# sortmerna/sortmerna

Measured on AMD Instinct MI355X. Metric: reads/sec (150 bp vs smr_v4.3_default_db-sized DB), higher is better.
Workload: dtype u8/i32

## Files before the change

include/smr_hip.h:

```cpp
#ifndef SMR_HIP_H
#define SMR_HIP_H
#include <stddef.h>
#include <stdint.h>

#ifdef __cplusplus
extern "C" {
#endif

#define SMR_OK 0
#define SMR_ERR_ARG (-1)
#define SMR_ERR_IO (-2)
#define SMR_ERR_DEVICE (-3)
#define SMR_ERR_CAPACITY (-4)
#define SMR_ERR_STATE (-5)

typedef struct smr_ctx smr_ctx;
typedef struct smr_index smr_index;
typedef struct smr_reads smr_reads;

typedef struct {
  uint32_t skiplengths[3];
  int32_t  num_seeds;
  int32_t  min_lis;
  int32_t  edges;
// ... 108 lines not shown
  int32_t paired_in, paired_out, out2, sout;
  int32_t want_aligned, want_other;
} smr_fxsplit_opts;
int smr_fastx_split(smr_ctx*, int mates , const smr_fxsplit_opts*,
                    const uint8_t* hit , uint8_t* bytes, uint64_t cap, uint64_t off[9], uint64_t* need);
int smr_fastx_split_times(const smr_ctx*, double ms[4]);
typedef struct {
  int  want_sam, want_blast;
  char blast_cols[64];
  double lambda, K;
  uint64_t full_ref_corr, full_read_corr;
} smr_rows_opts;
int smr_rows_part(smr_ctx*, int slot, const smr_params*, const smr_index* ix, const smr_rows_opts*,
                  uint8_t* bytes, uint64_t cap, uint64_t off[3], uint64_t* need);
int smr_rows_times(const smr_ctx*, double ms[4]);
int smr_rows_fmt_batch(smr_ctx*, uint32_t n, const uint32_t* num, const uint32_t* den, char* out);
int smr_pairwise_part(smr_ctx*, int slot, const smr_params*, const smr_index* ix, double lambda, double K, uint64_t full_ref_corr, uint64_t full_read_corr,
                      uint8_t* bytes, uint64_t cap, uint64_t* need);
int smr_pairwise_times(const smr_ctx*, double ms[4]);
typedef struct { uint32_t ref_num, n_reads; uint64_t off; } smr_otu_group;
int smr_otu_part(smr_ctx*, int slot, const smr_params*, const smr_index* ix, double min_id, double min_cov,
                 uint8_t* bytes, uint64_t cap, smr_otu_group* groups, uint64_t groups_cap, uint64_t need[2] , int* any_yid_ycov);
int smr_otu_times(const smr_ctx*, double ms[5]);
int smr_otu_sort_batch(smr_ctx*, uint32_t n, const uint32_t* keys, uint32_t key_bits, uint32_t* perm);
int smr_fastx_denovo(smr_ctx*, int mates, const smr_fxsplit_opts*, const uint8_t* dn ,
                     uint8_t* bytes, uint64_t cap, uint64_t off[5], uint64_t* need);
int smr_state_reset(smr_ctx*);

int smr_align_part(smr_ctx*, int slot, const smr_params*);
int smr_traceback(smr_ctx*, int slot, const smr_params*);

int smr_counters(smr_ctx*, uint64_t* out, uint32_t n_db);
int smr_counters_device(smr_ctx*, void** dptr, uint32_t* n_u64);
int smr_counters_accumulate(smr_ctx*, void* d_acc, uint32_t n_u64);

int smr_idcov_part(smr_ctx*, int slot, const smr_params*, double min_id, double min_cov);
int smr_idcov_counters(smr_ctx*, uint64_t out[4]);
int smr_idcov_counters_device(smr_ctx*, void** dptr, uint32_t* n_u64);
#define SMR_COUNTERS_WITH_IDCOV 70
int smr_idcov_batch(smr_ctx*, uint32_t n, const uint8_t* reads, const uint64_t* read_off, const uint8_t* refs, const uint64_t* ref_off,
                    const uint32_t* cigars, const uint64_t* cigar_off, const int32_t* read_begin, const int32_t* read_end, const uint32_t* readlen,
                    double min_id, double min_cov, uint32_t* out);

int    smr_results_fetch(smr_ctx*);
size_t smr_result_record(const smr_ctx*, uint32_t read_idx, uint8_t* buf, size_t cap);
size_t smr_result_record_batch(const smr_ctx*, int batch, uint32_t read_idx, uint8_t* buf, size_t cap);
int    smr_result_is_hit(const smr_ctx*, uint32_t read_idx);

int smr_state_import(smr_ctx*, const uint8_t* bytes, const uint64_t* off, uint32_t n);
int smr_state_export(smr_ctx*, uint8_t* bytes, uint64_t cap, uint64_t* off, uint32_t n, uint64_t* need);
int smr_counters_import(smr_ctx*, const uint64_t* in, uint32_t n_db);

int smr_seed_scan(smr_ctx*, int slot, const smr_params*, int strand, int pass, uint64_t* n_hits_out);
int smr_seed_hits_fetch(smr_ctx*, uint32_t* triples, uint64_t cap_triples, uint64_t* n_out);

typedef struct {
  double   seed_ms;  uint64_t seed_launches;
  double   chain_ms; uint64_t chain_launches;
  double   trace_ms; uint64_t trace_launches;
  uint64_t n_windows, n_lookup, n_node, n_entry, n_hit, n_read_bytes;
  uint64_t n_sw_fwd, n_sw_rev, n_sw_cells;
  uint64_t n_sw_spec, n_sw_spec_used;
  uint64_t n_seed_redo;
  uint64_t hit_list_cap;
  uint64_t n_seed_shared;
  uint64_t n_seed_shared_builds;
} smr_prof;
int smr_index_build_gpu(smr_ctx*, const char* ref_fasta, uint32_t lnwin, double max_mb, uint32_t max_pos,
                        smr_index** parts_out, uint32_t cap_parts, uint32_t* n_parts_out, char* err, size_t errcap);

int smr_sw_selfcheck(smr_ctx*, uint32_t n_cases, uint32_t seed, uint32_t max_len, uint64_t* n_bad);
int smr_sw_mode(smr_ctx*, int set_to);
int smr_walk_rounds(const smr_ctx*, uint32_t out[3]);
int smr_ssw_batch(smr_ctx*, uint32_t n_pairs, const uint8_t* reads, const uint64_t* read_off, const uint8_t* refs, const uint64_t* ref_off,
                  int match, int mismatch, int score_N, int gap_open, int gap_ext, uint32_t filters, int mode, int32_t* out);
int smr_sw_long_rows(int m);
typedef struct {
  uint32_t read, win_off;
  uint16_t aq, m, nref;
  uint8_t reversed, list_b;
} smr_sw16_task;
int smr_sw16_batch(smr_ctx*, uint32_t n_tasks, const smr_sw16_task* tasks, const uint8_t* ref, uint64_t ref_len, int force_any_n,
                   int match, int mismatch, int score_N, int gap_open, int gap_ext, uint32_t filters, int rows, uint32_t blocks, int32_t* out);
int smr_sw16_launches(const smr_ctx*, uint64_t out[8]);
int smr_cigar_batch(smr_ctx*, uint32_t n_pairs, const uint8_t* reads, const uint64_t* read_off, const uint8_t* refs, const uint64_t* ref_off,
                    const uint16_t* scores, int match, int mismatch, int score_N, int gap_open, int gap_ext,
                    uint32_t* cigar_out, uint64_t cigar_cap, uint64_t* cigar_off_out);
int smr_prof_reset(smr_ctx*);
int smr_prof_get(smr_ctx*, smr_prof* out);
typedef struct { char name[32]; double ms; uint64_t launches; uint64_t bytes; } smr_kprof;
int smr_prof_kernels(smr_ctx*, smr_kprof* out, uint32_t cap, uint32_t* n_out);

typedef struct smr_report smr_report;
typedef struct {
  int fastx;
  int other;
  int blast_tabular;
  char blast_cols[64];
  int sam;
  int blast_pairwise;
  int sam_sq;
  int paired_in;
  int paired_out;
  int out2;
  int sout;
  int zip_out;
  int otu_map;
  int denovo;
  double min_id, min_cov;
} smr_report_opts;
int smr_report_open(const char* out_dir, const smr_report_opts*, int is_fastq, smr_report** out, char* err, size_t errcap);
int smr_report_set_db(smr_report*, uint32_t index_num, double lambda, double K, uint64_t full_ref_corr, uint64_t full_read_corr);
int smr_report_set_part(smr_report*, uint32_t index_num, uint32_t part, const smr_index*);
int smr_report_add(smr_report*, const char* header, const char* seq, const char* qual, const uint8_t* record, size_t record_len);
int smr_report_add_pair(smr_report*, const char* header1, const char* seq1, const char* qual1, const uint8_t* record1, size_t record1_len,
                        const char* header2, const char* seq2, const char* qual2, const uint8_t* record2, size_t record2_len);
int smr_report_add_fastx(smr_report*, const uint8_t* bytes, const uint64_t off[9]);
int smr_report_add_rows(smr_report*, uint32_t index_num, uint32_t part, const uint8_t* bytes, const uint64_t off[3]);
int smr_report_skip_rows(smr_report*, int on);
int smr_report_add_pairwise(smr_report*, uint32_t index_num, uint32_t part, const uint8_t* bytes, uint64_t n);
int smr_report_skip_pairwise(smr_report*, int on);
int smr_report_skip_fastx(smr_report*, int on);
int smr_report_add_otu(smr_report*, uint32_t index_num, uint32_t part, const uint8_t* bytes, uint64_t n_bytes, const smr_otu_group* groups,
                       uint64_t n_groups, int any_yid_ycov);
int smr_report_skip_otu(smr_report*, int on);
int smr_report_add_denovo(smr_report*, const uint8_t* bytes, const uint64_t off[5]);
int smr_report_skip_denovo(smr_report*, int on);
int smr_report_otu_count(smr_report*, uint64_t* total_otu);
int smr_report_otu_merge(smr_report* dst, smr_report* src);
int smr_report_set_cmdline(smr_report*, const char* cmdline);
int smr_report_close(smr_report*);
const char* smr_report_last_error(const smr_report*);

typedef struct {
  const char* ref_file;
  uint32_t skiplengths[3];
  double lambda, K;
  uint32_t minimal_score;
  uint64_t reads_matched;
} smr_summary_db;
typedef struct {
  const char* cmdline; const char* pid; const char* timestamp;
  uint32_t seed_len; int32_t num_seeds, edges, match, mismatch, gap_open, gap_ext, score_N; int32_t sam_sq; int32_t threads;
  const char* const* reads_files; uint32_t n_reads_files;
  uint64_t total_reads, num_aligned, all_reads_len; uint32_t min_read_len, max_read_len;
  const smr_summary_db* dbs; uint32_t n_dbs;
  int is_denovo; uint64_t total_denovo;
  int is_otu_map; uint64_t total_id_cov, total_otu;
} smr_summary;
int smr_summary_write(const char* path, const smr_summary*);

size_t smr_readstats_record(uint64_t all_reads_count, uint64_t all_reads_len, uint32_t min_read_len, uint32_t max_read_len, uint64_t num_aligned,
                            uint64_t num_short, const uint64_t* reads_matched_per_db, uint32_t n_db, uint8_t* buf, size_t cap);
size_t smr_readstats_key(const char* const* reads_files, uint32_t n_files, char* buf, size_t cap);

#ifdef __cplusplus
}
#endif
#endif
```

sortmerna_amd/capi.py:

```python
import ctypes as C
import os

from . import build as _build


class Params(C.Structure):
    _fields_ = [
        ("skiplengths", C.c_uint32 * 3), ("num_seeds", C.c_int32), ("min_lis", C.c_int32), ("edges", C.c_int32),
        ("is_as_percent", C.c_int32), ("match", C.c_int32), ("mismatch", C.c_int32), ("score_N", C.c_int32),
        ("gap_open", C.c_int32), ("gap_ext", C.c_int32), ("num_alignments", C.c_uint32), ("is_best", C.c_int32),
        ("is_full_search", C.c_int32), ("is_forward", C.c_int32), ("is_reverse", C.c_int32), ("minoccur", C.c_uint32),
        ("minimal_score", C.c_uint32), ("index_num", C.c_uint32), ("part", C.c_uint32),
        ("is_last_index_part", C.c_int32),
    ]


class IndexInfo(C.Structure):
    _fields_ = [
        ("lnwin", C.c_uint32), ("n_kmers", C.c_uint32), ("trie_words", C.c_uint64), ("n_ids", C.c_uint32),
        ("n_pos", C.c_uint64), ("n_refs", C.c_uint32), ("ref_bytes", C.c_uint64), ("n_nodes", C.c_uint64),
        ("n_buckets", C.c_uint64), ("n_entries", C.c_uint64), ("bg", C.c_double * 4), ("full_len", C.c_uint64),
        ("numseq", C.c_uint64), ("n_parts", C.c_uint32),
    ]


class ReportOpts(C.Structure):
    _fields_ = [("fastx", C.c_int), ("other", C.c_int), ("blast_tabular", C.c_int), ("blast_cols", C.c_char * 64), ("sam", C.c_int),
                ("blast_pairwise", C.c_int), ("sam_sq", C.c_int), ("paired_in", C.c_int), ("paired_out", C.c_int), ("out2", C.c_int), ("sout", C.c_int), ("zip_out", C.c_int),
                ("otu_map", C.c_int), ("denovo", C.c_int), ("min_id", C.c_double), ("min_cov", C.c_double)]


class FxSplitOpts(C.Structure):
    _fields_ = [("layout", C.c_int32), ("paired_in", C.c_int32), ("paired_out", C.c_int32), ("out2", C.c_int32), ("sout", C.c_int32),
                ("want_aligned", C.c_int32), ("want_other", C.c_int32)]


class RowsOpts(C.Structure):
    _fields_ = [("want_sam", C.c_int), ("want_blast", C.c_int), ("blast_cols", C.c_char * 64), ("lam", C.c_double), ("K", C.c_double),
                ("full_ref_corr", C.c_uint64), ("full_read_corr", C.c_uint64)]


class SummaryDb(C.Structure):
    _fields_ = [("ref_file", C.c_char_p), ("skiplengths", C.c_uint32 * 3), ("lam", C.c_double), ("K", C.c_double),
                ("minimal_score", C.c_uint32), ("reads_matched", C.c_uint64)]


class Summary(C.Structure):
    _fields_ = [("cmdline", C.c_char_p), ("pid", C.c_char_p), ("timestamp", C.c_char_p), ("seed_len", C.c_uint32),
                ("num_seeds", C.c_int32), ("edges", C.c_int32), ("match", C.c_int32), ("mismatch", C.c_int32), ("gap_open", C.c_int32),
                ("gap_ext", C.c_int32), ("score_N", C.c_int32), ("sam_sq", C.c_int32), ("threads", C.c_int32),
                ("reads_files", C.POINTER(C.c_char_p)), ("n_reads_files", C.c_uint32),
                ("total_reads", C.c_uint64), ("num_aligned", C.c_uint64), ("all_reads_len", C.c_uint64),
                ("min_read_len", C.c_uint32), ("max_read_len", C.c_uint32), ("dbs", C.POINTER(SummaryDb)), ("n_dbs", C.c_uint32),
                ("is_denovo", C.c_int), ("total_denovo", C.c_uint64), ("is_otu_map", C.c_int), ("total_id_cov", C.c_uint64), ("total_otu", C.c_uint64)]


class Prof(C.Structure):
    _fields_ = [
        ("seed_ms", C.c_double), ("seed_launches", C.c_uint64), ("chain_ms", C.c_double), ("chain_launches", C.c_uint64),
        ("trace_ms", C.c_double), ("trace_launches", C.c_uint64), ("n_windows", C.c_uint64), ("n_lookup", C.c_uint64),
        ("n_node", C.c_uint64), ("n_entry", C.c_uint64), ("n_hit", C.c_uint64), ("n_read_bytes", C.c_uint64),
        ("n_sw_fwd", C.c_uint64), ("n_sw_rev", C.c_uint64), ("n_sw_cells", C.c_uint64), ("n_sw_spec", C.c_uint64), ("n_sw_spec_used", C.c_uint64), ("n_seed_redo", C.c_uint64), ("hit_list_cap", C.c_uint64),
        ("n_seed_shared", C.c_uint64), ("n_seed_shared_builds", C.c_uint64),
    ]


class Kprof(C.Structure):
    _fields_ = [("name", C.c_char * 32), ("ms", C.c_double), ("launches", C.c_uint64), ("bytes", C.c_uint64)]


EXPORTS = [
    "smr_otu_part", "smr_otu_times", "smr_otu_sort_batch", "smr_fastx_denovo", "smr_report_add_otu", "smr_report_skip_otu", "smr_report_add_denovo", "smr_report_skip_denovo",
    "smr_params_default", "smr_params_refused", "smr_index_load_files", "smr_index_build", "smr_index_build_gpu", "smr_index_write_files", "smr_index_save", "smr_index_load_flat", "smr_index_selfcheck", "smr_index_free",
    "smr_index_get_info", "smr_minimal_score", "smr_minimal_score_split", "smr_refstats_corrected_split", "smr_reads_pack", "smr_reads_load_fastx", "smr_reads_load_fastx_mt", "smr_reads_load_fastx_text", "smr_reads_is_fastq", "smr_reads_record_text", "smr_reads_free", "smr_reads_slice",
    "smr_reads_digest", "smr_reads_count", "smr_reads_total_len", "smr_reads_min_len", "smr_reads_max_len", "smr_create", "smr_device_count", "smr_destroy",
    "smr_last_error", "smr_tuning_text", "smr_index_upload", "smr_index_check_device", "smr_index_pigeonhole", "smr_seed_tuples_fetch", "smr_seed_pool_info", "smr_cand_info_enable", "smr_cand_info", "smr_cand_routes", "smr_index_unload", "smr_batch_select", "smr_set_seed_mode", "smr_reads_upload", "smr_reads_upload_batch", "smr_reads_upload_fastx", "smr_reads_upload_fastx_batch", "smr_reads_upload_fastx_file", "smr_fastx_info", "smr_fastx_times", "smr_fastx_split", "smr_fastx_split_times", "smr_rows_part", "smr_rows_times", "smr_rows_fmt_batch", "smr_pairwise_part", "smr_pairwise_times", "smr_state_reset", "smr_align_part",
    "smr_traceback", "smr_counters", "smr_counters_device", "smr_state_import", "smr_state_export", "smr_counters_import", "smr_results_fetch", "smr_result_record", "smr_result_record_batch", "smr_counters_accumulate",
    "smr_result_is_hit", "smr_seed_scan", "smr_seed_hits_fetch", "smr_sw_selfcheck", "smr_sw_mode", "smr_walk_rounds", "smr_ssw_batch", "smr_sw16_batch", "smr_sw16_launches", "smr_sw_long_rows", "smr_cigar_batch", "smr_idcov_part", "smr_idcov_counters", "smr_idcov_counters_device", "smr_idcov_batch", "smr_prof_reset", "smr_prof_get", "smr_prof_kernels", "smr_refstats_corrected", "smr_report_open",
    "smr_report_set_db", "smr_report_set_part", "smr_report_add", "smr_report_add_pair", "smr_report_add_fastx", "smr_report_skip_fastx", "smr_report_add_rows", "smr_report_skip_rows", "smr_report_add_pairwise", "smr_report_skip_pairwise", "smr_report_set_cmdline", "smr_report_otu_count", "smr_report_otu_merge", "smr_report_close", "smr_report_last_error",
    "smr_summary_write", "smr_readstats_record", "smr_readstats_key",
]

_lib = None


def load(rebuild_if_stale=True):
    global _lib
    if _lib is not None:
        return _lib
    path = _build.LIB
    if rebuild_if_stale and _build.is_stale():
        path = _build.build_library()
    if not os.path.isfile(path):
        raise RuntimeError("libsmr_hip.so is missing; run sortmerna_amd/build.py (needs hipcc)")
    _lib = bind(C.CDLL(path))
    return _lib


def bind(L):
    vp, cp, u32, u64, i32 = C.c_void_p, C.c_char_p, C.c_uint32, C.c_uint64, C.c_int
    L.smr_params_default.argtypes = [C.POINTER(Params)]
    L.smr_index_load_files.restype = i32
    L.smr_index_load_files.argtypes = [cp, u32, cp, C.POINTER(vp), cp, C.c_size_t]
    L.smr_index_build.restype = i32
    L.smr_index_build.argtypes = [cp, u32, C.c_double, u32, u32, C.POINTER(vp), u32, C.POINTER(u32), cp, C.c_size_t]
    L.smr_index_build_gpu.restype = i32
    L.smr_index_build_gpu.argtypes = [vp, cp, u32, C.c_double, u32, C.POINTER(vp), u32, C.POINTER(u32), cp, C.c_size_t]
    L.smr_index_write_files.restype = i32
    L.smr_index_write_files.argtypes = [C.POINTER(vp), u32, cp, cp, cp, C.c_size_t]
    L.smr_index_save.restype = i32
    L.smr_index_save.argtypes = [vp, cp, u64, cp, C.c_size_t]
    L.smr_index_load_flat.restype = i32
    L.smr_index_load_flat.argtypes = [cp, u64, C.POINTER(vp), cp, C.c_size_t]
    L.smr_index_selfcheck.restype = i32
    L.smr_index_selfcheck.argtypes = [vp, cp, C.c_size_t]
    L.smr_index_free.argtypes = [vp]
    L.smr_index_get_info.restype = i32
    L.smr_index_get_info.argtypes = [vp, C.POINTER(IndexInfo)]
    L.smr_minimal_score.restype = u32
    L.smr_minimal_score.argtypes = [C.c_double, C.c_double, C.POINTER(C.c_double), u64, u64, u64, u64, C.c_double]
    L.smr_minimal_score_split.restype = u32
    L.smr_minimal_score_split.argtypes = [C.c_double, C.c_double, C.POINTER(C.c_double), u64, u64, u64, u64, C.c_double, u32]
    L.smr_reads_pack.restype = i32
    L.smr_reads_pack.argtypes = [cp, vp, u32, C.POINTER(vp)]
    L.smr_reads_load_fastx.restype = i32
    L.smr_reads_load_fastx.argtypes = [cp, u64, u64, C.POINTER(vp), cp, C.c_size_t]
    L.smr_reads_load_fastx_mt.restype = i32
    L.smr_reads_load_fastx_mt.argtypes = [cp, u32, C.POINTER(vp), cp, C.c_size_t]
    L.smr_reads_load_fastx_text.restype = i32
    L.smr_reads_load_fastx_text.argtypes = [cp, u32, C.POINTER(vp), cp, C.c_size_t]
    L.smr_reads_is_fastq.restype = i32
    L.smr_reads_is_fastq.argtypes = [vp]
    L.smr_reads_record_text.restype = i32
    L.smr_reads_record_text.argtypes = [vp, u32, cp, C.c_size_t, cp, C.c_size_t, cp, C.c_size_t, C.POINTER(C.c_size_t)]
    L.smr_reads_free.argtypes = [vp]
    for f in ("smr_reads_count", "smr_reads_min_len", "smr_reads_max_len"):
        getattr(L, f).restype = u32
        getattr(L, f).argtypes = [vp]
    L.smr_reads_digest.restype = u64
    L.smr_reads_digest.argtypes = [vp]
    L.smr_reads_total_len.restype = u64
    L.smr_reads_total_len.argtypes = [vp]
    L.smr_create.restype = i32
    L.smr_create.argtypes = [i32, C.POINTER(vp), cp, C.c_size_t]
    L.smr_destroy.argtypes = [vp]
    L.smr_last_error.restype = cp
    L.smr_last_error.argtypes = [vp]
    L.smr_tuning_text.restype = i32
    L.smr_tuning_text.argtypes = [vp, cp, C.c_size_t]
    L.smr_index_upload.restype = i32
    L.smr_index_upload.argtypes = [vp, vp, i32]
    L.smr_index_check_device.restype = i32
    L.smr_index_check_device.argtypes = [vp, i32, vp]
    L.smr_index_pigeonhole.restype = i32
    L.smr_index_pigeonhole.argtypes = [vp, C.POINTER(C.POINTER(C.c_uint32)), C.POINTER(u64), C.POINTER(C.POINTER(C.c_uint32)), C.POINTER(u64), cp, C.c_size_t]
    L.smr_seed_tuples_fetch.restype = i32
    L.smr_seed_tuples_fetch.argtypes = [vp, vp, u64, vp, u32, C.POINTER(u32)]
    L.smr_seed_pool_info.restype = i32
    L.smr_seed_pool_info.argtypes = [vp, C.POINTER(u64)]
    L.smr_cand_info_enable.restype = i32
    L.smr_cand_info_enable.argtypes = [vp, i32]
    L.smr_cand_info.restype = i32
    L.smr_cand_info.argtypes = [vp, C.POINTER(u64)]
    L.smr_cand_routes.restype = i32
    L.smr_cand_routes.argtypes = [vp, vp, u32]
    L.smr_index_unload.restype = i32
    L.smr_index_unload.argtypes = [vp, i32]
    L.smr_batch_select.restype = i32
    L.smr_batch_select.argtypes = [vp, i32]
    L.smr_set_seed_mode.restype = i32
    L.smr_set_seed_mode.argtypes = [vp, i32]
    L.smr_reads_upload.restype = i32
    L.smr_reads_upload.argtypes = [vp, vp, u32]
    L.smr_state_reset.restype = i32
    L.smr_state_reset.argtypes = [vp]
    L.smr_align_part.restype = i32
    L.smr_align_part.argtypes = [vp, i32, C.POINTER(Params)]
    L.smr_traceback.restype = i32
    L.smr_traceback.argtypes = [vp, i32, C.POINTER(Params)]
    L.smr_counters.restype = i32
    L.smr_counters.argtypes = [vp, C.POINTER(u64), u32]
    L.smr_state_import.restype = i32
    L.smr_state_import.argtypes = [vp, vp, vp, u32]
    L.smr_state_export.restype = i32
    L.smr_state_export.argtypes = [vp, vp, u64, vp, u32, C.POINTER(u64)]
    L.smr_counters_import.restype = i32
    L.smr_counters_import.argtypes = [vp, C.POINTER(u64), u32]
    L.smr_counters_device.restype = i32
    L.smr_counters_device.argtypes = [vp, C.POINTER(vp), C.POINTER(u32)]
    L.smr_results_fetch.restype = i32
    L.smr_results_fetch.argtypes = [vp]
    L.smr_result_record.restype = C.c_size_t
    L.smr_result_record.argtypes = [vp, u32, vp, C.c_size_t]
    L.smr_result_record_batch.restype = C.c_size_t
    L.smr_result_record_batch.argtypes = [vp, i32, u32, vp, C.c_size_t]
    L.smr_counters_accumulate.restype = i32
    L.smr_counters_accumulate.argtypes = [vp, vp, u32]
    L.smr_result_is_hit.restype = i32
    L.smr_result_is_hit.argtypes = [vp, u32]
    L.smr_seed_scan.restype = i32
    L.smr_seed_scan.argtypes = [vp, i32, C.POINTER(Params), i32, i32, C.POINTER(u64)]
    L.smr_seed_hits_fetch.restype = i32
    L.smr_seed_hits_fetch.argtypes = [vp, vp, u64, C.POINTER(u64)]
    L.smr_sw_selfcheck.restype = i32
    L.smr_sw_selfcheck.argtypes = [vp, u32, u32, u32, C.POINTER(u64)]
    L.smr_ssw_batch.restype = i32
    L.smr_ssw_batch.argtypes = [vp, u32, vp, vp, vp, vp, i32, i32, i32, i32, i32, u32, i32, vp]
    L.smr_sw16_batch.restype = i32
    L.smr_sw16_batch.argtypes = [vp, u32, vp, vp, u64, i32, i32, i32, i32, i32, i32, u32, i32, u32, vp]
    L.smr_sw16_launches.restype = i32
    L.smr_sw16_launches.argtypes = [vp, C.POINTER(u64)]
    L.smr_sw_long_rows.restype = i32
    L.smr_sw_long_rows.argtypes = [i32]
    L.smr_readstats_record.restype = C.c_size_t
    L.smr_readstats_record.argtypes = [u64, u64, u32, u32, u64, u64, vp, u32, vp, C.c_size_t]
    L.smr_readstats_key.restype = C.c_size_t
    L.smr_readstats_key.argtypes = [vp, u32, vp, C.c_size_t]
    L.smr_reads_upload_batch.restype = i32
    L.smr_reads_upload_batch.argtypes = [vp, i32, vp, u32]
    L.smr_reads_upload_fastx.restype = i32
    L.smr_reads_upload_fastx.argtypes = [vp, vp, u64, u32, u32, C.POINTER(vp)]
    L.smr_reads_upload_fastx_batch.restype = i32
    L.smr_reads_upload_fastx_batch.argtypes = [vp, i32, vp, u64, u32, u32, C.POINTER(vp)]
    L.smr_reads_upload_fastx_file.restype = i32
    L.smr_reads_upload_fastx_file.argtypes = [vp, cp, u32, u32, C.POINTER(vp), cp, C.c_size_t]
    L.smr_fastx_info.restype = i32
    L.smr_fastx_info.argtypes = [vp, C.POINTER(u64)]
    L.smr_fastx_times.restype = i32
    L.smr_fastx_times.argtypes = [vp, C.POINTER(C.c_double)]
    L.smr_fastx_split.restype = i32
    L.smr_fastx_split.argtypes = [vp, i32, C.POINTER(FxSplitOpts), vp, vp, u64, C.POINTER(u64), C.POINTER(u64)]
    L.smr_fastx_split_times.restype = i32
    L.smr_fastx_split_times.argtypes = [vp, C.POINTER(C.c_double)]
    L.smr_rows_part.restype = i32
    L.smr_rows_part.argtypes = [vp, i32, C.POINTER(Params), vp, C.POINTER(RowsOpts), vp, u64, C.POINTER(u64), C.POINTER(u64)]
    L.smr_rows_times.restype = i32
    L.smr_rows_times.argtypes = [vp, C.POINTER(C.c_double)]
    L.smr_rows_fmt_batch.restype = i32
    L.smr_rows_fmt_batch.argtypes = [vp, u32, vp, vp, vp]
    L.smr_report_add_rows.restype = i32
    L.smr_report_add_rows.argtypes = [vp, u32, u32, vp, C.POINTER(u64)]
    L.smr_report_skip_rows.restype = i32
    L.smr_report_skip_rows.argtypes = [vp, i32]
    L.smr_pairwise_part.restype = i32
    L.smr_pairwise_part.argtypes = [vp, i32, C.POINTER(Params), vp, C.c_double, C.c_double, u64, u64, vp, u64, C.POINTER(u64)]
    L.smr_pairwise_times.restype = i32
    L.smr_pairwise_times.argtypes = [vp, C.POINTER(C.c_double)]
    L.smr_report_add_pairwise.restype = i32
    L.smr_report_add_pairwise.argtypes = [vp, u32, u32, vp, u64]
    L.smr_report_skip_pairwise.restype = i32
    L.smr_report_skip_pairwise.argtypes = [vp, i32]
    L.smr_otu_part.restype = i32
    L.smr_otu_part.argtypes = [vp, i32, C.POINTER(Params), vp, C.c_double, C.c_double, vp, u64, vp, u64, C.POINTER(u64), C.POINTER(i32)]
    L.smr_otu_times.restype = i32
    L.smr_otu_times.argtypes = [vp, C.POINTER(C.c_double)]
    L.smr_otu_sort_batch.restype = i32
    L.smr_otu_sort_batch.argtypes = [vp, u32, vp, u32, vp]
    L.smr_fastx_denovo.restype = i32
    L.smr_fastx_denovo.argtypes = [vp, i32, C.POINTER(FxSplitOpts), vp, vp, u64, C.POINTER(u64), C.POINTER(u64)]
    L.smr_report_add_otu.restype = i32
    L.smr_report_add_otu.argtypes = [vp, u32, u32, vp, u64, vp, u64, i32]
    L.smr_report_skip_otu.restype = i32
    L.smr_report_skip_otu.argtypes = [vp, i32]
    L.smr_report_add_denovo.restype = i32
    L.smr_report_add_denovo.argtypes = [vp, vp, C.POINTER(u64)]
    L.smr_report_skip_denovo.restype = i32
    L.smr_report_skip_denovo.argtypes = [vp, i32]
    L.smr_report_add_fastx.restype = i32
    L.smr_report_add_fastx.argtypes = [vp, vp, C.POINTER(u64)]
    L.smr_report_skip_fastx.restype = i32
    L.smr_report_skip_fastx.argtypes = [vp, i32]
    L.smr_reads_slice.restype = i32
    L.smr_reads_slice.argtypes = [vp, u64, u64, C.POINTER(vp)]
    L.smr_idcov_part.restype = i32
    L.smr_idcov_part.argtypes = [vp, i32, C.POINTER(Params), C.c_double, C.c_double]
    L.smr_idcov_counters.restype = i32
    L.smr_idcov_counters.argtypes = [vp, C.POINTER(u64)]
    L.smr_idcov_counters_device.restype = i32
    L.smr_idcov_counters_device.argtypes = [vp, C.POINTER(vp), C.POINTER(u32)]
    L.smr_idcov_batch.restype = i32
    L.smr_idcov_batch.argtypes = [vp, u32, vp, vp, vp, vp, vp, vp, vp, vp, vp, C.c_double, C.c_double, vp]
    L.smr_cigar_batch.restype = i32
    L.smr_cigar_batch.argtypes = [vp, u32, vp, vp, vp, vp, vp, i32, i32, i32, i32, i32, vp, u64, vp]
    L.smr_sw_mode.restype = i32
    L.smr_sw_mode.argtypes = [vp, i32]
    L.smr_walk_rounds.restype = i32
    L.smr_walk_rounds.argtypes = [vp, C.POINTER(C.c_uint32)]
    L.smr_prof_reset.restype = i32
    L.smr_prof_reset.argtypes = [vp]
    L.smr_prof_get.restype = i32
    L.smr_prof_get.argtypes = [vp, C.POINTER(Prof)]
    L.smr_prof_kernels.restype = i32
# ... 30 lines not shown
```

sortmerna_amd/csrc/smr_engine.hip:

```cpp
#include <hip/hip_runtime.h>

#include <algorithm>
#include <mutex>
#include <cstdio>
#include <cstdlib>
#include <cstring>
#include <string>
#include <vector>

#include "smr_kernels.hpp"
#include "smr_idcov.hpp"
#include "smr_import.hpp"
#include "smr_export.hpp"
#include "smr_fastx.hpp"
#include "smr_fxsplit.hpp"
#include "smr_rows.hpp"
#include "smr_pairwise.hpp"
#include "smr_otu.hpp"
#include "smr_ibuild.hpp"
#include "smr_pgbuild.hpp"
#include "smr_hostmem.hpp"
#include "smr_devbuf.hpp"
#include "smr_score_text.hpp"
#include "smr_tuning.hpp"
// ... 81 lines not shown
  double ms[4] = {0, 0, 0, 0};
  FxSplitScratch() = default;
  FxSplitScratch(const FxSplitScratch&) = delete;
  FxSplitScratch& operator=(const FxSplitScratch&) = delete;
  ~FxSplitScratch() { for (auto e : ev) if (e) (void)hipEventDestroy(e); }
};

struct RowsScratch {
  DevBuf<uint4> stat, meta; DevBuf<unsigned long long> excl_s, excl_b, part_s, part_b; DevBuf<uint32_t> err; DevBuf<uint8_t> tab, out;
  uint32_t tab_n = 0; double tab_lambda = 0, tab_K = 0; uint64_t tab_ref = 0, tab_read = 0;
  hipEvent_t ev[7] = {};
  double ms[4] = {0, 0, 0, 0};
  RowsScratch() = default;
  RowsScratch(const RowsScratch&) = delete;
  RowsScratch& operator=(const RowsScratch&) = delete;
  ~RowsScratch() { for (auto e : ev) if (e) (void)hipEventDestroy(e); }
};

struct PairScratch {
  hipEvent_t ev[7] = {};
  double ms[4] = {0, 0, 0, 0};
  PairScratch() = default;
  PairScratch(const PairScratch&) = delete;
  PairScratch& operator=(const PairScratch&) = delete;
  ~PairScratch() { for (auto e : ev) if (e) (void)hipEventDestroy(e); }
};

struct OtuScratch {
  DevBuf<uint8_t> pass, out; DevBuf<uint2> meta; DevBuf<uint4> pairs; DevBuf<uint32_t> key[2], val[2], gstart, err;
  DevBuf<unsigned long long> excl, part, hist, wexcl, wpart, gexcl, gpart; DevBuf<OtuGroup> groups;
  hipEvent_t ev[10] = {};
  double ms[5] = {0, 0, 0, 0, 0};
  OtuScratch() = default;
  OtuScratch(const OtuScratch&) = delete;
  OtuScratch& operator=(const OtuScratch&) = delete;
  ~OtuScratch() { for (auto e : ev) if (e) (void)hipEventDestroy(e); }
};

struct smr_ctx {
  const Tuning tune;
  explicit smr_ctx(const Tuning& t) : tune(t) {}
  int device = 0;
  DevStream stream, upload_stream;
  std::string err;
  std::mutex err_m, sel_m;
  int n_cu = 256;
  DevIndex idx[64];
  Batch bt[SMR_MAX_BATCHES];
  Batch* b = &bt[0];
  DevBuf<uint32_t> d_pool; uint64_t pool_words = 0;
  uint64_t n_pool_grown = 0;
  uint32_t pool_inline = 0;
  uint32_t hcap = 4;
  int seed_exact = tune.seed_exact;
  uint32_t cand_bloom = tune.cand_bloom;
  int seed_shared = tune.seed_shared;
  DevBuf<uint16_t> d_sw_scr; uint32_t sw_scr_stride = 0;
  int last_seed_slot = -1;
  SharedSort shared;
  uint64_t n_seed_shared = 0, n_seed_shared_builds = 0;
  uint32_t ccap = tune.ccap;
  SeedScratch seed; SeedBufs sb = {};
  uint64_t sb_slots = 0; uint32_t sb_nk = 0;
  uint32_t chain_blocks = 0;
  DevBuf<unsigned long long> d_tuples; uint32_t chain_scap = 512;
  uint32_t keys_need = 0;
  bool chain_ext = false;
  DevBuf<uint32_t> d_stab; DevBuf<unsigned long long> d_tuples2;
  size_t chain_lds_attr = 0, begins_lds_attr = 0, split_lds_attr = 0, bins_lds_attr = 0;
  DevBuf<uint32_t> d_fidx; DevBuf<RState> d_fstate; DevBuf<AlignRec> d_faln;
  DevBuf<uint32_t> d_fidcov;
  DevBuf<uint8_t> d_xbytes; DevBuf<unsigned long long> d_xoff, d_xpart;
  int sw_mode = tune.sw_packed;
  DevBuf<unsigned long long> d_keys; uint32_t keys_cap = 0;
  DevBuf<unsigned long long> d_pairs; DevBuf<uint32_t> d_lis; uint32_t pairs_cap = 0;
  DevBuf<uint2> d_hits; uint32_t hits_cap = 0;
  DevBuf<uint8_t> d_rdq;
  DevBuf<uint2> d_mrec; DevBuf<uint32_t> d_mpool;
  DevBuf<uint2> d_wlist[2]; DevBuf<WState> d_wstate[2]; DevBuf<WTask> d_wtask[2]; DevBuf<uint2> d_wres[2];
  DevBuf<uint32_t> d_wtidx, d_wslow; DevBuf<unsigned long long> d_wctr; size_t walk_cap = 0; uint32_t walk_kcap = 0;
  size_t walk_lds_attr = 0, pg_lds_attr = 0, search_lds_attr = 0;
  uint64_t sw16_launches[8] = {};
  uint32_t walk_need[3] = {0, 0, 0};
  DevBuf<unsigned long long> d_wstat; uint32_t wstat_n = 0; int wstat_pass[8] = {}; uint32_t wstat_rm[8] = {};
  DevBuf<int> d_bound;
  DevBuf<uint32_t> d_tasks;
  DevBuf<uint8_t> d_trflags;
  DevBuf<int> d_trrows;
  EvPool ev;
  double kp_ms[KP_COUNT] = {}; uint64_t kp_l[KP_COUNT] = {};
  DevBuf<unsigned long long> d_ctr_snap;
  bool cinfo_on = false; DevBuf<uint8_t> d_croute; uint32_t croute_n = 0;
  uint32_t cinfo_attempts = 0, cinfo_retry[5] = {0, 0, 0, 0, 0};
  FxScratch fx[2];
  uint64_t fx_info[4] = {0, 0, 0, 0}; double fx_ms[5] = {0, 0, 0, 0, 0};
  FxSplitScratch fxs;
  RowsScratch rows;
  PairScratch pair;
  OtuScratch otu;
};
struct KpSave { double ms[KP_COUNT]; uint64_t l[KP_COUNT]; };

#define SEED_REDO_CAP 16384u

int dev_fail(smr_ctx* c, const char* call, hipError_t e) {
  std::lock_guard<std::mutex> l_(c->err_m);
  c->err = std::string(call) + ": " + hipGetErrorString(e);
  return SMR_ERR_DEVICE;
}

namespace {

#define HIPCHK(ctx, call)                                          \
  do {                                                             \
    hipError_t e_ = (call);                                        \
    if (e_ != hipSuccess) return dev_fail((ctx), #call, e_);       \
  } while (0)

void set_err(smr_ctx* c, const std::string& msg) { std::lock_guard<std::mutex> l_(c->err_m); c->err = msg; }


template <class T> struct arg_of { typedef T type; };
template <class... P> void launch(smr_ctx* c, void (*k)(P...), dim3 grid, dim3 block, size_t lds, typename arg_of<P>::type... a) {
  hipLaunchKernelGGL(k, grid, block, lds, c->stream, a...);
}
template <class... P> void launch_on(hipStream_t st, void (*k)(P...), dim3 grid, dim3 block, size_t lds, typename arg_of<P>::type... a) {
  hipLaunchKernelGGL(k, grid, block, lds, st, a...);
}
template <class... F> int raise_lds_limit(smr_ctx* c, size_t& high_water, size_t bytes, size_t free_bytes, F... kernels) {
  if (bytes <= free_bytes || bytes <= high_water) return SMR_OK;
  for (const void* k : {(const void*)kernels...}) HIPCHK(c, hipFuncSetAttribute(k, hipFuncAttributeMaxDynamicSharedMemorySize, (int)bytes));
  high_water = bytes;
  return SMR_OK;
}

const char* scheme_unsupported(int mismatch, int score_N, int gap_open, int gap_ext);
DParams make_dparams(const smr_ctx* c, const DevIndex& di, const smr_params* p) {
  DParams P;
  memset(&P, 0, sizeof P);
  P.lnwin = di.lnwin; P.partialwin = di.lnwin / 2;
  if (p->skiplengths[0] == 0 || p->skiplengths[1] == 0 || p->skiplengths[2] == 0) {
    P.skip[0] = di.lnwin; P.skip[1] = di.lnwin / 2; P.skip[2] = 3;
  } else { P.skip[0] = p->skiplengths[0]; P.skip[1] = p->skiplengths[1]; P.skip[2] = p->skiplengths[2]; }
  P.num_seeds = p->num_seeds; P.min_lis = p->min_lis; P.edges = p->edges; P.is_as_percent = p->is_as_percent;
  P.match = p->match; P.mismatch = p->mismatch; P.score_N = p->score_N; P.gap_open = p->gap_open; P.gap_ext = p->gap_ext;
  P.minimal_score = p->minimal_score; P.num_alignments = p->num_alignments;
  P.is_best = p->is_best; P.is_full_search = p->is_full_search; P.is_forward = p->is_forward; P.is_reverse = p->is_reverse;
  P.minoccur = p->minoccur; P.index_num = p->index_num; P.part = p->part; P.is_last_index_part = p->is_last_index_part;
  P.slots = c->b->slots;
  P.sw_mode = scheme_unsupported(p->mismatch, p->score_N, p->gap_open, p->gap_ext) ? -1 : c->sw_mode;
  P.sw_scratch = c->d_sw_scr; P.sw_scratch_stride = c->sw_scr_stride;
  return P;
}

const char* scheme_unsupported(int mismatch, int score_N, int gap_open, int gap_ext) {
  const int mm = std::max(-mismatch, -std::min(score_N, 0));
  if (2 * gap_open < mm || 2 * gap_ext < mm) return "scoring scheme outside the supported range (2*gap_open and 2*gap_ext must be >= |mismatch|)";
  if (score_N > 0) return "scoring scheme outside the supported range (score_N must be <= 0: the kernels pad sequences with N)";
  if (gap_open <= gap_ext) return "scoring scheme outside the supported range (gap_open must be greater than gap_ext: the reference's 16-bit kernel ends its lazy-F loop early otherwise, ssw.c:496-507)";
  return nullptr;
}

int check_params(smr_ctx* c, const smr_params* p, bool sw = true) {
  if (!p) { set_err(c, "null params"); return SMR_ERR_ARG; }
  if (p->index_num >= 64) { set_err(c, "index_num must be < 64"); return SMR_ERR_ARG; }
  if ((uint64_t)p->minoccur >= 0x3FFFFFFFull) { set_err(c, "minoccur must be < 2^30 - 1"); return SMR_ERR_ARG; }
// ... 410 lines not shown
  c->wstat_n = 0;
  const uint32_t tb = 256, nb = (B.n + tb - 1) / tb;
  const int single = (p->is_forward != 0) ^ (p->is_reverse != 0);
  launch(c, k_ctr_begin, dim3(1), dim3(256), 0, B.d_ctr, c->d_ctr_snap);
  launch(c, k_begin_part, dim3(nb), dim3(tb), 0, dreads(c), P, B.d_saved, B.d_saved_aln, B.d_work, B.d_work_aln, B.d_rw, B.d_ctr);
  for (int count = 0; count < (single ? 1 : 2); count++) {
    launch(c, k_begin_strand, dim3(nb), dim3(tb), 0, B.n, P, count, B.d_work, B.d_rw);
    HIPCHK(c, hipMemsetAsync(&B.d_ctr[C_PCUR], 0, C_NSHARD * C_PCUR_STRIDE * 8, c->stream));
    for (int pass = 0; pass < 3; pass++) {
      if (pass > 0 && P.skip[pass] == P.skip[pass - 1]) continue;
      if ((rc = launch_seed(c, di, P, pass, !p->is_last_index_part, ((single && p->is_reverse) || count == 1) ? 1 : 0))) return rc;
      if ((rc = launch_chain(c, di, P, plan, pass, single || count == 1))) return rc;
    }
  }
  HIPCHK(c, hipGetLastError());
  return SMR_OK;
}

int judge_attempt(smr_ctx* c, const DParams& P, const std::vector<unsigned long long>& h, bool& retry) {
  int rc;
  retry = false;
  if (h[C_ERR_HITCAP]) { c->cinfo_retry[0]++; if (!grow_hcap(c, P.partialwin)) return SMR_ERR_CAPACITY; retry = true; }
  if (h[C_ERR_POOL]) { c->cinfo_retry[1]++; if ((rc = grow_pool(c))) return rc; retry = true; }
  if (h[C_ERR_PAIRS]) {
    c->cinfo_retry[2]++;
    c->pairs_cap *= 4; c->hits_cap *= 4; c->d_pairs.release(); c->d_lis.release(); c->d_hits.release(); c->d_tuples.release(); c->d_tuples2.release();
    if (c->pairs_cap > (1u << 22)) { set_err(c, "per-read candidate scratch exceeds capacity"); return SMR_ERR_CAPACITY; }
    retry = true;
  }
  if (h[C_ERR_REDO]) { c->cinfo_retry[3]++; c->seed_exact = 1; retry = true; }
  {
    Batch& B = *c->b;
    if (h[C_SEED_REDO] < B.redo_seen || h[C_WINDOWS] < B.win_seen) B.redo_seen = B.win_seen = 0;
    const unsigned long long redo = h[C_SEED_REDO] - B.redo_seen, waves = (h[C_WINDOWS] - B.win_seen) / 32;
    B.redo_seen = h[C_SEED_REDO]; B.win_seen = h[C_WINDOWS];
    if (!retry && redo * 64 > waves && c->ccap < PG_CAND_CAP_MAX) {
      c->ccap *= 2;
      say(c->tune, "%llu of ~%llu seed-search waves overflowed their candidate pool: %u records per wave from now on\n", redo, waves, c->ccap);
    }
  }
  if (h[C_ERR_SCAP]) {
    if (c->chain_ext) { set_err(c, "more than 49152 references share seeds with one read (candidate set capacity)"); return SMR_ERR_CAPACITY; }
    c->chain_ext = true; retry = true; c->cinfo_retry[4]++;
    say(c->tune, "a read shares seeds with more references than its wave's LDS table holds: per-block global candidate tables enabled (%.1f GB)\n",
        (double)c->chain_blocks * (4.0 * CH_EXT_CAP * 4 + (double)c->pairs_cap * 8 + (double)CH_EXT_CAP * 8) / 1e9);
    if (c->keys_cap < CH_EXT_CAP) { c->d_keys.release(); c->keys_cap = 0; c->keys_need = CH_EXT_CAP; }
  }
  if (h[C_ERR_SLOTS]) { set_err(c, "a read produced more alignments than max_alignments_per_read (smr_reads_upload)"); return SMR_ERR_CAPACITY; }
  return SMR_OK;
}
}

extern "C" int smr_align_part(smr_ctx* c, int slot, const smr_params* p) {
  if (!c || slot < 0 || slot >= 64) return SMR_ERR_ARG;
  if (!c->idx[slot].used || !c->b->d_saved) { set_err(c, "index slot empty or no reads uploaded"); return SMR_ERR_STATE; }
  if (c->b->idcov_ran) { set_err(c, "smr_align_part after smr_idcov_part: the id / coverage pass counts final alignments (denovo_stats runs after align, processor.cpp:368); smr_state_reset or upload first"); return SMR_ERR_STATE; }
  HIPCHK(c, hipSetDevice(c->device));
  int rc = check_params(c, p); if (rc) return rc;
  const DevIndex& di = c->idx[slot];
  if (di.lnwin < 8 || di.lnwin > 20) { set_err(c, "unsupported seed length"); return SMR_ERR_ARG; }
  DParams P = make_dparams(c, di, p);
  if ((rc = refuse_percent_edges(c, di, p))) return rc;
  const AlignPlan plan = align_plan(c, P);
  if (plan.lds > 150 * 1024) { set_err(c, "reads too long for this build of the SW kernel (LDS)"); return SMR_ERR_CAPACITY; }
  c->b->last_num_alignments = p->num_alignments;
  c->b->fetched = false;
  ev_drop(c);
  if (c->b->n == 0) return SMR_OK;
  if ((rc = ensure_pool(c))) return rc;
  if (plan.striped && (rc = ensure_striped_scratch(c, P, p))) return rc;
  std::vector<unsigned long long> h;
  HIPCHK(c, hipMemcpyAsync(c->d_ctr_snap, c->b->d_ctr, C_TOTAL * 8, hipMemcpyDeviceToDevice, c->stream));
  c->cinfo_attempts = 0;
  for (int q = 0; q < 5; q++) c->cinfo_retry[q] = 0;
  for (int attempt = 0; attempt < 16; attempt++) {
    const KpSave kp0 = kp_save(c);
    if ((rc = run_attempt(c, di, P, p, plan))) return rc;
    if ((rc = read_ctr(c, h))) return rc;
    ev_collect(c);
    bool retry;
    if ((rc = judge_attempt(c, P, h, retry))) return rc;
    if (retry) { kp_restore(c, kp0); continue; }
    if ((rc = adapt_walk_rounds(c))) return rc;
    if ((rc = launch_begins(c, di, P, plan))) return rc;
    launch(c, k_commit_part, dim3((c->b->n + 255u) / 256u), dim3(256), 0, c->b->n, P, c->b->d_saved, c->b->d_saved_aln, c->b->d_work, c->b->d_work_aln, c->b->d_rw);
    HIPCHK(c, hipGetLastError());
    HIPCHK(c, hipStreamSynchronize(c->stream));
    ev_collect(c);
    return SMR_OK;
  }
  set_err(c, "capacity retries exhausted");
  return SMR_ERR_CAPACITY;
}

#include "smr_engine_trace.hpp"
#include "smr_engine_idcov.hpp"
#include "smr_engine_import.hpp"
#include "smr_engine_export.hpp"
#include "smr_engine_fastx.hpp"
#include "smr_engine_fxsplit.hpp"
#include "smr_engine_rows.hpp"
#include "smr_engine_pairwise.hpp"
#include "smr_engine_otu.hpp"
extern "C" int smr_counters(smr_ctx* c, uint64_t* out, uint32_t n_db) {
  if (!c || !out) return SMR_ERR_ARG;
  HIPCHK(c, hipSetDevice(c->device));
  std::vector<unsigned long long> h;
  int rc = read_ctr(c, h); if (rc) return rc;
  out[0] = h[C_NUM_ALIGNED]; out[1] = h[C_NUM_SHORT];
  for (uint32_t i = 0; i < n_db && i < 64; i++) out[2 + i] = h[C_PER_DB + i];
  return SMR_OK;
}
extern "C" int smr_counters_device(smr_ctx* c, void** dptr, uint32_t* n_u64) {
  if (!c || !dptr || !n_u64) return SMR_ERR_ARG;
  *dptr = c->b->d_ctr; *n_u64 = C_PER_DB + 64;
  return SMR_OK;
}

__global__ void k_ctr_accumulate(const unsigned long long* __restrict__ ctr, unsigned long long* __restrict__ acc, uint32_t n) {
  const uint32_t k = blockIdx.x * blockDim.x + threadIdx.x;
  if (k < n) acc[k] += ctr[k < C_PER_DB + 64 ? k : C_IDCOV + (k - (C_PER_DB + 64))];
}
extern "C" int smr_counters_accumulate(smr_ctx* c, void* d_acc, uint32_t n_u64) {
  if (!c || !d_acc || n_u64 > C_PER_DB + 64 + 4 || !c->b->d_ctr) return SMR_ERR_ARG;
  HIPCHK(c, hipSetDevice(c->device));
  launch(c, k_ctr_accumulate, dim3((n_u64 + 127) / 128), dim3(128), 0, (const unsigned long long*)c->b->d_ctr, (unsigned long long*)d_acc, n_u64);
  HIPCHK(c, hipGetLastError());
  HIPCHK(c, hipStreamSynchronize(c->stream));
  return SMR_OK;
}

__global__ void k_results_compact(uint32_t n, uint32_t slots, const RState* __restrict__ saved, const AlignRec* __restrict__ saved_aln,
                                  uint32_t* __restrict__ out_idx, RState* __restrict__ out_state, AlignRec* __restrict__ out_aln, unsigned long long* __restrict__ ctr) {
  const uint32_t r = blockIdx.x * blockDim.x + threadIdx.x;
  RState s; s.n_align = 0;
  if (r < n) s = saved[r];
  const uint32_t p = block_append(&ctr[C_FETCH_N], s.n_align != 0);
  if (s.n_align == 0) return;
  out_idx[p] = r; out_state[p] = s;
  for (uint32_t k = 0; k < s.n_align && k < slots; k++) out_aln[(size_t)p * slots + k] = saved_aln[(size_t)r * slots + k];
}

extern "C" int smr_results_fetch(smr_ctx* c) {
  if (!c || !c->b->d_saved) return SMR_ERR_STATE;
  HIPCHK(c, hipSetDevice(c->device));
  Batch& B = *c->b;
  int rc;
  const size_t need_r = std::max<size_t>(B.n, 1), need_a = std::max<size_t>((size_t)B.n * B.slots, 1);
  if ((rc = c->d_fidx.reserve(c, need_r)) || (rc = c->d_fstate.reserve(c, need_r)) || (rc = c->d_faln.reserve(c, need_a))) return rc;
  HIPCHK(c, hipMemsetAsync(&B.d_ctr[C_FETCH_N], 0, 8, c->stream));
  if (B.n) launch(c, k_results_compact, dim3((B.n + 1023) / 1024), dim3(1024), 0, B.n, B.slots, (const RState*)B.d_saved, (const AlignRec*)B.d_saved_aln,
                              c->d_fidx, c->d_fstate, c->d_faln, B.d_ctr);
  std::vector<unsigned long long> h;
  rc = read_ctr(c, h); if (rc) return rc;
  const uint64_t cw = std::min<uint64_t>(h[C_CIGAR_CURSOR], B.cigar_words);
  const size_t nhit = (size_t)std::min<unsigned long long>(h[C_FETCH_N], B.n);
  B.h_cigar.resize(cw);
  B.h_idx.resize(nhit); B.h_state.resize(nhit); B.h_aln.resize(nhit * B.slots);
  if (nhit) {
    HIPCHK(c, hipMemcpyAsync(B.h_idx.data(), c->d_fidx, nhit * 4, hipMemcpyDeviceToHost, c->stream));
    HIPCHK(c, hipMemcpyAsync(B.h_state.data(), c->d_fstate, nhit * sizeof(RState), hipMemcpyDeviceToHost, c->stream));
    HIPCHK(c, hipMemcpyAsync(B.h_aln.data(), c->d_faln, nhit * B.slots * sizeof(AlignRec), hipMemcpyDeviceToHost, c->stream));
  }
  if (cw) HIPCHK(c, hipMemcpyAsync(B.h_cigar.data(), B.d_cigar, cw * 4, hipMemcpyDeviceToHost, c->stream));
  B.h_idcov.clear();
  if (B.d_idcov && nhit) {
// ... 110 lines not shown
  if (tuples) { if (cap_tuples < nt) return SMR_ERR_CAPACITY; if (nt) HIPCHK(c, hipMemcpy(tuples, c->sb.srt, (size_t)nt * sizeof(SeedTup), hipMemcpyDeviceToHost)); }
  if (cbase) { if (cap_cbase < c->sb.nc + 1u) return SMR_ERR_CAPACITY; HIPCHK(c, hipMemcpy(cbase, c->sb.cbase, (size_t)(c->sb.nc + 1u) * 4, hipMemcpyDeviceToHost)); }
  return SMR_OK;
}

extern "C" int smr_seed_pool_info(smr_ctx* c, uint64_t info[4]) {
  if (!c || !info) return SMR_ERR_ARG;
  HIPCHK(c, hipSetDevice(c->device));
  std::vector<unsigned long long> cur(C_NSHARD * C_PCUR_STRIDE, 0ull);
  if (c->b->d_ctr) {
    HIPCHK(c, hipMemcpyAsync(cur.data(), &c->b->d_ctr[C_PCUR], cur.size() * 8, hipMemcpyDeviceToHost, c->stream));
    HIPCHK(c, hipStreamSynchronize(c->stream));
  }
  const uint64_t region = std::min<uint64_t>(c->pool_words, 0x7FFFFFF0ull) / C_NSHARD;
  uint64_t hi = 0;
  for (int s = 0; s < C_NSHARD; s++) if (cur[s * C_PCUR_STRIDE]) hi = std::max<uint64_t>(hi, s * region + cur[s * C_PCUR_STRIDE]);
  info[0] = c->pool_words; info[1] = c->n_pool_grown; info[2] = hi; info[3] = c->pool_inline;
  return SMR_OK;
}

extern "C" int smr_cand_info_enable(smr_ctx* c, int on) {
  if (!c) return SMR_ERR_ARG;
  c->cinfo_on = on != 0;
  if (!c->cinfo_on) c->croute_n = 0;
  return SMR_OK;
}
extern "C" int smr_cand_info(smr_ctx* c, uint64_t info[13]) {
  if (!c || !info) return SMR_ERR_ARG;
  info[0] = c->cinfo_attempts;
  for (int q = 0; q < 5; q++) info[1 + q] = c->cinfo_retry[q];
  info[6] = c->chain_ext ? 1 : 0; info[7] = c->chain_scap; info[8] = c->keys_cap; info[9] = c->pairs_cap; info[10] = c->hits_cap;
  info[11] = c->cinfo_on ? 1 : 0; info[12] = c->croute_n;
  return SMR_OK;
}
extern "C" int smr_cand_routes(smr_ctx* c, uint8_t* out, uint32_t n) {
  if (!c || !out) return SMR_ERR_ARG;
  if (!c->cinfo_on || !c->d_croute || n != c->croute_n) { set_err(c, "smr_cand_routes: no route bytes for that many reads (smr_cand_info_enable before smr_align_part)"); return SMR_ERR_STATE; }
  HIPCHK(c, hipSetDevice(c->device));
  if (n) { HIPCHK(c, hipMemcpyAsync(out, c->d_croute, (size_t)n, hipMemcpyDeviceToHost, c->stream)); HIPCHK(c, hipStreamSynchronize(c->stream)); }
  return SMR_OK;
}

extern "C" int smr_seed_hits_fetch(smr_ctx* c, uint32_t* triples, uint64_t cap_triples, uint64_t* n_out) {
  if (!c || !n_out) return SMR_ERR_ARG;
  HIPCHK(c, hipSetDevice(c->device));
  std::vector<unsigned long long> h;
  int rc = read_ctr(c, h); if (rc) return rc;
  uint64_t words = h[C_POOL_CURSOR] ? std::min<uint64_t>(c->pool_words, 0x7FFFFFF0ull) : 0;
  std::vector<uint32_t> pool(words);
  std::vector<RWork> rw(c->b->n);
  if (words) HIPCHK(c, hipMemcpy(pool.data(), c->d_pool, words * 4, hipMemcpyDeviceToHost));
  if (c->b->n) HIPCHK(c, hipMemcpy(rw.data(), c->b->d_rw, (size_t)c->b->n * sizeof(RWork), hipMemcpyDeviceToHost));
  std::vector<uint32_t> po;
  if (c->last_seed_slot >= 0 && c->idx[c->last_seed_slot].used) {
    const DevIndex& di = c->idx[c->last_seed_slot];
    po.resize((size_t)di.n_ids + 1);
    HIPCHK(c, hipMemcpy(po.data(), di.pos_off, po.size() * 4, hipMemcpyDeviceToHost));
  }
  auto orig = [&](uint32_t idp) -> uint32_t {
    if (po.size() < 2) return idp;
    size_t lo = 0, hi = po.size() - 1;
    while (hi - lo > 1) { const size_t mid = (lo + hi) / 2; if ((uint64_t)po[mid] + mid <= idp) lo = mid; else hi = mid; }
    return (uint32_t)lo;
  };
  uint64_t o = 0;
  for (uint32_t r = 0; r < c->b->n; r++) {
    for (int pp = 0; pp < 3; pp++) {
      const uint32_t cnt = rw[r].blk_cnt[pp], bo = rw[r].blk_off[pp];
      for (uint32_t q = 0; q < cnt && (uint64_t)bo + 2 * q + 1 < words; q++) {
        if (triples && o < cap_triples) { triples[3 * o] = r; triples[3 * o + 1] = orig(pool[bo + 2 * q]); triples[3 * o + 2] = pool[bo + 2 * q + 1]; }
        o++;
      }
    }
  }
  *n_out = o;
  return SMR_OK;
}

extern "C" int smr_prof_reset(smr_ctx* c) {
  if (!c) return SMR_ERR_ARG;
  HIPCHK(c, hipSetDevice(c->device));
  for (int k = 0; k < KP_COUNT; k++) { c->kp_ms[k] = 0; c->kp_l[k] = 0; }
  c->n_seed_shared = c->n_seed_shared_builds = 0;
  for (int k = 0; k < SMR_MAX_BATCHES; k++)
    if (c->bt[k].d_ctr) {
      HIPCHK(c, hipMemsetAsync(&c->bt[k].d_ctr[C_WINDOWS], 0, 9 * 8, c->stream));
      HIPCHK(c, hipMemsetAsync(&c->bt[k].d_ctr[C_SW_SPEC], 0, 3 * 8, c->stream));
      HIPCHK(c, hipMemsetAsync(&c->bt[k].d_ctr[C_TUP_F], 0, C_SHARD_NX * 8, c->stream));
      HIPCHK(c, hipMemsetAsync(&c->bt[k].d_ctr[C_SHARDS], 0, C_SHARD_W * C_NSHARD * 8, c->stream));
    }
  HIPCHK(c, hipStreamSynchronize(c->stream));
  return SMR_OK;
}
extern "C" int smr_prof_get(smr_ctx* c, smr_prof* o) {
  if (!c || !o) return SMR_ERR_ARG;
  HIPCHK(c, hipSetDevice(c->device));
  std::vector<unsigned long long> h(C_TOTAL, 0), t(C_TOTAL);
  for (int k = 0; k < SMR_MAX_BATCHES; k++) {
    if (!c->bt[k].d_ctr) continue;
    HIPCHK(c, hipMemcpyAsync(t.data(), c->bt[k].d_ctr, C_TOTAL * 8, hipMemcpyDeviceToHost, c->stream));
    HIPCHK(c, hipStreamSynchronize(c->stream));
    if (c->tune.debug_phases) {
      unsigned long long ph[7] = {0, 0, 0, 0, 0, 0, 0};
      for (int s2 = 0; s2 < C_NSHARD; s2++) for (int q = 0; q < 7; q++) ph[q] += t[C_SHARDS + C_SHARD_W * s2 + C_SHARD_PH + q];
      fprintf(stderr, "[smr] phase cycles (batch %d): %llu %llu %llu %llu %llu %llu %llu  (-DSMR_CHAIN_PHASES: claim, gather+prefix, walk1, walk2+cands, pairs+sort, "
              "window/lis/book, sw; -DSMR_SEED_PHASES (k_seed_pg): setup, directory ranges, entries, -, candidate selection, output, -)\n", k, ph[0], ph[1], ph[2], ph[3], ph[4], ph[5], ph[6]);
    }
    fold_shards(t);
    for (int q = 0; q < C_COUNT; q++) h[q] += t[q];
  }
  o->seed_ms = c->kp_ms[KP_KEYS] + c->kp_ms[KP_SPLIT] + c->kp_ms[KP_BINS] + c->kp_ms[KP_PG0] + c->kp_ms[KP_PG1] + c->kp_ms[KP_FINISH]; o->seed_launches = c->kp_l[KP_KEYS];
  o->chain_ms = c->kp_ms[KP_CAND] + c->kp_ms[KP_CHAIN] + c->kp_ms[KP_BEGINS] + c->kp_ms[KP_WALK] + c->kp_ms[KP_SW16] + c->kp_ms[KP_WNEXT]; o->chain_launches = c->kp_l[KP_CAND] + c->kp_l[KP_BEGINS];
  o->trace_ms = c->kp_ms[KP_TRACE]; o->trace_launches = c->kp_l[KP_TRACE];
  o->n_windows = h[C_WINDOWS]; o->n_lookup = h[C_LOOKUP]; o->n_node = h[C_NODE]; o->n_entry = h[C_ENTRY]; o->n_hit = h[C_HIT]; o->n_read_bytes = h[C_READ_BYTES];
  o->n_sw_fwd = h[C_SW_FWD]; o->n_sw_rev = h[C_SW_REV]; o->n_sw_cells = h[C_SW_CELLS];
  o->n_sw_spec = h[C_SW_SPEC]; o->n_sw_spec_used = h[C_SW_SPEC_USED]; o->n_seed_redo = h[C_SEED_REDO]; o->hit_list_cap = c->hcap;
  o->n_seed_shared = c->n_seed_shared; o->n_seed_shared_builds = c->n_seed_shared_builds;
  return SMR_OK;
}

extern "C" int smr_prof_kernels(smr_ctx* c, smr_kprof* out, uint32_t cap, uint32_t* n_out) {
  if (!c || !out || !n_out) return SMR_ERR_ARG;
  HIPCHK(c, hipSetDevice(c->device));
  std::vector<unsigned long long> h(C_TOTAL, 0), t(C_TOTAL);
  for (int k = 0; k < SMR_MAX_BATCHES; k++) {
    if (!c->bt[k].d_ctr) continue;
    HIPCHK(c, hipMemcpyAsync(t.data(), c->bt[k].d_ctr, C_TOTAL * 8, hipMemcpyDeviceToHost, c->stream));
    HIPCHK(c, hipStreamSynchronize(c->stream));
    fold_shards(t);
    for (int q = 0; q < C_COUNT; q++) h[q] += t[q];
  }
  const unsigned long long T = h[C_TUP_ALL];
  unsigned long long bytes[KP_COUNT] = {};
  bytes[KP_KEYS] = h[C_B_KEYS] + sizeof(SeedTup) * T;
  bytes[KP_SPLIT] = bytes[KP_BINS] = 2 * sizeof(SeedTup) * T;
  bytes[KP_PG0] = h[C_B_PG0]; bytes[KP_PG1] = h[C_B_PG1]; bytes[KP_FINISH] = h[C_B_FIN];
  uint32_t n = 0;
  for (int k = 0; k < KP_COUNT && n < cap; k++, n++) {
    memset(&out[n], 0, sizeof out[n]);
    snprintf(out[n].name, sizeof out[n].name, "%s", KP_NAME[k]);
    out[n].ms = c->kp_ms[k]; out[n].launches = c->kp_l[k]; out[n].bytes = bytes[k];
  }
  *n_out = n;
  return SMR_OK;
}
```

sortmerna_amd/csrc/smr_engine_chain.hpp:

```cpp

uint32_t chain_edges(const DParams& P, uint32_t len) { return P.is_as_percent ? (uint32_t)((P.edges / 100.0) * len) + 1 : (uint32_t)std::max(P.edges, 0); }
void chain_lds(const smr_ctx* c, const DParams& P, uint32_t& ml, uint32_t& rf, uint32_t& rq, size_t& bytes) {
  const uint32_t mq_len = std::min<uint32_t>(c->b->max_len, SW_X4_MAX_ROWS);
  ml = (c->b->max_len + 15) & ~15u;
  rf = (c->b->max_len + 2 * chain_edges(P, c->b->max_len) + 16 + 15) & ~15u;
  rq = std::min(rf, (mq_len + 2 * chain_edges(P, mq_len) + 16 + 15) & ~15u);
  bytes = 5 * (size_t)std::min<uint32_t>(ml, SW_X4_MAX_ROWS) + (size_t)9 * rq + (size_t)CH_KEYS_LDS * 8 + (size_t)std::max<uint32_t>(4u * CH_PAIRS_LDS, 2u * c->chain_scap) * 4 +
          (size_t)CH_HITS_LDS * 8 + (size_t)(CH_HITS_LDS + 8) * 4 + (size_t)c->chain_scap * 4;
}
void chain_lds(const smr_ctx* c, const DParams& P, uint32_t& ml, uint32_t& rf, size_t& bytes) { uint32_t rq; chain_lds(c, P, ml, rf, rq, bytes); }
int ensure_bound(smr_ctx* c, uint32_t blocks, uint32_t rf) {
  if (c->b->max_len <= SW_X4_MAX_ROWS) return SMR_OK;
  int rc = c->d_bound.reserve(c, (size_t)blocks * 2 * rf);
  return rc ? rc : c->d_rdq.reserve(c, (size_t)blocks * ((c->b->max_len + 15) & ~15u));
}

struct AlignPlan { uint32_t ml, rf, rq; size_t lds; bool lng, striped, split, x4, begins_sw16; int rows; };
int sw16_rows(uint32_t max_len) {
  const uint32_t wmq = std::min<uint32_t>(max_len, WK_MAX_ROWS);
  return wmq <= 104 ? 13 : wmq <= 152 ? 19 : wmq <= 208 ? 26 : 32;
}
AlignPlan align_plan(const smr_ctx* c, const DParams& P) {
  AlignPlan a;
  chain_lds(c, P, a.ml, a.rf, a.rq, a.lds);
  const uint32_t max_len = c->b->max_len;
  const bool packed = P.sw_mode >= 1;
  a.lng = max_len > SW_X4_MAX_ROWS;
  a.striped = P.sw_mode < 0;
  a.split = packed && c->tune.walk_split && c->tune.handover && sw_pk_fits((int)std::min<uint32_t>(max_len, WK_MAX_ROWS), (int)a.rq, P.match, P.mismatch, P.score_N, P.gap_open);
  a.x4 = packed && !a.lng && sw_pk_fits((int)max_len, (int)a.rf, P.match, P.mismatch, P.score_N, P.gap_open);
  a.begins_sw16 = a.x4 && c->tune.walk_split && !c->tune.begins_x4;
  a.rows = sw16_rows(max_len);
  return a;
}

typedef decltype(&k_chain<false, false, false>) chain_fn;
chain_fn chain_kernel(bool ext, bool lng, bool striped) {
  static const chain_fn K[8] = {k_chain<false, false, false>, k_chain<true, false, false>, k_chain<false, true, false>, k_chain<true, true, false>,
                                k_chain<false, false, true>,  k_chain<true, false, true>,  k_chain<false, true, true>,  k_chain<true, true, true>};
  return K[(ext ? 1 : 0) | (lng ? 2 : 0) | (striped ? 4 : 0)];
}
typedef decltype(&k_begins<false, false>) begins_fn;
begins_fn begins_kernel(bool lng, bool striped) {
  static const begins_fn K[4] = {k_begins<false, false>, k_begins<true, false>, k_begins<false, true>, k_begins<true, true>};
  return K[(lng ? 1 : 0) | (striped ? 2 : 0)];
}
typedef decltype(&k_sw16<13>) sw16_fn;
void launch_sw16(smr_ctx* c, int rows, int counted, uint32_t blocks, const DReads& rd, const DIndex& ix, const DParams& P, const WTask* tasks, const uint32_t* tix, const uint32_t* tix2,
                 const unsigned long long* wc, uint2* res) {
  static const sw16_fn K[4] = {k_sw16<13>, k_sw16<19>, k_sw16<26>, k_sw16<32>};
  const int v = rows == 13 ? 0 : rows == 19 ? 1 : rows == 26 ? 2 : 3;
  launch(c, K[v], dim3(blocks ? blocks : (uint32_t)c->n_cu * 4u * (uint32_t)SW16_WAVES(rows)), dim3(64), 0, rd, ix, P, tasks, tix, tix2, wc, res);
  if (counted >= 0) c->sw16_launches[counted + v]++;
}

__global__ void k_wstat(const unsigned long long* __restrict__ wctr, unsigned long long* __restrict__ out, uint32_t rounds) {
  if (threadIdx.x < 32) out[threadIdx.x] = threadIdx.x < rounds ? wctr[(size_t)threadIdx.x * WC_STRIDE + WC_NLIST] : 0ull;
}
int adapt_walk_rounds(smr_ctx* c) {
  if (c->tune.walk_rounds_fixed || !c->wstat_n || !c->d_wstat) return SMR_OK;
  unsigned long long h[8 * 32];
  HIPCHK(c, hipMemcpyAsync(h, c->d_wstat, (size_t)c->wstat_n * 32 * 8, hipMemcpyDeviceToHost, c->stream));
  HIPCHK(c, hipStreamSynchronize(c->stream));
  const unsigned long long few = (unsigned long long)c->n_cu * 8ull;
  uint32_t need[3] = {0, 0, 0};
  for (uint32_t e = 0; e < c->wstat_n; e++) {
    uint32_t want = 2;
    for (uint32_t r = 0; r < c->wstat_rm[e]; r++) if (h[e * 32 + r] > few) want = r + 2 + (r + 1 == c->wstat_rm[e] ? 2u : 0u);
    need[c->wstat_pass[e]] = std::max(need[c->wstat_pass[e]], want);
  }
  for (int p = 0; p < 3; p++) if (need[p]) {
    const uint32_t prev = c->walk_need[p] ? c->walk_need[p] : c->tune.walk_rounds;
    c->walk_need[p] = std::min(c->tune.walk_rounds, need[p] >= prev ? need[p] : prev - std::max(1u, (prev - need[p]) / 2u));
  }
  c->wstat_n = 0;
  return SMR_OK;
}

int launch_chain(smr_ctx* c, const DevIndex& di, const DParams& P, const AlignPlan& plan, int pass, int is_last_strand) {
  Batch& B = *c->b;
  const uint32_t ml = plan.ml, rf = plan.rf, rq = plan.rq;
  const size_t lds = plan.lds;
  const bool split = plan.split;
  int rc;
  HIPCHK(c, hipMemsetAsync(&B.d_ctr[C_WORK_NEXT], 0, 8, c->stream));
  if ((rc = raise_lds_limit(c, c->chain_lds_attr, lds, 64 * 1024, chain_kernel(0, 0, 0), chain_kernel(1, 0, 0), chain_kernel(0, 1, 0), chain_kernel(1, 1, 0),
                            chain_kernel(0, 0, 1), chain_kernel(1, 0, 1), chain_kernel(0, 1, 1), chain_kernel(1, 1, 1)))) return rc;
  const uint32_t blocks = std::min<uint32_t>(c->chain_blocks, std::max(B.n, 1u));
  if ((rc = ensure_bound(c, c->chain_blocks, rf))) return rc;
  int* const gb = plan.lng ? c->d_bound.get() : nullptr;
  uint8_t* const grd = plan.lng ? c->d_rdq.get() : nullptr;
  if (c->tune.handover) {
    if ((rc = c->d_mrec.reserve(c, B.n)) || (rc = c->d_mpool.reserve(c, (size_t)((B.n + CAND_BLOCK - 1u) / CAND_BLOCK) * CAND_BLOCK * CAND_REC_WORDS))) return rc;
  }
  const uint2* const mrec = c->tune.handover ? c->d_mrec.get() : nullptr;
  const uint32_t wml = (std::min<uint32_t>(B.max_len, WK_MAX_ROWS) + 15) & ~15u;
  const uint32_t RMX = c->tune.walk_rounds, WK = c->tune.walk_k;
  const uint32_t RM = (!c->tune.walk_rounds_fixed && c->walk_need[pass]) ? std::min(RMX, c->walk_need[pass]) : RMX;
  if (split) {
    const size_t n = B.n;
    if (c->walk_cap < n || c->walk_kcap < WK) {
      for (int q = 0; q < 2; q++)
        if ((rc = c->d_wlist[q].alloc(c, n)) || (rc = c->d_wstate[q].alloc(c, n)) || (rc = c->d_wtask[q].alloc(c, n * WK)) || (rc = c->d_wres[q].alloc(c, n * WK))) return rc;
      if ((rc = c->d_wtidx.alloc(c, 2 * n * WK)) || (rc = c->d_wslow.alloc(c, n))) return rc;
      c->walk_cap = n; c->walk_kcap = WK;
    }
    if ((rc = c->d_wctr.reserve(c, (size_t)(RMX + 2) * WC_STRIDE)) || (rc = c->d_wstat.reserve(c, (size_t)8 * 32))) return rc;
    HIPCHK(c, hipMemsetAsync(c->d_wctr, 0, (size_t)(RMX + 2) * WC_STRIDE * 8, c->stream));
    if ((rc = raise_lds_limit(c, c->walk_lds_attr, (size_t)wml + rq, 64 * 1024, k_walk<true>))) return rc;
  }
  const size_t n_tix = (size_t)c->walk_cap * c->walk_kcap;
  unsigned long long* const n_slow = split ? c->d_wctr + (size_t)(RMX + 1) * WC_STRIDE : nullptr;
  const dim3 per_read((B.n + 255u) / 256u);
  ev_mark(c, KP_CAND);
  launch(c, k_cand, dim3((B.n + CAND_BLOCK - 1u) / CAND_BLOCK), dim3(256), CAND_LDS_BYTES(c->cand_bloom, c->tune.handover), dreads(c), dindex(di), P, pass, is_last_strand, B.d_work, B.d_rw, c->d_pool, B.d_marks, c->cand_bloom,
         c->tune.handover ? c->d_mrec.get() : nullptr, c->d_mpool, c->d_mpool.cap());
  if (split) {
    ev_mark(c, KP_WNEXT);
    launch(c, k_wlist, dim3((B.n + 1023u) / 1024u), dim3(1024), 0, dreads(c), B.d_marks, mrec, (uint32_t)WK_MAX_ROWS, c->d_wlist[0], c->d_wslow, c->d_wctr, n_slow, c->tune.walk_debug ? n_slow + 8 : nullptr, (P.num_seeds >= 2 && c->tune.walk_gather) ? 1 : 0);
    if (c->cinfo_on) launch(c, k_cand_route, per_read, dim3(256), 0, B.n, B.d_marks, mrec, c->d_wlist[0], c->d_wctr, 0, c->d_croute);
    const uint32_t walk_blocks = (uint32_t)c->n_cu * 4u * SMR_WALK_WAVES_PER_SIMD;
    for (uint32_t rnd = 0; rnd < RM; rnd++) {
      const int cur = (int)(rnd & 1u), prv = cur ^ 1;
      unsigned long long* const wc = c->d_wctr + (size_t)rnd * WC_STRIDE;
      const bool fin = rnd + 1 == RM;
      ev_mark(c, KP_WALK);
      launch(c, fin ? k_walk<true> : k_walk<false>, dim3(fin ? walk_blocks * 3u / SMR_WALK_WAVES_PER_SIMD : walk_blocks), dim3(64), fin ? (size_t)wml + rq : 0,
             dreads(c), dindex(di), P, pass, is_last_strand, B.d_work, B.d_work_aln, B.d_rw, B.d_ctr, mrec, c->d_mpool, c->d_pool, c->d_wlist[cur],
             c->d_wstate[prv], c->d_wtask[prv], c->d_wres[prv], c->d_wstate[cur], c->d_wtask[cur], c->d_wtidx, c->d_wtidx + n_tix, wc, WK, n_tix, (int)rnd, wml, rq, c->tune.walk_assume);
      if (fin) continue;
      ev_mark(c, KP_SW16);
      launch_sw16(c, plan.rows, 0, 0, dreads(c), dindex(di), P, c->d_wtask[cur], c->d_wtidx, c->d_wtidx + n_tix, wc, c->d_wres[cur]);
      ev_mark(c, KP_WNEXT);
      launch(c, k_wnext, dim3((uint32_t)c->n_cu * 2u), dim3(1024), 0, P, is_last_strand, B.d_work, B.d_rw, B.d_ctr, c->d_wlist[cur], c->d_wstate[cur],
             c->d_wres[cur], c->d_wlist[prv], wc, wc + WC_STRIDE, WK, n_tix, (int)rnd);
    }
    if (!c->tune.walk_rounds_fixed && c->wstat_n < 8) {
      launch(c, k_wstat, dim3(1), dim3(32), 0, c->d_wctr, c->d_wstat + (size_t)c->wstat_n * 32, RM);
      c->wstat_pass[c->wstat_n] = pass; c->wstat_rm[c->wstat_n] = RM; c->wstat_n++;
    }
    if (c->tune.walk_debug) {
      std::vector<unsigned long long> h((size_t)(RMX + 2) * WC_STRIDE);
      HIPCHK(c, hipMemcpyAsync(h.data(), c->d_wctr, h.size() * 8, hipMemcpyDeviceToHost, c->stream));
      HIPCHK(c, hipStreamSynchronize(c->stream));
      { const unsigned long long* q = &h[(size_t)(RMX + 1) * WC_STRIDE];
        fprintf(stderr, "libsmr_hip: walk rounds (pass %d): slow %llu (positions <= 64 / 128 / 256 / 512 / more / > 64 hits: %llu %llu %llu %llu %llu %llu);", pass, q[0], q[8], q[9], q[10], q[11], q[12], q[13]); }
      for (uint32_t rnd = 0; rnd < RM; rnd++) fprintf(stderr, " %llu/%llu+%llu", h[(size_t)rnd * WC_STRIDE + WC_NLIST], h[(size_t)rnd * WC_STRIDE + WC_NTASK], h[(size_t)rnd * WC_STRIDE + WC_NTASK2]);
      fprintf(stderr, "\n");
    }
  }
  ev_mark(c, KP_CHAIN);
  for (int ext = 0; ext <= (c->chain_ext ? 1 : 0); ext++) {
    if (ext) HIPCHK(c, hipMemsetAsync(&B.d_ctr[C_WORK_NEXT], 0, 8, c->stream));
    if (c->cinfo_on) launch(c, k_cand_route, per_read, dim3(256), 0, B.n, B.d_marks, nullptr, nullptr, nullptr, 1 + ext, c->d_croute);
    launch(c, chain_kernel(ext, plan.lng, plan.striped), dim3(blocks), dim3(64), lds, dreads(c), dindex(di), P, pass, is_last_strand, B.d_work, B.d_work_aln, B.d_rw, c->d_pool, B.d_ctr,
           c->d_tuples, c->d_keys, c->d_pairs, c->d_lis, c->d_hits, c->keys_cap, c->pairs_cap, c->hits_cap, ml, rf, c->chain_scap, c->chain_ext ? c->d_stab.get() : nullptr,
           c->chain_ext ? c->d_tuples2.get() : nullptr, rq, gb, grd, B.d_marks, mrec, c->d_mpool, split ? c->d_wslow.get() : nullptr, n_slow);
  }
  ev_stop(c);
  HIPCHK(c, hipGetLastError());
  return SMR_OK;
}

int launch_begins(smr_ctx* c, const DevIndex& di, const DParams& P, const AlignPlan& plan) {
  Batch& B = *c->b;
  int rc;
  const uint64_t ntot = (uint64_t)B.n * B.slots;
  if ((rc = c->d_tasks.reserve(c, 2 * ntot))) return rc;
  const int x4 = plan.x4 ? 1 : 0;
  const size_t lds_b = x4 ? (size_t)4 * (plan.ml + plan.rf) : (plan.lng ? 0 : (size_t)plan.ml + plan.rf);
  const uint32_t bg_blocks = (uint32_t)c->n_cu * 8u;
  if ((rc = ensure_bound(c, std::max(bg_blocks, c->chain_blocks), plan.rf))) return rc;
  if ((rc = raise_lds_limit(c, c->begins_lds_attr, lds_b, 64 * 1024, begins_kernel(0, 0), begins_kernel(1, 0), begins_kernel(0, 1), begins_kernel(1, 1)))) return rc;
  HIPCHK(c, hipMemsetAsync(&B.d_ctr[C_BEGIN_N], 0, 16, c->stream));
  ev_mark(c, KP_BEGINS);
  launch(c, k_begins_collect, dim3((uint32_t)((ntot + 1023) / 1024)), dim3(1024), 0, B.n, B.slots, B.d_work, B.d_rw, B.d_work_aln, c->d_tasks, B.d_ctr);
  const size_t task_cap = (size_t)c->walk_cap * c->walk_kcap;
  if (plan.begins_sw16 && c->d_wtask[0] && c->d_wctr && ntot <= task_cap) {
    for (int stage = 0; stage < 2; stage++) {
      HIPCHK(c, hipMemsetAsync(c->d_wctr, 0, (size_t)WC_STRIDE * 8, c->stream));
      launch(c, k_begins_prep, dim3((uint32_t)c->n_cu * 2u), dim3(1024), 0, dindex(di), B.slots, c->d_tasks, &B.d_ctr[C_BEGIN_N], B.d_work_aln, stage, c->d_wtask[0], c->d_wtidx, c->d_wctr);
      launch_sw16(c, plan.rows, 4, 0, dreads(c), dindex(di), P, c->d_wtask[0], c->d_wtidx, c->d_wtidx + task_cap, c->d_wctr, c->d_wres[0]);
      launch(c, k_begins_apply, dim3((uint32_t)c->n_cu * 4u), dim3(256), 0, c->d_tasks, &B.d_ctr[C_BEGIN_N], B.d_work_aln, stage, c->d_wtask[0], c->d_wres[0], B.d_ctr);
    }
  } else
    launch(c, begins_kernel(plan.lng, plan.striped), dim3(bg_blocks), dim3(64), lds_b, dreads(c), dindex(di), P, c->d_tasks, B.d_work_aln, B.d_ctr, plan.ml, plan.rf, x4,
           plan.lng ? c->d_bound.get() : nullptr, plan.lng ? c->d_rdq.get() : nullptr);
  ev_stop(c);
  return SMR_OK;
}

void fold_shards(std::vector<unsigned long long>& h) {
  for (int s = 0; s < C_NSHARD; s++)
    for (int k = 0; k < C_SHARD_W; k++) {
      if (k < C_SHARD_X) h[C_WINDOWS + k] += h[C_SHARDS + C_SHARD_W * s + k];
      else if (k < C_SHARD_X + C_SHARD_NX) h[C_TUP_F + k - C_SHARD_X] += h[C_SHARDS + C_SHARD_W * s + k];
      h[C_SHARDS + C_SHARD_W * s + k] = 0;
    }
  unsigned long long mx = 0;
  for (int s = 0; s < C_NSHARD; s++) mx = std::max(mx, h[C_PCUR + s * C_PCUR_STRIDE]);
  h[C_POOL_CURSOR] = mx;
}

int read_ctr(smr_ctx* c, std::vector<unsigned long long>& h) {
  h.resize(C_TOTAL);
  HIPCHK(c, hipMemcpyAsync(h.data(), c->b->d_ctr, C_TOTAL * 8, hipMemcpyDeviceToHost, c->stream));
  HIPCHK(c, hipStreamSynchronize(c->stream));
  fold_shards(h);
  return SMR_OK;
}
```

sortmerna_amd/csrc/smr_engine_swseam.hpp:

```cpp

__device__ __forceinline__ uint32_t sc_hash(uint32_t a, uint32_t b, uint32_t c) {
  uint32_t h = a * 0x9E3779B1u ^ (b + 0x7F4A7C15u) * 0x85EBCA6Bu ^ (c + 0x165667B1u) * 0xC2B2AE35u;
  h ^= h >> 15; h *= 0x2C1B3C6Du; h ^= h >> 12; h *= 0x297A2D39u; h ^= h >> 15;
  return h;
}
__global__ void __launch_bounds__(64) k_sw_selfcheck(uint32_t n_cases, uint32_t seed, uint32_t max_m, uint32_t lds_m, uint32_t lds_n,
                                                     int match, int mismatch, int scoreN, int go, int ge, int mode_b, unsigned long long* out) {
  SMR_DYN_LDS(unsigned char, lds_raw);
  uint8_t* rdq = lds_raw;
  uint8_t* rfq = rdq + lds_m;
  int* bound = (int*)(rfq + lds_n);
  __shared__ int s_n;
  const int lane = smr::lane_id();
  for (uint32_t cs = blockIdx.x; cs < n_cases; cs += gridDim.x) {
    const uint32_t hm = sc_hash(seed, cs, 1);
    const int m = 1 + (int)(hm % max_m);
    for (int q = lane; q < m; q += 64) { const uint32_t h = sc_hash(seed, cs, 100u + (uint32_t)q); rdq[q] = (h & 63u) == 0 ? 4 : (uint8_t)((h >> 8) & 3u); }
    __syncthreads();
    if (lane == 0) {
      int n = 0;
      const bool homolog = (hm >> 20) & 3u;
      const int flank = (int)((hm >> 24) & 15u);
      for (int q = 0; q < flank; q++) rfq[n++] = (uint8_t)(sc_hash(seed, cs, 5000u + (uint32_t)q) & 3u);
      for (int q = 0; q < m && n + 2 < (int)lds_n; q++) {
// ... 159 lines not shown
  HIPCHK(c, hipMemcpyAsync(d_ro, read_off, ((size_t)n_pairs + 1) * 8, hipMemcpyHostToDevice, c->stream));
  HIPCHK(c, hipMemcpyAsync(d_fo, ref_off, ((size_t)n_pairs + 1) * 8, hipMemcpyHostToDevice, c->stream));
  if (mode == 3) {
    for (uint32_t i = 0; i < n_pairs; i++) {
      const uint64_t m = read_off[i + 1] - read_off[i], n = ref_off[i + 1] - ref_off[i];
      if (m > SW_X4_MAX_ROWS || !sw_pk_fits((int)m, (int)n, match, mismatch, score_N, gap_open)) {
        set_err(c, "smr_ssw_batch mode 3: a pair is outside the range of the four-problem kernel"); return SMR_ERR_ARG;
      }
    }
    hipLaunchKernelGGL(k_ssw_batch_x4, dim3(std::min<uint32_t>((n_pairs + 3) / 4, (uint32_t)c->n_cu * 8u)), dim3(64), (size_t)4 * (lm + ln), c->stream, n_pairs, (const uint8_t*)d_reads,
                       (const unsigned long long*)d_ro, (const uint8_t*)d_refs, (const unsigned long long*)d_fo, lm, ln, match, mismatch, score_N, gap_open, gap_ext, filters, d_out);
  } else
  {
    const uint32_t gb = std::min<uint32_t>(n_pairs, (uint32_t)c->n_cu * 8u), stride = 5u * 16u * ((uint32_t)(mx_m + 7) / 8u + 1u);
    uint16_t* d_scr = nullptr;
    if (mode == 4) { IB_GET(d_scr_, uint16_t, (size_t)gb * stride); d_scr = d_scr_; }
    if (mode == 5) hipLaunchKernelGGL(k_ssw_long, dim3(gb), dim3(64), lds, c->stream, n_pairs, (const uint8_t*)d_reads,
                       (const unsigned long long*)d_ro, (const uint8_t*)d_refs, (const unsigned long long*)d_fo, lm, ln, match, mismatch, score_N, gap_open, gap_ext, filters, d_out);
    else if (mode == 4) hipLaunchKernelGGL(k_ssw_batch<true>, dim3(gb), dim3(64), lds, c->stream, n_pairs, (const uint8_t*)d_reads,
                       (const unsigned long long*)d_ro, (const uint8_t*)d_refs, (const unsigned long long*)d_fo, lm, ln, match, mismatch, score_N, gap_open, gap_ext, filters, -1, d_out, d_scr, stride);
    else hipLaunchKernelGGL(k_ssw_batch<false>, dim3(gb), dim3(64), lds, c->stream, n_pairs, (const uint8_t*)d_reads,
                       (const unsigned long long*)d_ro, (const uint8_t*)d_refs, (const unsigned long long*)d_fo, lm, ln, match, mismatch, score_N, gap_open, gap_ext, filters, mode, d_out, d_scr, stride);
  }
  HIPCHK(c, hipMemcpyAsync(out, d_out, (size_t)n_pairs * 5 * 4, hipMemcpyDeviceToHost, c->stream));
  HIPCHK(c, hipStreamSynchronize(c->stream));
  return SMR_OK;
}

extern "C" int smr_sw_long_rows(int m) { return smr::sw_long_rows(m); }

extern "C" int smr_sw16_batch(smr_ctx* c, uint32_t n_tasks, const smr_sw16_task* tasks, const uint8_t* ref, uint64_t ref_len, int force_any_n,
                              int match, int mismatch, int score_N, int gap_open, int gap_ext, uint32_t filters, int rows, uint32_t blocks, int32_t* out) {
  if (!c || (n_tasks && (!tasks || !out)) || (ref_len && !ref)) return SMR_ERR_ARG;
  if (rows != 13 && rows != 19 && rows != 26 && rows != 32) { set_err(c, "smr_sw16_batch: rows must be 13, 19, 26 or 32"); return SMR_ERR_ARG; }
  if (blocks > 65536u) { set_err(c, "smr_sw16_batch: at most 65536 blocks"); return SMR_ERR_ARG; }
  if (match <= 0 || match > 127 || mismatch > 0 || mismatch < -127 || score_N < -127 || gap_open < 0 || gap_open > 255 || gap_ext < 0 || gap_ext > 255) { set_err(c, "smr_sw16_batch: bad scoring options"); return SMR_ERR_ARG; }
  if (const char* why = scheme_unsupported(mismatch, score_N, gap_open, gap_ext)) { set_err(c, why); return SMR_ERR_ARG; }
  if (!c->b->used || !c->b->d_words) { set_err(c, "smr_sw16_batch: no reads uploaded into the selected batch"); return SMR_ERR_STATE; }
  (void)hipSetDevice(c->device);
  const uint32_t n_reads = c->b->n;
  std::vector<uint32_t> len(n_reads);
  if (n_reads) HIPCHK(c, hipMemcpyAsync(len.data(), c->b->d_len, (size_t)n_reads * 4, hipMemcpyDeviceToHost, c->stream));
  HIPCHK(c, hipStreamSynchronize(c->stream));
  std::vector<WTask> tk(std::max<uint32_t>(n_tasks, 1));
  std::vector<uint32_t> ia, ib;
  for (uint32_t i = 0; i < n_tasks; i++) {
    const smr_sw16_task& t = tasks[i];
    const char* why = nullptr;
    if (t.read >= n_reads) why = "read index outside the batch";
    else if (t.m == 0 || t.nref == 0) why = "empty span or window";
    else if (t.m > WK_MAX_ROWS || (int)t.m > 8 * rows) why = "span longer than the kernel takes (8 x rows, at most WK_MAX_ROWS)";
    else if ((uint64_t)t.aq + t.m > len[t.read]) why = "rows outside the read";
    else if ((uint64_t)t.win_off + t.nref > ref_len) why = "window outside the reference letters";
    else if (!sw_pk_fits((int)t.m, (int)t.nref, match, mismatch, score_N, gap_open)) why = "numbers outside the packed representation (sw_pk_fits)";
    else if (t.reversed > 1 || t.list_b > 1) why = "reversed / list_b must be 0 or 1";
    if (why) { set_err(c, std::string("smr_sw16_batch: task ") + std::to_string(i) + ": " + why); return SMR_ERR_ARG; }
    WTask o;
    memset(&o, 0, sizeof o);
    o.r = t.read; o.max_ref = 0; o.rf_start = t.win_off; o.ars = 0; o.head = 0; o.aq = t.aq; o.m = t.m; o.nref = t.nref; o.flags = t.reversed ? 1 : 0;
    tk[i] = o;
    (t.list_b ? ib : ia).push_back(i);
  }
  if (n_tasks == 0) return SMR_OK;
  DevPool pool;
  IB_GET(d_ref, uint8_t, ref_len + 8); IB_GET(d_tk, WTask, n_tasks); IB_GET(d_ia, uint32_t, n_tasks); IB_GET(d_ib, uint32_t, n_tasks);
  IB_GET(d_wc, unsigned long long, WC_STRIDE); IB_GET(d_res, uint2, n_tasks);
  HIPCHK(c, hipMemsetAsync(d_ref, 0, ref_len + 8, c->stream));
  if (ref_len) HIPCHK(c, hipMemcpyAsync(d_ref, ref, ref_len, hipMemcpyHostToDevice, c->stream));
  DIndex ix;
  memset(&ix, 0, sizeof ix);
  ix.ref_seq = d_ref;
  ix.ref_any_n = (force_any_n || (ref_len && memchr(ref, 4, ref_len))) ? 1u : 0u;
  DParams P;
  memset(&P, 0, sizeof P);
  P.match = match; P.mismatch = mismatch; P.score_N = score_N; P.gap_open = gap_open; P.gap_ext = gap_ext; P.sw_mode = c->sw_mode;
  unsigned long long wc[WC_STRIDE] = {};
  std::vector<uint2> res(n_tasks);
  wc[WC_NTASK] = ia.size(); wc[WC_NTASK2] = ib.size();
  HIPCHK(c, hipMemcpyAsync(d_tk, tk.data(), (size_t)n_tasks * sizeof(WTask), hipMemcpyHostToDevice, c->stream));
  if (!ia.empty()) HIPCHK(c, hipMemcpyAsync(d_ia, ia.data(), ia.size() * 4, hipMemcpyHostToDevice, c->stream));
  if (!ib.empty()) HIPCHK(c, hipMemcpyAsync(d_ib, ib.data(), ib.size() * 4, hipMemcpyHostToDevice, c->stream));
  HIPCHK(c, hipMemcpyAsync(d_wc, wc, sizeof wc, hipMemcpyHostToDevice, c->stream));
  HIPCHK(c, hipMemsetAsync(d_res, 0xEE, (size_t)n_tasks * sizeof(uint2), c->stream));
  launch_sw16(c, rows, -1, blocks, dreads(c), ix, P, d_tk, d_ia, d_ib, d_wc, d_res);
  HIPCHK(c, hipGetLastError());
  HIPCHK(c, hipMemcpyAsync(res.data(), d_res, (size_t)n_tasks * sizeof(uint2), hipMemcpyDeviceToHost, c->stream));
  HIPCHK(c, hipStreamSynchronize(c->stream));
  std::vector<uint32_t> beg;
  std::vector<WTask> tb(tk);
  for (uint32_t i = 0; i < n_tasks; i++) {
    int32_t* o = out + (size_t)i * 5;
    const int score = res[i].x > 65535u ? 65535 : (int)res[i].x;
    o[0] = score; o[1] = o[2] = o[3] = o[4] = -1;
    if (tasks[i].list_b) {
      if (res[i].y != 0xFFFFFFFFu) { set_err(c, "smr_sw16_batch: a score-only task came back with an end cell"); return SMR_ERR_DEVICE; }
      continue;
    }
    if (res[i].y == 0xFFFFFFFFu || res[i].y == 0xEEEEEEEEu) { set_err(c, "smr_sw16_batch: a task of the end-cell list came back without one"); return SMR_ERR_DEVICE; }
    const int end_ref = (int)(res[i].y >> 16) - 1, end_read = (int)(res[i].y & 0xFFFFu);
    o[2] = end_ref; o[4] = score > 0 ? end_read : 0;
    if (end_ref < -1 || end_ref >= (int)tk[i].nref || end_read >= (int)tk[i].m || (score > 0 && end_ref < 0)) {
      set_err(c, "smr_sw16_batch: task " + std::to_string(i) + " came back with an end cell outside its span and window"); return SMR_ERR_DEVICE;
    }
    if ((uint32_t)score >= filters && score > 0) {
      WTask& b = tb[i];
      b.m = (uint16_t)(end_read + 1); b.nref = (uint16_t)(end_ref + 1);
      b.aq = (uint16_t)(tk[i].aq + end_read); b.rf_start = tk[i].rf_start + (uint64_t)end_ref; b.flags = (uint16_t)(tk[i].flags | 2u);
      beg.push_back(i);
    }
  }
  if (beg.empty()) return SMR_OK;
  memset(wc, 0, sizeof wc);
  wc[WC_NTASK] = beg.size();
  HIPCHK(c, hipMemcpyAsync(d_tk, tb.data(), (size_t)n_tasks * sizeof(WTask), hipMemcpyHostToDevice, c->stream));
  HIPCHK(c, hipMemcpyAsync(d_ia, beg.data(), beg.size() * 4, hipMemcpyHostToDevice, c->stream));
  HIPCHK(c, hipMemcpyAsync(d_wc, wc, sizeof wc, hipMemcpyHostToDevice, c->stream));
  HIPCHK(c, hipMemsetAsync(d_res, 0xEE, (size_t)n_tasks * sizeof(uint2), c->stream));
  launch_sw16(c, rows, -1, blocks, dreads(c), ix, P, d_tk, d_ia, d_ib, d_wc, d_res);
  HIPCHK(c, hipGetLastError());
  HIPCHK(c, hipMemcpyAsync(res.data(), d_res, (size_t)n_tasks * sizeof(uint2), hipMemcpyDeviceToHost, c->stream));
  HIPCHK(c, hipStreamSynchronize(c->stream));
  for (uint32_t i : beg) {
    int32_t* o = out + (size_t)i * 5;
    if (res[i].y == 0xFFFFFFFFu || res[i].y == 0xEEEEEEEEu) { set_err(c, "smr_sw16_batch: a begin-cell task came back without a cell"); return SMR_ERR_DEVICE; }
    const int b_ref = (int)(res[i].y >> 16) - 1, b_read = (int)(res[i].y & 0xFFFFu);
    o[1] = o[2] - b_ref; o[3] = o[4] - b_read;
  }
  return SMR_OK;
}

extern "C" int smr_sw16_launches(const smr_ctx* c, uint64_t out[8]) {
  if (!c || !out) return SMR_ERR_ARG;
  for (int k = 0; k < 8; k++) out[k] = c->sw16_launches[k];
  return SMR_OK;
}

extern "C" int smr_sw_mode(smr_ctx* c, int set_to) {
  if (!c) return SMR_ERR_ARG;
  if (set_to >= 0 && set_to <= 2) c->sw_mode = set_to;
  return c->sw_mode;
}

extern "C" int smr_walk_rounds(const smr_ctx* c, uint32_t out[3]) {
  if (!c || !out) return SMR_ERR_ARG;
  for (int p = 0; p < 3; p++) out[p] = (!c->tune.walk_rounds_fixed && c->walk_need[p]) ? std::min(c->tune.walk_rounds, c->walk_need[p]) : c->tune.walk_rounds;
  return SMR_OK;
}
```

sortmerna_amd/csrc/smr_tuning.hpp:

```cpp
#pragma once
#include <algorithm>
#include <cstdarg>
#include <cstdint>
#include <cstdio>
#include <cstdlib>
#include <string>

namespace smr {

struct TuningLimits { uint32_t walk_k_max, cand_cap0, cand_cap_max, bloom_words_max, pool_words_min, hot_bin, hot_sub, selfcheck_cases; };

struct Tuning {
  int sw_packed = 2;
  bool seed_exact = false;
  int seed_shared = 1;
  uint32_t hot_min = 1024;
  uint32_t hot_bin = 0;
  uint32_t hot_sub = 0;
  bool seg_inline = true;
  int handover = 1;
  int walk_split = 1;
  uint32_t walk_rounds = 8;
  bool walk_rounds_fixed = false;
  uint32_t walk_k = 4;
  int walk_gather = 1;
  uint32_t walk_assume = 3;
  bool begins_x4 = false;
  bool pg_host = false;
  bool trace_global_rows = false;
  uint32_t cand_bloom = 128;
  uint32_t ccap = 0;
  uint64_t pool_words = 0;
  uint64_t cigar_words = 0;
  uint32_t sw_selfcheck = 0;
  bool verbose = false;
  bool seed_debug = false;
  bool walk_debug = false;
  bool debug_phases = false;
};

#define SMR_TUNING_TABLE(X)                                                                                                              \
  X(SMR_SW_PACKED, sw_packed) X(SMR_SEED_EXACT, seed_exact) X(SMR_SEED_SHARED, seed_shared) X(SMR_SEED_DEDUP, hot_min)                   \
  X(SMR_SEED_HOT_BIN, hot_bin) X(SMR_SEED_HOT_SUB, hot_sub) X(SMR_SEG_INLINE, seg_inline) X(SMR_HANDOVER, handover)                     \
  X(SMR_WALK_SPLIT, walk_split) X(SMR_WALK_ROUNDS, walk_rounds) X(SMR_WALK_K, walk_k) X(SMR_WALK_GATHER, walk_gather)                   \
  X(SMR_WALK_ASSUME, walk_assume) X(SMR_BEGINS_X4, begins_x4) X(SMR_PG_HOST, pg_host) X(SMR_TRACE_GLOBAL_ROWS, trace_global_rows)       \
  X(SMR_CAND_BLOOM, cand_bloom) X(SMR_PG_CAND_CAP, ccap) X(SMR_SEED_POOL_WORDS, pool_words) X(SMR_CIGAR_POOL_WORDS, cigar_words)        \
  X(SMR_SW_SELFCHECK, sw_selfcheck) X(SMR_VERBOSE, verbose) X(SMR_SEED_DEBUG, seed_debug) X(SMR_WALK_DEBUG, walk_debug)                 \
  X(SMR_DEBUG_PHASES, debug_phases)

inline Tuning read_tuning(const TuningLimits& L) {
  Tuning t;
  t.hot_bin = L.hot_bin; t.hot_sub = L.hot_sub; t.ccap = L.cand_cap0; t.sw_selfcheck = L.selfcheck_cases;
  const char* e;
  if ((e = getenv("SMR_SW_PACKED"))) t.sw_packed = atoi(e);
  if ((e = getenv("SMR_SEED_EXACT"))) t.seed_exact = atoi(e) != 0;
  if ((e = getenv("SMR_SEED_SHARED"))) t.seed_shared = atoi(e);
  if ((e = getenv("SMR_SEED_DEDUP"))) t.hot_min = (uint32_t)std::max(0, atoi(e));
  if ((e = getenv("SMR_SEED_HOT_BIN"))) t.hot_bin = (uint32_t)std::max(1, atoi(e));
  if ((e = getenv("SMR_SEED_HOT_SUB"))) t.hot_sub = (uint32_t)std::max(1, atoi(e));
  if ((e = getenv("SMR_SEG_INLINE"))) t.seg_inline = atoi(e) != 0;
  if ((e = getenv("SMR_HANDOVER"))) t.handover = atoi(e);
  if ((e = getenv("SMR_WALK_SPLIT"))) t.walk_split = atoi(e);
  if ((e = getenv("SMR_WALK_ROUNDS"))) { t.walk_rounds = (uint32_t)std::max(1, std::min(32, atoi(e))); t.walk_rounds_fixed = true; }
  if ((e = getenv("SMR_WALK_K"))) t.walk_k = (uint32_t)std::max(1, std::min((int)L.walk_k_max, atoi(e)));
  if ((e = getenv("SMR_WALK_GATHER"))) t.walk_gather = atoi(e);
  if ((e = getenv("SMR_WALK_ASSUME"))) t.walk_assume = (uint32_t)atoi(e);
  t.begins_x4 = getenv("SMR_BEGINS_X4") != nullptr;
  if ((e = getenv("SMR_PG_HOST"))) t.pg_host = atoi(e) != 0;
  t.trace_global_rows = getenv("SMR_TRACE_GLOBAL_ROWS") != nullptr;
  if ((e = getenv("SMR_CAND_BLOOM"))) { uint32_t b = 64; while (b < L.bloom_words_max && b < (uint32_t)atoi(e)) b <<= 1; t.cand_bloom = b; }
  if ((e = getenv("SMR_PG_CAND_CAP"))) t.ccap = std::min<uint32_t>(L.cand_cap_max, std::max<uint32_t>(4u, (uint32_t)atoi(e)));
  if ((e = getenv("SMR_SEED_POOL_WORDS"))) t.pool_words = std::min<uint64_t>(std::max<uint64_t>(strtoull(e, nullptr, 0), L.pool_words_min), 0x7FFFFFF0ull);
  if ((e = getenv("SMR_CIGAR_POOL_WORDS"))) t.cigar_words = std::max<uint64_t>(strtoull(e, nullptr, 10), 16);
  if ((e = getenv("SMR_SW_SELFCHECK"))) t.sw_selfcheck = (uint32_t)atoi(e);
  t.verbose = getenv("SMR_VERBOSE") != nullptr;
  t.seed_debug = getenv("SMR_SEED_DEBUG") != nullptr;
  t.walk_debug = getenv("SMR_WALK_DEBUG") != nullptr;
  t.debug_phases = getenv("SMR_DEBUG_PHASES") != nullptr;
  return t;
}

inline std::string tuning_text(const Tuning& t) {
  std::string s;
#define SMR_TUNING_LINE(name, member) s += #name "=" + std::to_string(+t.member) + "\n";
  SMR_TUNING_TABLE(SMR_TUNING_LINE)
#undef SMR_TUNING_LINE
  return s;
}

__attribute__((format(printf, 2, 3))) inline void say(const Tuning& t, const char* fmt, ...) {
  if (!t.verbose) return;
  va_list a;
  va_start(a, fmt);
  fputs("libsmr_hip: ", stderr);
  vfprintf(stderr, fmt, a);
  va_end(a);
}

inline uint32_t tuning_host_threads(uint32_t cap) { const char* e = getenv("SMR_HOST_THREADS"); return e ? std::min<uint32_t>(cap, (uint32_t)std::max(1, atoi(e))) : cap; }
inline uint32_t tuning_load_threads(uint32_t dflt) { const char* e = getenv("SMR_LOAD_THREADS"); return e ? std::min<uint32_t>(256, std::max(1, atoi(e))) : dflt; }
inline bool tuning_ib_timing() { return getenv("SMR_IB_TIMING") != nullptr; }

}
```

sortmerna_amd/csrc/smr_walk.hpp:

```cpp
#pragma once

namespace smr {

#define WK_MAX 15u
__host__ __device__ __forceinline__ uint32_t walk_tasks_per_read(uint32_t nlist, unsigned long long cap, uint32_t k0, int round) {
  if (round == 0) return k0;
  const unsigned long long q = nlist ? cap / nlist : (unsigned long long)WK_MAX;
  return (uint32_t)(q < k0 ? k0 : (q > WK_MAX ? WK_MAX : q));
}
#define WK_MAX_ROWS 256u
#define WK_MAX_POS 128u
#ifndef WK_CLAIM
#define WK_CLAIM 24u
#endif
enum { WC_NLIST = 0, WC_CLAIM = 16, WC_NTASK = 32, WC_NTASK2 = 48, WC_STRIDE = 64 };

struct WTask {
  uint32_t r, max_ref;
  uint64_t rf_start;
  uint32_t ars, head;
  uint16_t aq, m, nref;
  uint16_t flags;
};
struct WState {
  uint32_t k, it, ms_lo, ms_hi, begin_ref, begin_read;
  int32_t best;
  uint32_t bits;
  uint32_t cells;
};
#define WS_NK(bits) (((bits) >> 8) & 15u)

__global__ void __launch_bounds__(1024) k_wlist(DReads rd, uint8_t* __restrict__ marks, const uint2* __restrict__ mrec, uint32_t max_rows, uint2* __restrict__ list0,
                                                uint32_t* __restrict__ slow, unsigned long long* __restrict__ wc0, unsigned long long* __restrict__ n_slow, unsigned long long* census, int gather) {
  const uint32_t i = blockIdx.x * blockDim.x + threadIdx.x;
  const bool mk = i < rd.n && marks[i] == 1;
  const bool fast = mk && mrec && (mrec[i].x != NONE || (mrec[i].y - 1u < WK_MAX_POS && gather)) && rd.len[i] <= max_rows;
  const uint32_t o = block_append(&wc0[WC_NLIST], fast);
  if (fast) { list0[o] = make_uint2(i, NONE); marks[i] = 0; }
  const uint32_t o2 = block_append(n_slow, mk && !fast);
  if (mk && !fast) slow[o2] = i;
  if (census) {
    const uint32_t np = (mk && !fast && mrec) ? mrec[i].y : 0u;
    const bool s = mk && !fast;
    const int cls = !s ? -1 : np == 0xFFFFFFFFu ? 5 : np <= 64u ? 0 : np <= 128u ? 1 : np <= 256u ? 2 : np <= 512u ? 3 : 4;
    for (int q = 0; q < 6; q++) { const unsigned long long m = __ballot(cls == q); if (m && (threadIdx.x & 63u) == 0) atomicAdd(&census[q], (unsigned long long)__popcll(m)); }
  }
}

__global__ void __launch_bounds__(256) k_cand_route(uint32_t n, const uint8_t* __restrict__ marks, const uint2* __restrict__ mrec, const uint2* __restrict__ list0,
                                                    const unsigned long long* __restrict__ wc0, int stage, uint8_t* __restrict__ route) {
  const uint32_t i = blockIdx.x * blockDim.x + threadIdx.x;
  if (stage == 0) {
    if (i < n && i < (uint32_t)wc0[WC_NLIST]) { const uint32_t r = list0[i].x; if (r < n) route[r] |= (uint8_t)(mrec[r].x != NONE ? SMR_ROUTE_RECORD : SMR_ROUTE_GATHER); }
  } else if (i < n && marks[i] == (stage == 1 ? 1u : 2u)) route[i] |= (uint8_t)(stage == 1 ? SMR_ROUTE_CHAIN : SMR_ROUTE_EXT);
}

__device__ __forceinline__ int dpp_quad_ror1(int v) { return __builtin_amdgcn_update_dpp(v, v, 0x93 , 0xF, 0xF, false); }
template <int U> __device__ __forceinline__ int dpp_quad_bcast(int v) { return __builtin_amdgcn_update_dpp(v, v, U * 0x55 , 0xF, 0xF, false); }
__device__ __forceinline__ unsigned long long quad_max_u64(unsigned long long v) {
  for (int d = 2; d > 0; d >>= 1) { const unsigned long long o = __shfl_xor(v, d, 64); v = o > v ? o : v; }
  return v;
}

struct __attribute__((aligned(4))) Sw16W3 { uint32_t a, b, c; };
struct __attribute__((aligned(4))) Sw16W2 { uint32_t a, b; };
template <int R, bool HASN, bool KEYS>
__device__ __forceinline__ SwRes sw_quad16(const uint32_t* __restrict__ rec, uint32_t len, uint32_t reversed, int m, int aq, const uint8_t* __restrict__ ref, int n,
                                           int match, int mismatch, int scoreN, int go, int ge, int dir) {
  const int gl = lane_id() & 3;
  const pk16 GE = pk_splat(ge), GO = pk_splat(go), ZERO = pk_splat(0);
  const uint32_t TN = (((uint32_t)(scoreN + go)) & 0xFFFFu) * 0x00010001u;
  uint32_t tlo[R], thi[R];
  pk16 Y[R], E[R];
  uint32_t key[KEYS ? R : 1];
  pk16 hmax = ZERO;
  const uint32_t t_mm = ((uint32_t)(mismatch + go) & 0xFFu) * 0x01010101u, t_x = ((uint32_t)(mismatch + go) ^ (uint32_t)(match + go)) & 0xFFu,
                 t_n = ((uint32_t)(scoreN + go) & 0xFFu) * 0x01010101u;
  const uint32_t cw = (len + 15u) >> 4, cwm = max(cw, 1u) - 1u, awm = max((len + 31u) >> 5, 1u) - 1u;
  const int sgn = reversed ? -dir : dir;
  uint32_t cwd[2][3], awd[2][2];
  int pa[2], cw0[2], aw0[2];
#pragma unroll
  for (int hf = 0; hf < 2; hf++) {
    const int row0 = (gl + 4 * hf) * R, nv = max(1, min(R, m - row0));
    const int k0 = aq + dir * row0;
    pa[hf] = reversed ? (int)len - 1 - k0 : k0;
    const int pmin = max(0, min(pa[hf], pa[hf] + sgn * (nv - 1)));
    cw0[hf] = (int)min((uint32_t)pmin >> 4, cwm); aw0[hf] = (int)min((uint32_t)pmin >> 5, awm);
    const Sw16W3 c3 = *reinterpret_cast<const Sw16W3*>(rec + cw0[hf]);
    const Sw16W2 a2 = *reinterpret_cast<const Sw16W2*>(rec + cw + aw0[hf]);
    cwd[hf][0] = c3.a; cwd[hf][1] = c3.b; cwd[hf][2] = c3.c; awd[hf][0] = a2.a; awd[hf][1] = a2.b;
  }
#pragma unroll
  for (int j = 0; j < R; j++) {
    uint32_t t2[2];
#pragma unroll
    for (int hf = 0; hf < 2; hf++) {
      const int row = (gl + 4 * hf) * R + j;
      uint32_t t = 0;
      if (row < m) {
        const int ph = pa[hf] + sgn * j;
        const int wi = (ph >> 4) - cw0[hf], ai = (ph >> 5) - aw0[hf];
        const uint32_t wd = wi == 0 ? cwd[hf][0] : wi == 1 ? cwd[hf][1] : cwd[hf][2];
        const uint32_t ad = ai == 0 ? awd[hf][0] : awd[hf][1];
        uint32_t c = (wd >> ((ph & 15) * 2)) & 3u;
        if (reversed) c = 3u - c;
        if ((ad >> (ph & 31)) & 1u) c = 4u;
        t = c == 4u ? t_n : t_mm ^ (t_x << (8u * c));
      }
      t2[hf] = t;
    }
    tlo[j] = t2[0]; thi[j] = t2[1];
    Y[j] = pk_splat(-go); E[j] = ZERO; if (KEYS) key[j] = 0;
  }
  int steps = m > 0 ? n + (m + R - 1) / R - 1 : 0;
  for (int d = 32; d > 0; d >>= 1) steps = max(steps, __shfl_xor(steps, d, 64));
#ifdef SMR_SW16_NOSTEPS
  steps = min(steps, 4);
#endif
  uint32_t lastY = pk_bits(pk_splat(-go)), lastF = 0, selcur = PK_SEL_NONE * 0x00010001u;
  pk16 diag0 = pk_splat(-go);
  const uint32_t in_y = (uint32_t)(-go) & 0xFFFFu;
  uint32_t xlo = ((uint32_t)(0x3FFF + gl) << 1) | 1u;
  const bool first = gl == 0;
  uint32_t wnext = gl < n ? pk_sel_of(ref[dir * gl]) : PK_SEL_NONE;
#define SW16_STEP(U)                                                                                                        \
  {                                                                                                                         \
    const uint32_t win = (uint32_t)dpp_quad_bcast<U>((int)wcur);                                                            \
    const uint32_t rY = (uint32_t)dpp_quad_ror1((int)lastY), rF = (uint32_t)dpp_quad_ror1((int)lastF), rS = (uint32_t)dpp_quad_ror1((int)selcur); \
    const pk16 upY = pk_from(first ? ((rY << 16) | in_y) : rY);                                                             \
    const pk16 upF = pk_from(first ? (rF << 16) : rF);                                                                      \
    selcur = first ? ((rS << 16) | win | 0x00040000u) : rS;                                                                 \
    uint32_t nmask = 0;                                                                                                     \
    if (HASN) nmask = ((selcur >> 8) & 0x00010001u) * 0xFFFFu;                                                              \
    const uint32_t xhi = xlo + 7u;                                                                                          \
    pk16 diag = diag0, uy = upY, uf = upF;                                                                                  \
    _Pragma("unroll") for (int j = 0; j < R; j++) {                                                                         \
      uint32_t T = perm_b32(thi[j], tlo[j], selcur);                                                                        \
      if (HASN) T = (T & ~nmask) | (TN & nmask);                                                                            \
      const pk16 a = pk_add(diag, pk_from(T));                                                                              \
      const pk16 e = pk_max(pk_subs_u(E[j], GE), Y[j]);       \
      const pk16 f = pk_max(pk_sub(uf, GE), uy);                                                                            \
      const pk16 h = pk_max(pk_max(a, e), f);                            \
      diag = Y[j];                                                                                                          \
      const pk16 y = pk_sub(h, GO);                                                                                         \
      Y[j] = y; E[j] = e;                                                                                                   \
      if (KEYS) { const uint32_t hu = pk_bits(h); key[j] = max(key[j], max((hu << 16) | xlo, (hu & 0xFFFF0000u) | xhi)); }  \
      else hmax = pk_max(hmax, h);                                                                                          \
      uy = y; uf = f;                                                                                                       \
    }                                                                                                                       \
    diag0 = upY;                                                                                                            \
    lastY = pk_bits(uy); lastF = pk_bits(uf);                                                                               \
    xlo -= 2u;                                                                                                              \
  }
  for (int t = 0; t < steps; t += 4) {
    const uint32_t wcur = wnext;
    const int cq = t + 4 + gl;
    wnext = cq < n ? pk_sel_of(ref[dir * cq]) : PK_SEL_NONE;
    SW16_STEP(0) SW16_STEP(1) SW16_STEP(2) SW16_STEP(3)
  }
#undef SW16_STEP
  if (!KEYS) {
    const uint32_t hb = pk_bits(hmax);
    int sc = max((int)(hb & 0xFFFFu), (int)(hb >> 16));
    for (int d = 2; d > 0; d >>= 1) sc = max(sc, __shfl_xor(sc, d, 64));
    SwRes rs; rs.score = sc; rs.end_ref = -2; rs.end_read = 0xFFFF;
    return rs;
  }
  int bestH = 0, bestcol = 0x1FFFFF, bestrow = 0x1FFFFF;
#pragma unroll
  for (int j = 0; j < R; j++) {
    const int h = (int)(key[j] >> 16);
    const int hf = (key[j] & 1u) ? 0 : 1;
    const int col = 0x3FFF - (int)((key[j] >> 1) & 0x7FFFu);
    const int row = (gl + 4 * hf) * R + j;
    if (h > bestH || (h == bestH && h > 0 && (col < bestcol || (col == bestcol && row < bestrow)))) { bestH = h; bestcol = col; bestrow = row; }
  }
  unsigned long long k64 = bestH > 0 ? (((unsigned long long)bestH << 42) | ((unsigned long long)(0x1FFFFF - bestcol) << 21) |
                                        (unsigned long long)(0x1FFFFF - bestrow)) : 0ull;
  k64 = quad_max_u64(k64);
  SwRes rr;
  if (k64 == 0) { rr.score = 0; rr.end_ref = -1; rr.end_read = m - 1; return rr; }
  rr.score = (int)(k64 >> 42);
  rr.end_ref = 0x1FFFFF - (int)((k64 >> 21) & 0x1FFFFF);
  rr.end_read = 0x1FFFFF - (int)(k64 & 0x1FFFFF);
  return rr;
}

__device__ __forceinline__ uint2 wres_pack(const SwRes& s) { return make_uint2((uint32_t)s.score, s.end_ref < -1 ? 0xFFFFFFFFu : ((uint32_t)(s.end_ref + 1) << 16) | ((uint32_t)s.end_read & 0xFFFFu)); }
__device__ __forceinline__ SwRes wres_unpack(const uint2 v) {
  SwRes s; s.score = (int)v.x;
  if (v.y == 0xFFFFFFFFu) { s.end_ref = -2; s.end_read = 0; }
  else { s.end_ref = (int)(v.y >> 16) - 1; s.end_read = (int)(v.y & 0xFFFFu); }
  return s;
}

#ifndef SW16_WAVES
#define SW16_WAVES(R) ((R) <= 13 ? 4 : (R) <= 19 ? 3 : 2)
#endif
template <int R>
__global__ void __launch_bounds__(64, SW16_WAVES(R)) k_sw16(DReads rd, DIndex ix, DParams P, const WTask* __restrict__ tk, const uint32_t* __restrict__ tidx1,
                                                           const uint32_t* __restrict__ tidx2, const unsigned long long* __restrict__ wc, uint2* __restrict__ res) {
  const int lane = lane_id(), g = lane >> 2, gl = lane & 3;
  const uint32_t ntA = (uint32_t)wc[WC_NTASK], ntB = (uint32_t)wc[WC_NTASK2];
  const uint32_t npassA = (ntA + 15u) / 16u, npass = npassA + (ntB + 15u) / 16u;
  auto slot_of = [&](uint32_t p) -> uint32_t {
    const bool keys = p < npassA;
    const uint32_t ti = (keys ? p : p - npassA) * 16u + (uint32_t)g;
    return (p < npass && ti < (keys ? ntA : ntB)) ? (keys ? tidx1 : tidx2)[ti] : NONE;
  };
  uint32_t slot_next = slot_of(blockIdx.x);
  for (uint32_t p = blockIdx.x; p < npass; p += gridDim.x) {
    const bool keys = p < npassA;
    const uint32_t ti = (keys ? p : p - npassA) * 16u + (uint32_t)g;
    const uint32_t* const tidx = keys ? tidx1 : tidx2;
    const uint32_t slot = slot_next;
    const bool have = slot != NONE;
    int m = 0, n = 0, aq = 0, dir = 1;
    uint32_t len = 0, reversed = 0;
    const uint32_t* rec = rd.words;
    const uint8_t* ref = ix.ref_seq;
    if (have) {
      const WTask t = tk[slot];
      m = t.m; n = t.nref; aq = t.aq; reversed = t.flags & 1u; dir = (t.flags & 2u) ? -1 : 1;
      len = rd.len[t.r]; rec = rd.words + rd.rec_off[t.r];
      ref = ix.ref_seq + t.rf_start;
    }
    slot_next = slot_of(p + gridDim.x);
    int nn = n;
    for (int d = 32; d > 0; d >>= 1) nn = max(nn, __shfl_xor(nn, d, 64));
    bool hn = false;
    if (ix.ref_any_n) {
      const int nm = max(n, 1) - 1;
      for (int q0 = gl; q0 < nn; q0 += 32) {
        uint8_t b[8];
#pragma unroll
        for (int i = 0; i < 8; i++) b[i] = ref[dir * min(q0 + 4 * i, nm)];
#pragma unroll
        for (int i = 0; i < 8; i++) hn |= (q0 + 4 * i < n) && b[i] == 4;
      }
    }
    SwRes s;
    const bool hasn = __any(hn);
#define SW16_ARGS rec, len, reversed, m, aq, ref, n, P.match, P.mismatch, P.score_N, P.gap_open, P.gap_ext, dir
    if (keys) { if (hasn) s = sw_quad16<R, true, true>(SW16_ARGS); else s = sw_quad16<R, false, true>(SW16_ARGS); }
    else { if (hasn) s = sw_quad16<R, true, false>(SW16_ARGS); else s = sw_quad16<R, false, false>(SW16_ARGS); }
#undef SW16_ARGS
    if (have && gl == 0) res[tidx[ti]] = wres_pack(s);
  }
}

#ifndef SMR_WALK_WAVES_PER_SIMD
#define SMR_WALK_WAVES_PER_SIMD 5
#endif
template <bool FINAL>
__global__ void __launch_bounds__(64, FINAL ? 3 : SMR_WALK_WAVES_PER_SIMD)
k_walk(DReads rd, DIndex ix, DParams P, int pass, int is_last_strand, RState* __restrict__ work, AlignRec* __restrict__ work_aln, RWork* __restrict__ rw,
       unsigned long long* __restrict__ ctr, const uint2* __restrict__ mrec, const uint32_t* __restrict__ mpool, const uint32_t* __restrict__ pool,
       const uint2* __restrict__ list, const WState* __restrict__ ws_prev, const WTask* __restrict__ tk_prev, const uint2* __restrict__ res_prev,
       WState* __restrict__ ws_cur, WTask* __restrict__ tk_cur, uint32_t* __restrict__ tidx, uint32_t* __restrict__ tidx2, unsigned long long* __restrict__ wc,
       uint32_t K0, unsigned long long task_cap, int round, uint32_t lds_ml, uint32_t lds_rf, uint32_t assume_min) {
  SMR_DYN_LDS(unsigned char, lds_raw);
  __shared__ unsigned long long l_pairs[WK_MAX_POS];
  __shared__ uint2 l_cand[64];
  __shared__ unsigned long long l_cref[64];
  __shared__ uint32_t l_clen[64];
  __shared__ uint32_t l_hkey[256], l_hcnt[256];
  __shared__ unsigned long long l_stage[WK_MAX_POS];
  __shared__ WTask s_ctk[WK_MAX];
  __shared__ uint2 s_cres[WK_MAX];
  __shared__ uint32_t s_tix[WK_CLAIM * WK_MAX];
  __shared__ uint32_t s_next, s_tbase;
  const int lane = lane_id();
  const uint32_t nlist = (uint32_t)wc[WC_NLIST];
  const uint32_t K = walk_tasks_per_read(nlist, task_cap, K0, round);
  const uint32_t Kp = round > 0 ? walk_tasks_per_read((uint32_t)(wc - WC_STRIDE)[WC_NLIST], task_cap, K0, round - 1) : K0;
  unsigned long long n_fwd = 0, n_cells = 0, n_spec = 0, n_spec_used = 0, n_newhit = 0;
#ifdef SMR_WALK_PHASES
  unsigned long long wph[7] = {0, 0, 0, 0, 0, 0, 0}, wlast = clock64();
#define WPH(i) { const unsigned long long tn_ = clock64(); wph[i] += tn_ - wlast; wlast = tn_; }
#else
#define WPH(i)
#endif
  const uint32_t claim = max(1u, min(WK_CLAIM, nlist / (gridDim.x * 4u)));
  for (;;) {
    __syncthreads();
    if (lane == 0) s_next = (uint32_t)atomicAdd(&wc[WC_CLAIM], (unsigned long long)claim);
    __syncthreads();
    const uint32_t chunk_base = s_next;
    if (chunk_base >= nlist) break;
    const uint32_t chunk_n = min(claim, nlist - chunk_base);
    uint32_t ntix = 0, ntix2 = 0;
    uint32_t c_r = 0, c_prev = NONE, c_len = 0;
    uint2 c_mr = make_uint2(NONE, 0u);
    if ((uint32_t)lane < chunk_n) { const uint2 le = list[chunk_base + lane]; c_r = le.x; c_prev = le.y; c_mr = mrec[c_r]; c_len = rd.len[c_r]; }
    for (uint32_t ci = 0; ci < chunk_n; ci++) {
      const uint32_t e = chunk_base + ci;
      const uint32_t r = (uint32_t)__builtin_amdgcn_readlane((int)c_r, (int)ci), prev = (uint32_t)__builtin_amdgcn_readlane((int)c_prev, (int)ci);
      const uint32_t len = (uint32_t)__builtin_amdgcn_readlane((int)c_len, (int)ci);
      const uint2 mr = make_uint2((uint32_t)__builtin_amdgcn_readlane((int)c_mr.x, (int)ci), (uint32_t)__builtin_amdgcn_readlane((int)c_mr.y, (int)ci));
      RWork w = rw[r];
      RState st = work[r];
      const uint32_t* rec = FINAL ? rd.words + rd.rec_off[r] : nullptr;
      WState ps; ps.bits = 0;
      if (prev != NONE) ps = ws_prev[prev];
      uint32_t live_bits = 0;
      if (w.strand_active && w.search && w.pass_n == (uint32_t)pass && mr.y - 1u < WK_MAX_POS) {
        WPH(0)
        const uint32_t npos = mr.y;
        uint32_t seq[2] = {0, 0}, pos[2] = {0, 0}, win[2] = {0, 0};
        const bool valid[2] = {(uint32_t)lane < npos, (uint32_t)lane + 64u < npos};
        __syncthreads();
        if (mr.x != NONE) {
          const uint32_t* rp = mpool + mr.x;
          if (valid[0]) { seq[0] = rp[lane]; pos[0] = rp[npos + lane]; win[0] = rp[2u * npos + lane]; }
        } else {
          uint32_t* const g_hp = (uint32_t*)l_stage;
          uint32_t* const g_lo = g_hp + 65, * const g_wn = g_lo + 64;
          const uint32_t nh = w.hit_total;
          uint32_t lo = 0, ln = 0;
          if ((uint32_t)lane < nh) {
            const uint32_t h = (uint32_t)lane, c0 = w.blk_cnt[0], c1 = w.blk_cnt[1];
            const uint32_t at = h < c0 ? w.blk_off[0] + 2 * h : h - c0 < c1 ? w.blk_off[1] + 2 * (h - c0) : w.blk_off[2] + 2 * (h - c0 - c1);
            const uint32_t id = pool[at];
            g_wn[lane] = pool[at + 1];
            lo = id + 1u; ln = ix.pos_arr[id].x;
          }
          uint32_t tot;
          const uint32_t ex = wave_excl_scan_u32(ln, tot);
          if ((uint32_t)lane < nh) { g_hp[lane] = ex; g_lo[lane] = lo; }
          if (lane == 0) g_hp[nh] = tot;
          __syncthreads();
#pragma unroll
          for (int q = 0; q < 2; q++) if (valid[q]) {
            const uint32_t p = (uint32_t)lane + 64u * q;
            uint32_t h = 0;
            for (uint32_t step = 32; step > 0; step >>= 1) { const uint32_t t = h + step; if (t < nh && g_hp[t] <= p) h = t; }
            const uint2 pa = ix.pos_arr[g_lo[h] + (p - g_hp[h])];
            seq[q] = pa.y; pos[q] = pa.x; win[q] = g_wn[h];
          }
          __syncthreads();
        }
#pragma unroll
        for (int q = 0; q < 4; q++) { l_hkey[lane + 64 * q] = 0xFFFFFFFFu; l_hcnt[lane + 64 * q] = 0; }
        __syncthreads();
        uint32_t slot[2] = {0, 0};
#pragma unroll
        for (int q = 0; q < 2; q++) if (valid[q]) {
          uint32_t sl = (seq[q] * 0x9E3779B1u) >> 24;
          for (;;) { const uint32_t o = atomicCAS(&l_hkey[sl], 0xFFFFFFFFu, seq[q]); if (o == 0xFFFFFFFFu || o == seq[q]) break; sl = (sl + 1u) & 255u; }
          atomicAdd(&l_hcnt[sl], 1u);
          slot[q] = sl;
        }
        __threadfence_block();
        __syncthreads();
        const bool mem0 = valid[0] && (int)l_hcnt[slot[0]] >= P.num_seeds, mem1 = valid[1] && (int)l_hcnt[slot[1]] >= P.num_seeds;
        const unsigned long long mm0 = __ballot(mem0), mm1 = __ballot(mem1);
        const uint32_t tot0 = (uint32_t)__popcll(mm0), total = tot0 + (uint32_t)__popcll(mm1);
        const unsigned long long ltm = (1ull << lane) - 1ull;
        if (mem0) l_stage[__popcll(mm0 & ltm)] = ((unsigned long long)slot[0] << 48) | ((unsigned long long)pos[0] << 16) | (unsigned long long)(win[0] & 0xFFFFu);
        if (mem1) l_stage[tot0 + (uint32_t)__popcll(mm1 & ltm)] = ((unsigned long long)slot[1] << 48) | ((unsigned long long)pos[1] << 16) | (unsigned long long)(win[1] & 0xFFFFu);
        __syncthreads();
        if (total > 64) wave_sort_u64(l_stage, total);
        else if (total > 1) {
          unsigned long long key = (uint32_t)lane < total ? l_stage[lane] : ~0ull;
          uint32_t np2 = 2; while (np2 < total) np2 <<= 1;
          for (uint32_t kk = 2; kk <= np2; kk <<= 1)
            for (uint32_t j = kk >> 1; j > 0; j >>= 1) {
              const unsigned long long o = __shfl_xor(key, (int)j, 64);
              const bool want_min = (((uint32_t)lane & j) == 0) == (((uint32_t)lane & kk) == 0);
              if (want_min ? o < key : key < o) key = o;
            }
          if ((uint32_t)lane < total) l_stage[lane] = key;
        }
        __syncthreads();
// ... 61 lines not shown
          wk.pending_pop = 0;
          return 1;
        };
        auto next_task = [&](Walk& wk, SwTask& tk) -> bool {
          const uint2 ce = l_cand[wk.k];
          const unsigned long long* pairs = l_pairs + (ce.y >> 8);
          const uint32_t np = ce.y & 0xFFu;
          while (wk.it != np && wk.go_on) {
            if (!wk.pending_pop) {
              wk.pending_pop = 1;
              const uint64_t end_ref_max = (uint64_t)wk.begin_ref + len - wk.begin_read - P.lnwin + 1;
              int push = 0;
              for (;;) {
                const uint32_t pi = wk.it + (uint32_t)lane;
                const bool okp = pi < np && (uint64_t)(uint32_t)(pairs[min(pi, np - 1)] >> 32) <= end_ref_max;
                const unsigned long long pm = __ballot(okp);
                const uint32_t pc = pm == ~0ull ? 64u : (uint32_t)__ffsll((long long)~pm) - 1u;
                if (pc) { wk.it += pc; wk.ms_hi = wk.it; push = 1; }
                if (pc < 64u) break;
              }
              int skip_to_pop = 0;
              if (!push && wk.is_aligned) skip_to_pop = 1;
              else wk.is_aligned = 0;
              if (!skip_to_pop && (wk.ms_hi - wk.ms_lo) >= (uint32_t)P.num_seeds) {
                uint32_t lis0;
                const uint32_t nw = wk.ms_hi - wk.ms_lo;
                uint32_t* const lisb = (uint32_t*)l_stage;
                const uint32_t nl = nw <= 64 ? wave_lis_first(pairs + wk.ms_lo, nw, lis0) : serial_lis_first(pairs + wk.ms_lo, nw, lisb, lisb + WK_MAX_POS, lis0);
                if (nl >= (uint32_t)P.min_lis) {
                  const unsigned long long pl = pairs[wk.ms_lo + lis0];
                  const uint32_t lcs_ref_start = (uint32_t)(pl >> 32), lcs_que_start = (uint32_t)pl;
                  const uint64_t reflen = l_clen[wk.k];
                  uint64_t hd = 0, tail = 0, align_ref_start = 0, align_que_start = 0, align_length = 0;
                  uint32_t edges;
                  if (P.is_as_percent) edges = (uint32_t)((P.edges / 100.0) * (double)rlen);
                  else edges = (uint32_t)P.edges;
                  if (lcs_ref_start < lcs_que_start) {
                    align_ref_start = 0; align_que_start = lcs_que_start - lcs_ref_start; hd = 0;
                    if (reflen < rlen) {
                      tail = 0;
                      if (align_que_start > (rlen - reflen)) align_length = reflen - (align_que_start - (rlen - reflen));
                      else align_length = reflen;
                    } else {
                      tail = reflen - align_ref_start - rlen;
                      if (tail > (uint64_t)(uint32_t)(edges - 1)) tail = edges;
                      align_length = rlen + hd + tail - align_que_start;
                    }
                  } else {
                    align_ref_start = lcs_ref_start - lcs_que_start; align_que_start = 0;
                    if (align_ref_start > (uint64_t)(uint32_t)(edges - 1)) hd = edges;
                    if (align_ref_start + rlen > reflen) { tail = 0; align_length = reflen - align_ref_start - hd; }
                    else {
                      tail = reflen - align_ref_start - rlen;
                      if (tail > (uint64_t)(uint32_t)(edges - 1)) tail = edges;
                      align_length = rlen + hd + tail;
                    }
                  }
                  tk.max_ref = ce.x; tk.align_ref_start = align_ref_start; tk.head = hd; tk.align_que_start = align_que_start;
                  tk.m = (int)(align_length - hd - tail); tk.nref = (int)align_length;
                  tk.rf_start = l_cref[wk.k] + align_ref_start - hd;
                  return true;
                }
              }
            }
            wk.pending_pop = 0;
            if (wk.ms_hi > wk.ms_lo) wk.ms_lo++;
            if (wk.ms_hi == wk.ms_lo) {
              if (wk.it != np) { const unsigned long long pn = pairs[wk.it]; wk.begin_ref = (uint32_t)(pn >> 32); wk.begin_read = (uint32_t)pn; }
              else break;
            } else { const unsigned long long pn = pairs[wk.ms_lo]; wk.begin_ref = (uint32_t)(pn >> 32); wk.begin_read = (uint32_t)pn; }
          }
          return false;
        };
        auto advance = [&](Walk& wk, SwTask& tk) -> int {
          for (;;) {
            if (!wk.started) {
              if (load_candidate(wk) != 1) return 0;
              wk.started = 1;
            }
            if (next_task(wk, tk)) return 1;
            wk.k++; wk.started = 0;
          }
        };
        auto put_task = [&](uint32_t j, const SwTask& t) {
          if (lane == 0) {
            WTask o; o.r = r; o.max_ref = t.max_ref; o.rf_start = t.rf_start; o.ars = (uint32_t)t.align_ref_start; o.head = (uint32_t)t.head; o.aq = (uint16_t)t.align_que_start;
            o.m = (uint16_t)t.m; o.nref = (uint16_t)t.nref; o.flags = w.reversed ? 1 : 0;
            tk_cur[(size_t)e * K + j] = o;
          }
        };
        auto task_ok = [&](const SwTask& t) -> bool { return t.m > 0 && t.nref > 0 && (uint32_t)t.m <= lds_ml && (uint32_t)t.nref <= lds_rf && (uint32_t)t.nref <= 0xFFFFu; };

        Walk R;
        int search = 1, last_aligned = 0;
        SwTask tk;
        bool have_tk = false;
        if (prev == NONE) {
          R.k = 0; R.it = 0; R.ms_lo = 0; R.ms_hi = 0; R.begin_ref = 0; R.begin_read = 0;
          R.is_aligned = 0; R.best = w.best; R.go_on = 1; R.started = 0; R.pending_pop = 0;
        } else {
          R.k = ps.k; R.it = ps.it; R.ms_lo = ps.ms_lo; R.ms_hi = ps.ms_hi; R.begin_ref = ps.begin_ref; R.begin_read = ps.begin_read; R.best = ps.best;
          R.is_aligned = (int)(ps.bits & 1u); R.go_on = (int)((ps.bits >> 1) & 1u); R.started = (int)((ps.bits >> 2) & 1u); R.pending_pop = (int)((ps.bits >> 3) & 1u);
          search = (int)((ps.bits >> 4) & 1u); last_aligned = (int)((ps.bits >> 6) & 1u);
          const WTask c0 = s_ctk[0];
          tk.max_ref = c0.max_ref; tk.rf_start = c0.rf_start; tk.align_ref_start = c0.ars; tk.head = c0.head; tk.align_que_start = c0.aq; tk.m = c0.m; tk.nref = c0.nref;
          have_tk = true;
        }
        const uint32_t max_SW_score = len * (uint32_t)P.match;
        bool live = false, rdq_staged = false, dirty = false;
        for (;;) {
          WPH(3)
          if (!have_tk) { if (advance(R, tk) != 1) break; }
          WPH(2)
          if (w.has_amb && !w.is04) { w.is04 = 1; w.aval = 4; }
          const int m = tk.m, nref = tk.nref;
          const bool sw_ok = task_ok(tk);
          if (!sw_ok && (m > 0 && nref > 0)) { if (lane == 0) atomicAdd(&ctr[C_ERR_PAIRS], 1ull); }
          SwRes fw; fw.score = 0; fw.end_ref = -1; fw.end_read = m - 1;
          if (sw_ok) {
            int ce = -1;
            if (have_tk) ce = 0;
            else for (uint32_t q = 0; q < n_prev; q++)
              if (s_ctk[q].max_ref == tk.max_ref && s_ctk[q].rf_start == tk.rf_start && (uint32_t)s_ctk[q].aq == (uint32_t)tk.align_que_start && (int)s_ctk[q].m == m && (int)s_ctk[q].nref == nref) { ce = (int)q; break; }
            if (ce >= 0) { fw = wres_unpack(s_cres[ce]); if (ce > 0) n_spec_used++; }
            else if (!FINAL) {
              const int assume = prev == NONE ? ((ncand > 0 && (l_cand[0].y & 0xFFu) >= assume_min) ? 1 : 0) : last_aligned;
              WState o; o.k = R.k; o.it = R.it; o.ms_lo = R.ms_lo; o.ms_hi = R.ms_hi; o.begin_ref = R.begin_ref; o.begin_read = R.begin_read; o.best = R.best;
              const uint32_t bits0 = (uint32_t)(R.is_aligned & 1) | ((uint32_t)(R.go_on & 1) << 1) | ((uint32_t)(R.started & 1) << 2) | ((uint32_t)(R.pending_pop & 1) << 3) | ((uint32_t)(search & 1) << 4) |
                                     ((uint32_t)(last_aligned & 1) << 6);
              uint32_t nk = 1, cells = (uint32_t)m * (uint32_t)nref;
              put_task(0, tk);
              R.is_aligned = assume;
              bool ended = false;
              while (nk < K) {
                SwTask t2;
                if (advance(R, t2) != 1) { ended = true; break; }
                if (!task_ok(t2)) break;
                put_task(nk, t2); nk++; cells += (uint32_t)t2.m * (uint32_t)t2.nref;
                R.is_aligned = assume;
              }
              n_spec += nk - 1;
              o.bits = bits0 | ((ended && !assume) ? 32u : 0u) | (nk << 8); o.cells = cells;
              if (lane == 0) ws_cur[e] = o;
              live_bits = nk << 8;
              if (assume) { for (uint32_t q = lane; q < nk; q += 64) s_tix[ntix + q] = e * K + q; ntix += nk; }
              else { for (uint32_t q = lane; q < nk; q += 64) s_tix[WK_CLAIM * WK_MAX - 1u - (ntix2 + q)] = e * K + q; ntix2 += nk; }
              live = true;
              WPH(4)
              break;
            } else {
              uint8_t* const rdq = lds_raw; uint8_t* const rfq = lds_raw + lds_ml;
              __syncthreads();
              if (!rdq_staged) { for (uint32_t q = lane; q < len; q += 64) rdq[q] = (uint8_t)read_nt(rec, len, q, w.reversed, 4u); rdq_staged = true; }
              for (int q = lane; q < nref; q += 64) rfq[q] = ix.ref_seq[tk.rf_start + q];
              __syncthreads();
              fw = sw_wave(rdq, m, (int)tk.align_que_start, 1, rfq, nref, 0, 1, nullptr, P.match, P.mismatch, P.score_N, P.gap_open, P.gap_ext, P.sw_mode);
              __syncthreads();
            }
            n_fwd++; n_cells += (unsigned long long)m * nref;
          }
          have_tk = false;
          const int score1 = fw.score > 65535 ? 65535 : fw.score;
          R.is_aligned = (sw_ok && (uint32_t)score1 > P.minimal_score);
          last_aligned = R.is_aligned;
          if (R.is_aligned) {
            dirty = true;
            if ((uint32_t)score1 == max_SW_score) ++st.max_SW_count;
            AlignRec al;
            al.ref_begin1 = (int32_t)(tk.align_ref_start - tk.head);
            const bool no_end = fw.end_ref < -1;
            al.ref_end1 = (no_end ? nref - 1 : fw.end_ref) + (int32_t)(tk.align_ref_start - tk.head);
            al.read_begin1 = (int32_t)tk.align_que_start;
            al.read_end1 = (no_end ? m - 1 : fw.end_read) + (int32_t)tk.align_que_start;
            al.readlen = len; al.ref_num = tk.max_ref;
            al.index_num = (uint16_t)P.index_num; al.part = (uint16_t)P.part;
            al.strand = (uint8_t)!w.reversed; al.score1 = (uint16_t)score1;
            al.has_cigar = no_end ? 3 : 2; al.cigar_off = 0; al.cigar_len = 0;
            AlignRec* slots = work_aln + (size_t)r * P.slots;
            if (!st.is_hit) {
              st.is_hit = 1;
              n_newhit++;
            }
            if (P.num_alignments == 0 || !P.is_best || (P.is_best && st.n_align < P.num_alignments)) {
              if (st.n_align < P.slots) { if (lane == 0) slots[st.n_align] = al; st.n_align++; w.is_new_hit = 1; }
              else { if (lane == 0) atomicAdd(&ctr[C_ERR_SLOTS], 1ull); }
            } else if (P.is_best && st.n_align == P.num_alignments) {
              __syncthreads();
              if (slots[st.min_index].score1 < (uint16_t)score1) {
                if (P.num_alignments > 1 && st.max_index == 0 && st.min_index == 0) {
                  uint32_t mn = 0, mx = 0;
                  for (uint32_t q = 1; q < st.n_align; q++) { if (slots[q].score1 < slots[mn].score1) mn = q; if (slots[q].score1 > slots[mx].score1) mx = q; }
                  st.min_index = mn; st.max_index = mx;
                }
                const uint32_t mn = st.min_index, mx = st.max_index;
                const uint16_t mx_score = slots[mx].score1;
                __syncthreads();
                if (lane == 0) slots[mn] = al;
                __threadfence_block();
                __syncthreads();
                w.is_new_hit = 1;
                if ((uint16_t)score1 > (mn == mx ? (uint16_t)score1 : mx_score) && st.n_align > 1) {
                  st.max_index = mn;
                  uint32_t m2 = 0;
                  for (uint32_t q = 1; q < st.n_align; q++) if (slots[q].score1 < slots[m2].score1) m2 = q;
                  st.min_index = m2;
                }
              }
            }
            __syncthreads();
            if (P.num_alignments > 0) {
              if (P.is_best) { if (P.num_alignments == st.max_SW_count) R.go_on = 0; }
              else if (P.num_alignments == st.n_align) R.go_on = 0;
            }
            search = 0;
          }
        }
        if (live) { if (dirty && lane == 0) { work[r] = st; rw[r] = w; } }
        else { w.best = R.best; chain_finish_read(P, is_last_strand, r, st, w, search, lane == 0, work, rw); }
        WPH(5)
      }
      if (!live_bits && lane == 0) ws_cur[e].bits = 0;
    }
    if (!FINAL && ntix) {
      __syncthreads();
      if (lane == 0) s_tbase = (uint32_t)atomicAdd(&wc[WC_NTASK], (unsigned long long)ntix);
      __syncthreads();
      const uint32_t tb = s_tbase;
      for (uint32_t q = lane; q < ntix; q += 64) tidx[tb + q] = s_tix[q];
    }
    if (!FINAL && ntix2) {
      __syncthreads();
      if (lane == 0) s_tbase = (uint32_t)atomicAdd(&wc[WC_NTASK2], (unsigned long long)ntix2);
      __syncthreads();
      const uint32_t tb = s_tbase;
      for (uint32_t q = lane; q < ntix2; q += 64) tidx2[tb + q] = s_tix[WK_CLAIM * WK_MAX - 1u - q];
    }
    WPH(6)
  }
  if (lane == 0) {
    if (n_fwd) ctr_add(ctr, C_SW_FWD, n_fwd);
    if (n_cells) ctr_add(ctr, C_SW_CELLS, n_cells);
    if (n_spec) atomicAdd(&ctr[C_SW_SPEC], n_spec);
    if (n_spec_used) atomicAdd(&ctr[C_SW_SPEC_USED], n_spec_used);
    if (n_newhit) { atomicAdd(&ctr[C_NUM_ALIGNED], n_newhit); atomicAdd(&ctr[C_PER_DB + P.index_num], n_newhit); }
#ifdef SMR_WALK_PHASES
    for (int q = 0; q < 7; q++) if (wph[q]) atomicAdd(&ctr[C_SHARDS + (blockIdx.x & (C_NSHARD - 1)) * C_SHARD_W + C_SHARD_PH + q], wph[q]);
#endif
  }
#undef WPH
}

__global__ void __launch_bounds__(1024) k_wnext(DParams P, int is_last_strand, RState* __restrict__ work, RWork* __restrict__ rw, unsigned long long* __restrict__ ctr,
                                                const uint2* __restrict__ list, const WState* __restrict__ ws, const uint2* __restrict__ res, uint2* __restrict__ list_next,
                                                const unsigned long long* __restrict__ wc, unsigned long long* __restrict__ wc_next, uint32_t K0, unsigned long long task_cap, int round) {
  const uint32_t n = (uint32_t)wc[WC_NLIST];
  const uint32_t K = walk_tasks_per_read(n, task_cap, K0, round);
  unsigned long long n_fwd = 0, n_cells = 0, n_used = 0;
  for (uint32_t base = blockIdx.x * blockDim.x; base < n; base += gridDim.x * blockDim.x) {
    const uint32_t e = base + threadIdx.x;
    bool live = false;
    uint32_t r = 0;
    if (e < n) {
      const WState s = ws[e];
      const uint32_t nk = WS_NK(s.bits);
      if (nk > 0) {
        live = true;
        r = list[e].x;
        if (s.bits & 32u) {
          bool any = false;
          for (uint32_t j = 0; j < nk; j++) { const uint32_t sc = res[(size_t)e * K + j].x; any |= (sc > 65535u ? 65535u : sc) > P.minimal_score; }
          if (!any) {
            RWork w = rw[r];
            RState st = work[r];
            if (w.has_amb && !w.is04) { w.is04 = 1; w.aval = 4; }
            w.best = s.best;
            n_fwd += nk; n_cells += s.cells; n_used += nk - 1;
            chain_finish_read(P, is_last_strand, r, st, w, (int)((s.bits >> 4) & 1u), true, work, rw);
            live = false;
          }
        }
      }
    }
    const uint32_t o = block_append(&wc_next[WC_NLIST], live);
    if (live) list_next[o] = make_uint2(r, e);
  }
  for (int d = 32; d > 0; d >>= 1) { n_fwd += __shfl_xor(n_fwd, d, 64); n_cells += __shfl_xor(n_cells, d, 64); n_used += __shfl_xor(n_used, d, 64); }
  if (lane_id() == 0) {
    if (n_fwd) ctr_add(ctr, C_SW_FWD, n_fwd);
    if (n_cells) ctr_add(ctr, C_SW_CELLS, n_cells);
    if (n_used) atomicAdd(&ctr[C_SW_SPEC_USED], n_used);
  }
}

__global__ void __launch_bounds__(1024) k_begins_prep(DIndex ix, uint32_t slots, const uint32_t* __restrict__ tasks, const unsigned long long* __restrict__ n_tasks_p, const AlignRec* __restrict__ work_aln,
                                                      int stage, WTask* __restrict__ tk, uint32_t* __restrict__ tidx, unsigned long long* __restrict__ wc) {
  const uint32_t n_tasks = (uint32_t)*n_tasks_p;
  for (uint32_t base = blockIdx.x * blockDim.x; base < n_tasks; base += gridDim.x * blockDim.x) {
    const uint32_t t = base + threadIdx.x;
    bool take = false;
    if (t < n_tasks) {
      const AlignRec al = work_aln[tasks[t]];
      take = stage == 0 ? al.has_cigar == 3 : al.has_cigar >= 2;
      if (take) {
        WTask o;
        o.r = tasks[t] / slots; o.max_ref = al.ref_num; o.ars = 0; o.head = 0;
        o.m = (uint16_t)(al.read_end1 - al.read_begin1 + 1); o.nref = (uint16_t)(al.ref_end1 - al.ref_begin1 + 1);
        if (stage == 0) { o.aq = (uint16_t)al.read_begin1; o.rf_start = ix.ref_off[al.ref_num] + (uint64_t)al.ref_begin1; o.flags = al.strand ? 0 : 1; }
        else { o.aq = (uint16_t)al.read_end1; o.rf_start = ix.ref_off[al.ref_num] + (uint64_t)al.ref_end1; o.flags = (al.strand ? 0 : 1) | 2; }
        tk[t] = o;
      }
    }
    const uint32_t p = block_append(&wc[WC_NTASK], take);
    if (take) tidx[p] = t;
  }
}
__global__ void __launch_bounds__(256) k_begins_apply(const uint32_t* __restrict__ tasks, const unsigned long long* __restrict__ n_tasks_p, AlignRec* __restrict__ work_aln, int stage,
                                                      const WTask* __restrict__ tk, const uint2* __restrict__ res, unsigned long long* __restrict__ ctr) {
  const uint32_t n_tasks = (uint32_t)*n_tasks_p;
  unsigned long long n_rev = 0, n_cells = 0;
  for (uint32_t t = blockIdx.x * blockDim.x + threadIdx.x; t < n_tasks; t += gridDim.x * blockDim.x) {
    AlignRec* const al = work_aln + tasks[t];
    const uint32_t hc = al->has_cigar;
    if (stage == 0 ? hc != 3 : hc < 2) continue;
    const SwRes s = wres_unpack(res[t]);
    if (stage == 0) { al->ref_end1 = al->ref_begin1 + s.end_ref; al->read_end1 = al->read_begin1 + s.end_read; al->has_cigar = 2; }
    else { al->ref_begin1 = al->ref_end1 - s.end_ref; al->read_begin1 = al->read_end1 - s.end_read; al->has_cigar = 0; n_rev++; n_cells += (unsigned long long)tk[t].m * tk[t].nref; }
  }
  for (int d = 32; d > 0; d >>= 1) { n_rev += __shfl_xor(n_rev, d, 64); n_cells += __shfl_xor(n_cells, d, 64); }
  if (lane_id() == 0) { if (n_rev) ctr_add(ctr, C_SW_REV, n_rev); if (n_cells) ctr_add(ctr, C_SW_CELLS, n_cells); }
}

}
// ... 1 lines not shown
```

sortmerna_amd/engine.py:

```python
import ctypes as C

import numpy as np

from . import capi


OTU_GROUP = np.dtype([("ref_num", np.uint32), ("n_reads", np.uint32), ("off", np.uint64)])


class SmrError(RuntimeError):
    pass


def default_params(**kw):
    p = capi.Params()
    capi.load().smr_params_default(C.byref(p))
    for k, v in kw.items():
        if k == "skiplengths":
            for i in range(3):
                p.skiplengths[i] = v[i]
        else:
            if not hasattr(p, k):
                raise AttributeError(k)
            setattr(p, k, v)
# ... 188 lines not shown
    err = C.create_string_buffer(512)
    rc = L.smr_index_pigeonhole(index.h, C.byref(pg), C.byref(npg), C.byref(r3), C.byref(nr3), err, 512)
    if rc != 0:
        raise SmrError("smr_index_pigeonhole: %s (rc=%d)" % (err.value.decode(), rc))
    return np.ctypeslib.as_array(pg, shape=(npg.value,)), np.ctypeslib.as_array(r3, shape=(nr3.value,))


ROUTE_RECORD, ROUTE_GATHER, ROUTE_CHAIN, ROUTE_EXT = 1, 2, 4, 8
FASTX_VIEW = 1
FASTX_KEEP = 2


class Engine:

    def __init__(self, device=0):
        self.L = capi.load()
        h = C.c_void_p()
        err = C.create_string_buffer(512)
        rc = self.L.smr_create(device, C.byref(h), err, 512)
        if rc != 0:
            raise SmrError("smr_create: %s (rc=%d)" % (err.value.decode(), rc))
        self.h = h
        self.n_reads = 0
        self._batch_n = {}
        self._cur = 0

    def _chk(self, rc, what):
        if rc != 0:
            raise SmrError("%s: %s (rc=%d)" % (what, self.L.smr_last_error(self.h).decode(), rc))

    def upload_index(self, index, slot=0):
        self._chk(self.L.smr_index_upload(self.h, index.h, slot), "smr_index_upload")

    def check_device_index(self, index, slot=0):
        self._chk(self.L.smr_index_check_device(self.h, slot, index.h), "smr_index_check_device")

    def unload_index(self, slot=0):
        self._chk(self.L.smr_index_unload(self.h, slot), "smr_index_unload")

    def select_batch(self, batch):
        self._chk(self.L.smr_batch_select(self.h, batch), "smr_batch_select")
        self.n_reads = self._batch_n.get(batch, 0)
        self._cur = batch

    def set_seed_mode(self, exact_counters):
        self._chk(self.L.smr_set_seed_mode(self.h, int(bool(exact_counters))), "smr_set_seed_mode")

    def sw_mode(self, set_to=-1):
        return self.L.smr_sw_mode(self.h, set_to)

    def walk_rounds(self):
        out = (C.c_uint32 * 3)()
        self._chk(self.L.smr_walk_rounds(self.h, out), "smr_walk_rounds")
        return list(out)

    def sw_selfcheck(self, n_cases=256, seed=1, max_len=700):
        bad = C.c_uint64()
        self._chk(self.L.smr_sw_selfcheck(self.h, n_cases, seed, max_len, C.byref(bad)), "smr_sw_selfcheck")
        return bad.value

    def ssw_batch(self, reads, refs, match=2, mismatch=-3, score_N=-3, gap_open=5, gap_ext=2, filters=0, mode=1):
        import numpy as np
        n = len(reads)
        ro = np.zeros(n + 1, dtype=np.uint64); fo = np.zeros(n + 1, dtype=np.uint64)
        ro[1:] = np.cumsum([len(x) for x in reads]); fo[1:] = np.cumsum([len(x) for x in refs])
        rb = np.frombuffer(b"".join(reads) + b"\0", dtype=np.uint8).copy(); fb = np.frombuffer(b"".join(refs) + b"\0", dtype=np.uint8).copy()
        out = np.zeros((n, 5), dtype=np.int32)
        self._chk(self.L.smr_ssw_batch(self.h, n, rb.ctypes.data, ro.ctypes.data, fb.ctypes.data, fo.ctypes.data, match, mismatch, score_N,
                                       gap_open, gap_ext, filters, mode, out.ctypes.data), "smr_ssw_batch")
        return out

    SW16_TASK = np.dtype([("read", "<u4"), ("win_off", "<u4"), ("aq", "<u2"), ("m", "<u2"), ("nref", "<u2"), ("reversed", "u1"), ("list_b", "u1")])

    def sw16_batch(self, tasks, ref, rows, match=2, mismatch=-3, score_N=-3, gap_open=5, gap_ext=2, filters=0, blocks=0, force_any_n=False):
        n = len(tasks)
        t = np.zeros(max(n, 1), dtype=self.SW16_TASK)
        for i, (r, aq, m, rev, wo, nref, lb) in enumerate(tasks):
            t[i] = (r, wo, aq, m, nref, rev, lb)
        rf = np.frombuffer(bytes(ref) + b"\0", dtype=np.uint8).copy()
        out = np.zeros((max(n, 1), 5), dtype=np.int32)
        self._chk(self.L.smr_sw16_batch(self.h, n, t.ctypes.data, rf.ctypes.data, len(ref), int(bool(force_any_n)), match, mismatch, score_N, gap_open, gap_ext,
                                        filters, rows, blocks, out.ctypes.data), "smr_sw16_batch")
        return out[:n]

    def sw16_launches(self):
        out = (C.c_uint64 * 8)()
        self._chk(self.L.smr_sw16_launches(self.h, out), "smr_sw16_launches")
        return dict(zip((13, 19, 26, 32), out[:4])), dict(zip((13, 19, 26, 32), out[4:]))

    def sw_long_rows(self, m):
        return self.L.smr_sw_long_rows(int(m))

    def cigar_batch(self, reads, refs, scores, match=2, mismatch=-3, score_N=-3, gap_open=5, gap_ext=2):
        n = len(reads)
        ro = np.zeros(n + 1, dtype=np.uint64); fo = np.zeros(n + 1, dtype=np.uint64)
        ro[1:] = np.cumsum([len(x) for x in reads]); fo[1:] = np.cumsum([len(x) for x in refs])
        rb = np.frombuffer(b"".join(reads) + b"\0", dtype=np.uint8).copy(); fb = np.frombuffer(b"".join(refs) + b"\0", dtype=np.uint8).copy()
        sc = np.asarray(scores, dtype=np.uint16)
        off = np.zeros(n + 1, dtype=np.uint64)
        cap = int(ro[-1] + fo[-1]) + 4 * n + 16
        out = np.zeros(cap, dtype=np.uint32)
        self._chk(self.L.smr_cigar_batch(self.h, n, rb.ctypes.data, ro.ctypes.data, fb.ctypes.data, fo.ctypes.data, sc.ctypes.data, match, mismatch, score_N,
                                         gap_open, gap_ext, out.ctypes.data, cap, off.ctypes.data), "smr_cigar_batch")
        return [out[int(off[i]):int(off[i + 1])].copy() for i in range(n)]

    def upload_reads(self, reads, max_alignments_per_read=1):
        self._chk(self.L.smr_reads_upload(self.h, reads.h, max_alignments_per_read), "smr_reads_upload")
        self.n_reads = reads.count
        self._batch_n[self._cur] = reads.count

    def upload_reads_batch(self, batch, reads, max_alignments_per_read=1):
        self._chk(self.L.smr_reads_upload_batch(self.h, batch, reads.h, max_alignments_per_read), "smr_reads_upload_batch")
        self._batch_n[batch] = reads.count

    def upload_fastx(self, data_or_path, max_alignments_per_read=1, batch=None, view=False, keep=False):
        h = C.c_void_p()
        flags = (FASTX_VIEW if view else 0) | (FASTX_KEEP if keep else 0)
        keep = None
        if isinstance(data_or_path, str):
            if batch is not None:
                raise SmrError("upload_fastx: batch= takes bytes (read the file first)")
            err = C.create_string_buffer(512)
            rc, what = self.L.smr_reads_upload_fastx_file(self.h, data_or_path.encode(), max_alignments_per_read, flags, C.byref(h), err, 512), "smr_reads_upload_fastx_file"
        else:
            keep = C.create_string_buffer(bytes(data_or_path), len(data_or_path) + 1)
            if batch is None:
                rc, what = self.L.smr_reads_upload_fastx(self.h, keep, len(data_or_path), max_alignments_per_read, flags, C.byref(h)), "smr_reads_upload_fastx"
            else:
                rc, what = self.L.smr_reads_upload_fastx_batch(self.h, batch, keep, len(data_or_path), max_alignments_per_read, flags, C.byref(h)), "smr_reads_upload_fastx_batch"
        self._chk(rc, what)
        reads = Reads(h, keep)
        if batch is None:
            self.n_reads = reads.count
        self._batch_n[self._cur if batch is None else batch] = reads.count
        return reads

    def fastx_info(self):
        info = (C.c_uint64 * 4)()
        self._chk(self.L.smr_fastx_info(self.h, info), "smr_fastx_info")
        return tuple(int(x) for x in info)

    def fastx_times(self):
        ms = (C.c_double * 5)()
        self._chk(self.L.smr_fastx_times(self.h, ms), "smr_fastx_times")
        return dict(zip(("h2d", "lines", "records", "pack", "d2h"), (float(x) for x in ms)))

    def fastx_split(self, layout=0, mates=None, paired_in=False, paired_out=False, out2=False, sout=False, aligned=True, other=True, hit=None):
        o = capi.FxSplitOpts(int(layout), int(bool(paired_in)), int(bool(paired_out)), int(bool(out2)), int(bool(sout)), int(bool(aligned)), int(bool(other)))
        hb = None if hit is None else (C.c_uint8 * max(len(hit), 1))(*[1 if x else 0 for x in hit])
        m = -1 if mates is None else int(mates)
        off = (C.c_uint64 * 9)()
        need = C.c_uint64(0)
        self._chk(self.L.smr_fastx_split(self.h, m, C.byref(o), hb, None, 0, off, C.byref(need)), "smr_fastx_split")
        buf = (C.c_uint8 * max(need.value, 1))()
        if need.value:
            self._chk(self.L.smr_fastx_split(self.h, m, C.byref(o), hb, buf, need.value, off, C.byref(need)), "smr_fastx_split")
        raw = bytes(buf)
        return [raw[off[k]:off[k + 1]] for k in range(8)]

    def fastx_split_times(self):
        ms = (C.c_double * 4)()
        self._chk(self.L.smr_fastx_split_times(self.h, ms), "smr_fastx_split_times")
        return dict(zip(("measure", "scans", "copy", "d2h"), (float(x) for x in ms)))

    def rows_part(self, slot, params, index, sam=True, blast=False, cols="", lam=0.0, K=0.0, full_ref=0, full_read=0):
        o = capi.RowsOpts()
# ... 319 lines not shown
```

Before: 54.58 million.

## Score speculative look-ahead SW tasks on a column prefix with adaptive fallback

Speculative look-ahead Smith-Waterman tasks for reads expected to align can now be scored over only a prefix of the reference window. The prefix result is packed as a lower and upper bound. The walk accepts the lower bound when it already decides the outcome against the current best-N minimum score, and otherwise redoes the full task. Prefix tasks go through a separate third index list, and device counters track how many were decided versus redone. A host-side adapter turns prefix tasks off for a number of parts when too many are redone, at the cost of an extra sync per part to read those counters.

Result: faster. 55.69 million, median of 6 (+2.0%).

```diff
diff --git a/include/smr_hip.h b/include/smr_hip.h
--- a/include/smr_hip.h
+++ b/include/smr_hip.h
@@ -214,6 +214,14 @@
 } smr_sw16_task;
 int smr_sw16_batch(smr_ctx*, uint32_t n_tasks, const smr_sw16_task* tasks, const uint8_t* ref, uint64_t ref_len, int force_any_n,
                    int match, int mismatch, int score_N, int gap_open, int gap_ext, uint32_t filters, int rows, uint32_t blocks, int32_t* out);
+typedef struct {
+  uint32_t read, win_off;
+  uint16_t aq, m, nref, cols;
+  uint8_t reversed, pad_[3];
+} smr_sw16_prefix_task;
+int smr_sw16_prefix_batch(smr_ctx*, uint32_t n_tasks, const smr_sw16_prefix_task* tasks, const uint8_t* ref, uint64_t ref_len, int force_any_n,
+                          int match, int mismatch, int score_N, int gap_open, int gap_ext, int rows, uint32_t blocks, int32_t* out);
+int smr_walk_prefix_stats(smr_ctx*, uint64_t out[8]);
 int smr_sw16_launches(const smr_ctx*, uint64_t out[8]);
 int smr_cigar_batch(smr_ctx*, uint32_t n_pairs, const uint8_t* reads, const uint64_t* read_off, const uint8_t* refs, const uint64_t* ref_off,
                     const uint16_t* scores, int match, int mismatch, int score_N, int gap_open, int gap_ext,
diff --git a/sortmerna_amd/capi.py b/sortmerna_amd/capi.py
--- a/sortmerna_amd/capi.py
+++ b/sortmerna_amd/capi.py
@@ -76,7 +76,7 @@
     "smr_reads_digest", "smr_reads_count", "smr_reads_total_len", "smr_reads_min_len", "smr_reads_max_len", "smr_create", "smr_device_count", "smr_destroy",
     "smr_last_error", "smr_tuning_text", "smr_index_upload", "smr_index_check_device", "smr_index_pigeonhole", "smr_seed_tuples_fetch", "smr_seed_pool_info", "smr_cand_info_enable", "smr_cand_info", "smr_cand_routes", "smr_index_unload", "smr_batch_select", "smr_set_seed_mode", "smr_reads_upload", "smr_reads_upload_batch", "smr_reads_upload_fastx", "smr_reads_upload_fastx_batch", "smr_reads_upload_fastx_file", "smr_fastx_info", "smr_fastx_times", "smr_fastx_split", "smr_fastx_split_times", "smr_rows_part", "smr_rows_times", "smr_rows_fmt_batch", "smr_pairwise_part", "smr_pairwise_times", "smr_state_reset", "smr_align_part",
     "smr_traceback", "smr_counters", "smr_counters_device", "smr_state_import", "smr_state_export", "smr_counters_import", "smr_results_fetch", "smr_result_record", "smr_result_record_batch", "smr_counters_accumulate",
-    "smr_result_is_hit", "smr_seed_scan", "smr_seed_hits_fetch", "smr_sw_selfcheck", "smr_sw_mode", "smr_walk_rounds", "smr_ssw_batch", "smr_sw16_batch", "smr_sw16_launches", "smr_sw_long_rows", "smr_cigar_batch", "smr_idcov_part", "smr_idcov_counters", "smr_idcov_counters_device", "smr_idcov_batch", "smr_prof_reset", "smr_prof_get", "smr_prof_kernels", "smr_refstats_corrected", "smr_report_open",
+    "smr_result_is_hit", "smr_seed_scan", "smr_seed_hits_fetch", "smr_sw_selfcheck", "smr_sw_mode", "smr_walk_rounds", "smr_ssw_batch", "smr_sw16_batch", "smr_sw16_prefix_batch", "smr_walk_prefix_stats", "smr_sw16_launches", "smr_sw_long_rows", "smr_cigar_batch", "smr_idcov_part", "smr_idcov_counters", "smr_idcov_counters_device", "smr_idcov_batch", "smr_prof_reset", "smr_prof_get", "smr_prof_kernels", "smr_refstats_corrected", "smr_report_open",
     "smr_report_set_db", "smr_report_set_part", "smr_report_add", "smr_report_add_pair", "smr_report_add_fastx", "smr_report_skip_fastx", "smr_report_add_rows", "smr_report_skip_rows", "smr_report_add_pairwise", "smr_report_skip_pairwise", "smr_report_set_cmdline", "smr_report_otu_count", "smr_report_otu_merge", "smr_report_close", "smr_report_last_error",
     "smr_summary_write", "smr_readstats_record", "smr_readstats_key",
 ]
@@ -208,6 +208,10 @@
     L.smr_ssw_batch.argtypes = [vp, u32, vp, vp, vp, vp, i32, i32, i32, i32, i32, u32, i32, vp]
     L.smr_sw16_batch.restype = i32
     L.smr_sw16_batch.argtypes = [vp, u32, vp, vp, u64, i32, i32, i32, i32, i32, i32, u32, i32, u32, vp]
+    L.smr_sw16_prefix_batch.restype = i32
+    L.smr_sw16_prefix_batch.argtypes = [vp, u32, vp, vp, u64, i32, i32, i32, i32, i32, i32, i32, u32, vp]
+    L.smr_walk_prefix_stats.restype = i32
+    L.smr_walk_prefix_stats.argtypes = [vp, C.POINTER(u64)]
     L.smr_sw16_launches.restype = i32
     L.smr_sw16_launches.argtypes = [vp, C.POINTER(u64)]
     L.smr_sw_long_rows.restype = i32
diff --git a/sortmerna_amd/csrc/smr_engine.hip b/sortmerna_amd/csrc/smr_engine.hip
--- a/sortmerna_amd/csrc/smr_engine.hip
+++ b/sortmerna_amd/csrc/smr_engine.hip
@@ -187,6 +187,8 @@
   size_t walk_lds_attr = 0, pg_lds_attr = 0, search_lds_attr = 0;
   uint64_t sw16_launches[8] = {};
   uint32_t walk_need[3] = {0, 0, 0};
+  DevBuf<unsigned long long> d_wpstat;
+  bool pfx_live = true; uint32_t pfx_parts_off = 0; unsigned long long pfx_seen[2] = {0, 0};
   DevBuf<unsigned long long> d_wstat; uint32_t wstat_n = 0; int wstat_pass[8] = {}; uint32_t wstat_rm[8] = {};
   DevBuf<int> d_bound;
   DevBuf<uint32_t> d_tasks;
@@ -763,6 +765,7 @@
     if ((rc = judge_attempt(c, P, h, retry))) return rc;
     if (retry) { kp_restore(c, kp0); continue; }
     if ((rc = adapt_walk_rounds(c))) return rc;
+    if ((rc = adapt_walk_prefix(c))) return rc;
     if ((rc = launch_begins(c, di, P, plan))) return rc;
     launch(c, k_commit_part, dim3((c->b->n + 255u) / 256u), dim3(256), 0, c->b->n, P, c->b->d_saved, c->b->d_saved_aln, c->b->d_work, c->b->d_work_aln, c->b->d_rw);
     HIPCHK(c, hipGetLastError());
@@ -1039,6 +1042,7 @@
   HIPCHK(c, hipSetDevice(c->device));
   for (int k = 0; k < KP_COUNT; k++) { c->kp_ms[k] = 0; c->kp_l[k] = 0; }
   c->n_seed_shared = c->n_seed_shared_builds = 0;
+  if (c->d_wpstat) HIPCHK(c, hipMemsetAsync(c->d_wpstat, 0, WPS_N * 8, c->stream));
   for (int k = 0; k < SMR_MAX_BATCHES; k++)
     if (c->bt[k].d_ctr) {
       HIPCHK(c, hipMemsetAsync(&c->bt[k].d_ctr[C_WINDOWS], 0, 9 * 8, c->stream));
diff --git a/sortmerna_amd/csrc/smr_engine_chain.hpp b/sortmerna_amd/csrc/smr_engine_chain.hpp
--- a/sortmerna_amd/csrc/smr_engine_chain.hpp
+++ b/sortmerna_amd/csrc/smr_engine_chain.hpp
@@ -47,10 +47,10 @@
 }
 typedef decltype(&k_sw16<13>) sw16_fn;
 void launch_sw16(smr_ctx* c, int rows, int counted, uint32_t blocks, const DReads& rd, const DIndex& ix, const DParams& P, const WTask* tasks, const uint32_t* tix, const uint32_t* tix2,
-                 const unsigned long long* wc, uint2* res) {
+                 const uint32_t* tix3, const unsigned long long* wc, uint2* res) {
   static const sw16_fn K[4] = {k_sw16<13>, k_sw16<19>, k_sw16<26>, k_sw16<32>};
   const int v = rows == 13 ? 0 : rows == 19 ? 1 : rows == 26 ? 2 : 3;
-  launch(c, K[v], dim3(blocks ? blocks : (uint32_t)c->n_cu * 4u * (uint32_t)SW16_WAVES(rows)), dim3(64), 0, rd, ix, P, tasks, tix, tix2, wc, res);
+  launch(c, K[v], dim3(blocks ? blocks : (uint32_t)c->n_cu * 4u * (uint32_t)SW16_WAVES(rows)), dim3(64), 0, rd, ix, P, tasks, tix, tix2, tix3, wc, res);
   if (counted >= 0) c->sw16_launches[counted + v]++;
 }
 
@@ -74,6 +74,24 @@
     c->walk_need[p] = std::min(c->tune.walk_rounds, need[p] >= prev ? need[p] : prev - std::max(1u, (prev - need[p]) / 2u));
   }
   c->wstat_n = 0;
+  return SMR_OK;
+}
+
+#define WALK_PREFIX_RETRY 64u
+#define WALK_PREFIX_MIN_SEEN 64ull
+int adapt_walk_prefix(smr_ctx* c) {
+  if (!c->tune.walk_prefix || !c->d_wpstat) return SMR_OK;
+  if (!c->pfx_live) { if (++c->pfx_parts_off >= WALK_PREFIX_RETRY) { c->pfx_live = true; c->pfx_parts_off = 0; } return SMR_OK; }
+  unsigned long long h[WPS_N];
+  HIPCHK(c, hipMemcpyAsync(h, c->d_wpstat, sizeof h, hipMemcpyDeviceToHost, c->stream));
+  HIPCHK(c, hipStreamSynchronize(c->stream));
+  if (h[WPS_DECIDED] < c->pfx_seen[0] || h[WPS_REDONE] < c->pfx_seen[1]) c->pfx_seen[0] = c->pfx_seen[1] = 0;
+  const unsigned long long dec = h[WPS_DECIDED] - c->pfx_seen[0], redo = h[WPS_REDONE] - c->pfx_seen[1];
+  c->pfx_seen[0] = h[WPS_DECIDED]; c->pfx_seen[1] = h[WPS_REDONE];
+  if (dec + redo >= WALK_PREFIX_MIN_SEEN && dec < 2 * redo) {
+    c->pfx_live = false; c->pfx_parts_off = 0;
+    say(c->tune, "prefix tasks off for %u parts: %llu intervals decided, %llu undecided in the last part\n", WALK_PREFIX_RETRY, dec, redo);
+  }
   return SMR_OK;
 }
 
@@ -102,11 +120,12 @@
     if (c->walk_cap < n || c->walk_kcap < WK) {
       for (int q = 0; q < 2; q++)
         if ((rc = c->d_wlist[q].alloc(c, n)) || (rc = c->d_wstate[q].alloc(c, n)) || (rc = c->d_wtask[q].alloc(c, n * WK)) || (rc = c->d_wres[q].alloc(c, n * WK))) return rc;
-      if ((rc = c->d_wtidx.alloc(c, 2 * n * WK)) || (rc = c->d_wslow.alloc(c, n))) return rc;
+      if ((rc = c->d_wtidx.alloc(c, 3 * n * WK)) || (rc = c->d_wslow.alloc(c, n))) return rc;
       c->walk_cap = n; c->walk_kcap = WK;
     }
     if ((rc = c->d_wctr.reserve(c, (size_t)(RMX + 2) * WC_STRIDE)) || (rc = c->d_wstat.reserve(c, (size_t)8 * 32))) return rc;
     HIPCHK(c, hipMemsetAsync(c->d_wctr, 0, (size_t)(RMX + 2) * WC_STRIDE * 8, c->stream));
+    if (!c->d_wpstat) { if ((rc = c->d_wpstat.alloc(c, WPS_N))) return rc; HIPCHK(c, hipMemsetAsync(c->d_wpstat, 0, WPS_N * 8, c->stream)); }
     if ((rc = raise_lds_limit(c, c->walk_lds_attr, (size_t)wml + rq, 64 * 1024, k_walk<true>))) return rc;
   }
   const size_t n_tix = (size_t)c->walk_cap * c->walk_kcap;
@@ -127,10 +146,11 @@
       ev_mark(c, KP_WALK);
       launch(c, fin ? k_walk<true> : k_walk<false>, dim3(fin ? walk_blocks * 3u / SMR_WALK_WAVES_PER_SIMD : walk_blocks), dim3(64), fin ? (size_t)wml + rq : 0,
              dreads(c), dindex(di), P, pass, is_last_strand, B.d_work, B.d_work_aln, B.d_rw, B.d_ctr, mrec, c->d_mpool, c->d_pool, c->d_wlist[cur],
-             c->d_wstate[prv], c->d_wtask[prv], c->d_wres[prv], c->d_wstate[cur], c->d_wtask[cur], c->d_wtidx, c->d_wtidx + n_tix, wc, WK, n_tix, (int)rnd, wml, rq, c->tune.walk_assume);
+             c->d_wstate[prv], c->d_wtask[prv], c->d_wres[prv], c->d_wstate[cur], c->d_wtask[cur], c->d_wtidx, c->d_wtidx + n_tix, c->d_wtidx + 2 * n_tix, wc, WK, n_tix, (int)rnd, wml, rq, c->tune.walk_assume,
+             c->pfx_live ? c->tune.walk_prefix : 0u, c->d_wpstat);
       if (fin) continue;
       ev_mark(c, KP_SW16);
-      launch_sw16(c, plan.rows, 0, 0, dreads(c), dindex(di), P, c->d_wtask[cur], c->d_wtidx, c->d_wtidx + n_tix, wc, c->d_wres[cur]);
+      launch_sw16(c, plan.rows, 0, 0, dreads(c), dindex(di), P, c->d_wtask[cur], c->d_wtidx, c->d_wtidx + n_tix, c->d_wtidx + 2 * n_tix, wc, c->d_wres[cur]);
       ev_mark(c, KP_WNEXT);
       launch(c, k_wnext, dim3((uint32_t)c->n_cu * 2u), dim3(1024), 0, P, is_last_strand, B.d_work, B.d_rw, B.d_ctr, c->d_wlist[cur], c->d_wstate[cur],
              c->d_wres[cur], c->d_wlist[prv], wc, wc + WC_STRIDE, WK, n_tix, (int)rnd);
@@ -145,8 +165,13 @@
       HIPCHK(c, hipStreamSynchronize(c->stream));
       { const unsigned long long* q = &h[(size_t)(RMX + 1) * WC_STRIDE];
         fprintf(stderr, "libsmr_hip: walk rounds (pass %d): slow %llu (positions <= 64 / 128 / 256 / 512 / more / > 64 hits: %llu %llu %llu %llu %llu %llu);", pass, q[0], q[8], q[9], q[10], q[11], q[12], q[13]); }
-      for (uint32_t rnd = 0; rnd < RM; rnd++) fprintf(stderr, " %llu/%llu+%llu", h[(size_t)rnd * WC_STRIDE + WC_NLIST], h[(size_t)rnd * WC_STRIDE + WC_NTASK], h[(size_t)rnd * WC_STRIDE + WC_NTASK2]);
+      for (uint32_t rnd = 0; rnd < RM; rnd++) fprintf(stderr, " %llu/%llu+%llu+%llu", h[(size_t)rnd * WC_STRIDE + WC_NLIST], h[(size_t)rnd * WC_STRIDE + WC_NTASK], h[(size_t)rnd * WC_STRIDE + WC_NTASK2], h[(size_t)rnd * WC_STRIDE + WC_NTASK3]);
       fprintf(stderr, "\n");
+      unsigned long long ps[WPS_N];
+      HIPCHK(c, hipMemcpyAsync(ps, c->d_wpstat, sizeof ps, hipMemcpyDeviceToHost, c->stream));
+      HIPCHK(c, hipStreamSynchronize(c->stream));
+      fprintf(stderr, "libsmr_hip: prefix tasks so far (SMR_WALK_PREFIX=%u): scored %llu decided %llu redone %llu; look-ahead tasks of reads expected to align under best N %llu, their cells %llu\n",
+              c->tune.walk_prefix, ps[WPS_SCORED], ps[WPS_DECIDED], ps[WPS_REDONE], ps[WPS_AHEAD], ps[WPS_AHEAD_CELLS]);
     }
   }
   ev_mark(c, KP_CHAIN);
@@ -180,7 +205,7 @@
     for (int stage = 0; stage < 2; stage++) {
       HIPCHK(c, hipMemsetAsync(c->d_wctr, 0, (size_t)WC_STRIDE * 8, c->stream));
       launch(c, k_begins_prep, dim3((uint32_t)c->n_cu * 2u), dim3(1024), 0, dindex(di), B.slots, c->d_tasks, &B.d_ctr[C_BEGIN_N], B.d_work_aln, stage, c->d_wtask[0], c->d_wtidx, c->d_wctr);
-      launch_sw16(c, plan.rows, 4, 0, dreads(c), dindex(di), P, c->d_wtask[0], c->d_wtidx, c->d_wtidx + task_cap, c->d_wctr, c->d_wres[0]);
+      launch_sw16(c, plan.rows, 4, 0, dreads(c), dindex(di), P, c->d_wtask[0], c->d_wtidx, c->d_wtidx + task_cap, c->d_wtidx + 2 * task_cap, c->d_wctr, c->d_wres[0]);
       launch(c, k_begins_apply, dim3((uint32_t)c->n_cu * 4u), dim3(256), 0, c->d_tasks, &B.d_ctr[C_BEGIN_N], B.d_work_aln, stage, c->d_wtask[0], c->d_wres[0], B.d_ctr);
     }
   } else
diff --git a/sortmerna_amd/csrc/smr_engine_swseam.hpp b/sortmerna_amd/csrc/smr_engine_swseam.hpp
--- a/sortmerna_amd/csrc/smr_engine_swseam.hpp
+++ b/sortmerna_amd/csrc/smr_engine_swseam.hpp
@@ -265,7 +265,7 @@
   if (!ib.empty()) HIPCHK(c, hipMemcpyAsync(d_ib, ib.data(), ib.size() * 4, hipMemcpyHostToDevice, c->stream));
   HIPCHK(c, hipMemcpyAsync(d_wc, wc, sizeof wc, hipMemcpyHostToDevice, c->stream));
   HIPCHK(c, hipMemsetAsync(d_res, 0xEE, (size_t)n_tasks * sizeof(uint2), c->stream));
-  launch_sw16(c, rows, -1, blocks, dreads(c), ix, P, d_tk, d_ia, d_ib, d_wc, d_res);
+  launch_sw16(c, rows, -1, blocks, dreads(c), ix, P, d_tk, d_ia, d_ib, d_ib, d_wc, d_res);
   HIPCHK(c, hipGetLastError());
   HIPCHK(c, hipMemcpyAsync(res.data(), d_res, (size_t)n_tasks * sizeof(uint2), hipMemcpyDeviceToHost, c->stream));
   HIPCHK(c, hipStreamSynchronize(c->stream));
@@ -299,7 +299,7 @@
   HIPCHK(c, hipMemcpyAsync(d_ia, beg.data(), beg.size() * 4, hipMemcpyHostToDevice, c->stream));
   HIPCHK(c, hipMemcpyAsync(d_wc, wc, sizeof wc, hipMemcpyHostToDevice, c->stream));
   HIPCHK(c, hipMemsetAsync(d_res, 0xEE, (size_t)n_tasks * sizeof(uint2), c->stream));
-  launch_sw16(c, rows, -1, blocks, dreads(c), ix, P, d_tk, d_ia, d_ib, d_wc, d_res);
+  launch_sw16(c, rows, -1, blocks, dreads(c), ix, P, d_tk, d_ia, d_ib, d_ib, d_wc, d_res);
   HIPCHK(c, hipGetLastError());
   HIPCHK(c, hipMemcpyAsync(res.data(), d_res, (size_t)n_tasks * sizeof(uint2), hipMemcpyDeviceToHost, c->stream));
   HIPCHK(c, hipStreamSynchronize(c->stream));
@@ -312,6 +312,84 @@
   return SMR_OK;
 }
 
+extern "C" int smr_sw16_prefix_batch(smr_ctx* c, uint32_t n_tasks, const smr_sw16_prefix_task* tasks, const uint8_t* ref, uint64_t ref_len, int force_any_n,
+                                     int match, int mismatch, int score_N, int gap_open, int gap_ext, int rows, uint32_t blocks, int32_t* out) {
+  if (!c || (n_tasks && (!tasks || !out)) || (ref_len && !ref)) return SMR_ERR_ARG;
+  if (rows != 13 && rows != 19 && rows != 26 && rows != 32) { set_err(c, "smr_sw16_prefix_batch: rows must be 13, 19, 26 or 32"); return SMR_ERR_ARG; }
+  if (blocks > 65536u) { set_err(c, "smr_sw16_prefix_batch: at most 65536 blocks"); return SMR_ERR_ARG; }
+  if (match <= 0 || match > 127 || mismatch > 0 || mismatch < -127 || score_N < -127 || gap_open < 0 || gap_open > 255 || gap_ext < 0 || gap_ext > 255) { set_err(c, "smr_sw16_prefix_batch: bad scoring options"); return SMR_ERR_ARG; }
+  if (const char* why = scheme_unsupported(mismatch, score_N, gap_open, gap_ext)) { set_err(c, why); return SMR_ERR_ARG; }
+  if (!c->b->used || !c->b->d_words) { set_err(c, "smr_sw16_prefix_batch: no reads uploaded into the selected batch"); return SMR_ERR_STATE; }
+  (void)hipSetDevice(c->device);
+  const uint32_t n_reads = c->b->n;
+  std::vector<uint32_t> len(n_reads);
+  if (n_reads) HIPCHK(c, hipMemcpyAsync(len.data(), c->b->d_len, (size_t)n_reads * 4, hipMemcpyDeviceToHost, c->stream));
+  HIPCHK(c, hipStreamSynchronize(c->stream));
+  std::vector<WTask> tk(std::max<uint32_t>(n_tasks, 1));
+  std::vector<uint32_t> ic(std::max<uint32_t>(n_tasks, 1));
+  for (uint32_t i = 0; i < n_tasks; i++) {
+    const smr_sw16_prefix_task& t = tasks[i];
+    const char* why = nullptr;
+    if (t.read >= n_reads) why = "read index outside the batch";
+    else if (t.m == 0 || t.nref == 0) why = "empty span or window";
+    else if (t.m > WK_MAX_ROWS || (int)t.m > 8 * rows) why = "span longer than the kernel takes (8 x rows, at most WK_MAX_ROWS)";
+    else if ((uint64_t)t.aq + t.m > len[t.read]) why = "rows outside the read";
+    else if ((uint64_t)t.win_off + t.nref > ref_len) why = "window outside the reference letters";
+    else if (!sw_pk_fits((int)t.m, (int)t.nref, match, mismatch, score_N, gap_open)) why = "numbers outside the packed representation (sw_pk_fits)";
+    else if (t.reversed > 1) why = "reversed must be 0 or 1";
+    else if (t.cols == 0) why = "cols must not be 0";
+    else if (t.cols % 4u) why = "cols must be a multiple of 4 (the kernel's period)";
+    else if (t.cols >= t.nref) why = "cols must be less than nref";
+    if (why) { set_err(c, std::string("smr_sw16_prefix_batch: task ") + std::to_string(i) + ": " + why); return SMR_ERR_ARG; }
+    WTask o;
+    memset(&o, 0, sizeof o);
+    o.r = t.read; o.rf_start = t.win_off; o.aq = t.aq; o.m = t.m; o.nref = t.nref; o.flags = (uint16_t)((t.reversed ? 1u : 0u) | t.cols);
+    tk[i] = o; ic[i] = i;
+  }
+  if (n_tasks == 0) return SMR_OK;
+  DevPool pool;
+  IB_GET(d_ref, uint8_t, ref_len + 8); IB_GET(d_tk, WTask, n_tasks); IB_GET(d_ic, uint32_t, n_tasks);
+  IB_GET(d_wc, unsigned long long, WC_STRIDE); IB_GET(d_res, uint2, n_tasks);
+  HIPCHK(c, hipMemsetAsync(d_ref, 0, ref_len + 8, c->stream));
+  if (ref_len) HIPCHK(c, hipMemcpyAsync(d_ref, ref, ref_len, hipMemcpyHostToDevice, c->stream));
+  DIndex ix;
+  memset(&ix, 0, sizeof ix);
+  ix.ref_seq = d_ref;
+  ix.ref_any_n = (force_any_n || (ref_len && memchr(ref, 4, ref_len))) ? 1u : 0u;
+  DParams P;
+  memset(&P, 0, sizeof P);
+  P.match = match; P.mismatch = mismatch; P.score_N = score_N; P.gap_open = gap_open; P.gap_ext = gap_ext; P.sw_mode = c->sw_mode;
+  unsigned long long wc[WC_STRIDE] = {};
+  std::vector<uint2> res(n_tasks);
+  wc[WC_NTASK3] = n_tasks;
+  HIPCHK(c, hipMemcpyAsync(d_tk, tk.data(), (size_t)n_tasks * sizeof(WTask), hipMemcpyHostToDevice, c->stream));
+  HIPCHK(c, hipMemcpyAsync(d_ic, ic.data(), (size_t)n_tasks * 4, hipMemcpyHostToDevice, c->stream));
+  HIPCHK(c, hipMemcpyAsync(d_wc, wc, sizeof wc, hipMemcpyHostToDevice, c->stream));
+  HIPCHK(c, hipMemsetAsync(d_res, 0xEE, (size_t)n_tasks * sizeof(uint2), c->stream));
+  launch_sw16(c, rows, -1, blocks, dreads(c), ix, P, d_tk, d_ic, d_ic, d_ic, d_wc, d_res);
+  HIPCHK(c, hipGetLastError());
+  HIPCHK(c, hipMemcpyAsync(res.data(), d_res, (size_t)n_tasks * sizeof(uint2), hipMemcpyDeviceToHost, c->stream));
+  HIPCHK(c, hipStreamSynchronize(c->stream));
+  for (uint32_t i = 0; i < n_tasks; i++) {
+    if (res[i].y != WRES_PREFIX) { set_err(c, "smr_sw16_prefix_batch: a prefix task came back without an interval"); return SMR_ERR_DEVICE; }
+    out[2 * (size_t)i] = (int32_t)(res[i].x & 0xFFFFu); out[2 * (size_t)i + 1] = (int32_t)(res[i].x >> 16);
+  }
+  return SMR_OK;
+}
+
+extern "C" int smr_walk_prefix_stats(smr_ctx* c, uint64_t out[8]) {
+  if (!c || !out) return SMR_ERR_ARG;
+  unsigned long long h[WPS_N] = {};
+  if (c->d_wpstat) {
+    HIPCHK(c, hipSetDevice(c->device));
+    HIPCHK(c, hipMemcpyAsync(h, c->d_wpstat, sizeof h, hipMemcpyDeviceToHost, c->stream));
+    HIPCHK(c, hipStreamSynchronize(c->stream));
+  }
+  out[0] = h[WPS_SCORED]; out[1] = h[WPS_DECIDED]; out[2] = h[WPS_REDONE]; out[3] = h[WPS_SCORED] - h[WPS_DECIDED] - h[WPS_REDONE];
+  out[4] = h[WPS_AHEAD]; out[5] = h[WPS_AHEAD_CELLS]; out[6] = c->tune.walk_prefix; out[7] = c->pfx_live ? 1 : 0;
+  return SMR_OK;
+}
+
 extern "C" int smr_sw16_launches(const smr_ctx* c, uint64_t out[8]) {
   if (!c || !out) return SMR_ERR_ARG;
   for (int k = 0; k < 8; k++) out[k] = c->sw16_launches[k];
diff --git a/sortmerna_amd/csrc/smr_tuning.hpp b/sortmerna_amd/csrc/smr_tuning.hpp
--- a/sortmerna_amd/csrc/smr_tuning.hpp
+++ b/sortmerna_amd/csrc/smr_tuning.hpp
@@ -25,6 +25,7 @@
   uint32_t walk_k = 4;
   int walk_gather = 1;
   uint32_t walk_assume = 3;
+  uint32_t walk_prefix = 44;
   bool begins_x4 = false;
   bool pg_host = false;
   bool trace_global_rows = false;
@@ -65,6 +66,7 @@
   if ((e = getenv("SMR_WALK_K"))) t.walk_k = (uint32_t)std::max(1, std::min((int)L.walk_k_max, atoi(e)));
   if ((e = getenv("SMR_WALK_GATHER"))) t.walk_gather = atoi(e);
   if ((e = getenv("SMR_WALK_ASSUME"))) t.walk_assume = (uint32_t)atoi(e);
+  if ((e = getenv("SMR_WALK_PREFIX"))) t.walk_prefix = (uint32_t)std::max(0, std::min(100, atoi(e)));
   t.begins_x4 = getenv("SMR_BEGINS_X4") != nullptr;
   if ((e = getenv("SMR_PG_HOST"))) t.pg_host = atoi(e) != 0;
   t.trace_global_rows = getenv("SMR_TRACE_GLOBAL_ROWS") != nullptr;
diff --git a/sortmerna_amd/csrc/smr_walk.hpp b/sortmerna_amd/csrc/smr_walk.hpp
--- a/sortmerna_amd/csrc/smr_walk.hpp
+++ b/sortmerna_amd/csrc/smr_walk.hpp
@@ -13,7 +13,7 @@
 #ifndef WK_CLAIM
 #define WK_CLAIM 24u
 #endif
-enum { WC_NLIST = 0, WC_CLAIM = 16, WC_NTASK = 32, WC_NTASK2 = 48, WC_STRIDE = 64 };
+enum { WC_NLIST = 0, WC_CLAIM = 16, WC_NTASK = 32, WC_NTASK2 = 48, WC_NTASK3 = 64, WC_STRIDE = 80 };
 
 struct WTask {
   uint32_t r, max_ref;
@@ -22,6 +22,10 @@
   uint16_t aq, m, nref;
   uint16_t flags;
 };
+#define WT_COLS(flags) (((uint32_t)(flags) >> 2) * 4u)
+#define WRES_PREFIX 0xFFFFFFFEu
+__host__ __device__ __forceinline__ uint32_t walk_prefix_cols(uint32_t nref, uint32_t pct) { return ((nref * pct + 99u) / 100u + 3u) & ~3u; }
+enum { WPS_SCORED = 0, WPS_DECIDED, WPS_REDONE, WPS_AHEAD, WPS_AHEAD_CELLS, WPS_N = 8 };
 struct WState {
   uint32_t k, it, ms_lo, ms_hi, begin_ref, begin_read;
   int32_t best;
@@ -64,9 +68,10 @@
 
 struct __attribute__((aligned(4))) Sw16W3 { uint32_t a, b, c; };
 struct __attribute__((aligned(4))) Sw16W2 { uint32_t a, b; };
-template <int R, bool HASN, bool KEYS>
+enum { SW16_SCORE = 0, SW16_KEYS = 1, SW16_PREFIX = 2 };
+template <int R, bool HASN, int KEYS>
 __device__ __forceinline__ SwRes sw_quad16(const uint32_t* __restrict__ rec, uint32_t len, uint32_t reversed, int m, int aq, const uint8_t* __restrict__ ref, int n,
-                                           int match, int mismatch, int scoreN, int go, int ge, int dir) {
+                                           int match, int mismatch, int scoreN, int go, int ge, int dir, int rem = 0) {
   const int gl = lane_id() & 3;
   const pk16 GE = pk_splat(ge), GO = pk_splat(go), ZERO = pk_splat(0);
   const uint32_t TN = (((uint32_t)(scoreN + go)) & 0xFFFFu) * 0x00010001u;
@@ -96,9 +101,8 @@
     uint32_t t2[2];
 #pragma unroll
     for (int hf = 0; hf < 2; hf++) {
-      const int row = (gl + 4 * hf) * R + j;
       uint32_t t = 0;
-      if (row < m) {
+      if (j < m - (gl + 4 * hf) * R) {
         const int ph = pa[hf] + sgn * j;
         const int wi = (ph >> 4) - cw0[hf], ai = (ph >> 5) - aw0[hf];
         const uint32_t wd = wi == 0 ? cwd[hf][0] : wi == 1 ? cwd[hf][1] : cwd[hf][2];
@@ -145,7 +149,8 @@
       diag = Y[j];                                                                                                          \
       const pk16 y = pk_sub(h, GO);                                                                                         \
       Y[j] = y; E[j] = e;                                                                                                   \
-      if (KEYS) { const uint32_t hu = pk_bits(h); key[j] = max(key[j], max((hu << 16) | xlo, (hu & 0xFFFF0000u) | xhi)); }  \
+      if (KEYS == SW16_KEYS) { const uint32_t hu = pk_bits(h); key[j] = max(key[j], max((hu << 16) | xlo, (hu & 0xFFFF0000u) | xhi)); } \
+      else if (KEYS == SW16_PREFIX) key[j] = pk_bits(pk_max(pk_from(key[j]), h));                                           \
       else hmax = pk_max(hmax, h);                                                                                          \
       uy = y; uf = f;                                                                                                       \
     }                                                                                                                       \
@@ -160,7 +165,24 @@
     SW16_STEP(0) SW16_STEP(1) SW16_STEP(2) SW16_STEP(3)
   }
 #undef SW16_STEP
-  if (!KEYS) {
+  if (KEYS == SW16_PREFIX) {
+    const int sg = max(max(match, mismatch), max(scoreN, 0));
+    int lo = 0, hi = sg * min(m, rem);
+    const int below0 = m - 1 - gl * R;
+#pragma unroll
+    for (int j = 0; j < R; j++) {
+#pragma unroll
+      for (int hf = 0; hf < 2; hf++) {
+        const int below = below0 - 4 * R * hf - j;
+        const int mi = below >= 0 ? (int)(hf ? key[j] >> 16 : key[j] & 0xFFFFu) : 0;
+        lo = max(lo, mi); hi = max(hi, mi + sg * max(min(below, rem), 0));
+      }
+    }
+    for (int d = 2; d > 0; d >>= 1) { lo = max(lo, __shfl_xor(lo, d, 64)); hi = max(hi, __shfl_xor(hi, d, 64)); }
+    SwRes rs; rs.score = lo; rs.end_ref = -3; rs.end_read = min(max(hi, lo), 0xFFFF);
+    return rs;
+  }
+  if (KEYS == SW16_SCORE) {
     const uint32_t hb = pk_bits(hmax);
     int sc = max((int)(hb & 0xFFFFu), (int)(hb >> 16));
     for (int d = 2; d > 0; d >>= 1) sc = max(sc, __shfl_xor(sc, d, 64));
@@ -187,7 +209,10 @@
   return rr;
 }
 
-__device__ __forceinline__ uint2 wres_pack(const SwRes& s) { return make_uint2((uint32_t)s.score, s.end_ref < -1 ? 0xFFFFFFFFu : ((uint32_t)(s.end_ref + 1) << 16) | ((uint32_t)s.end_read & 0xFFFFu)); }
+__device__ __forceinline__ uint2 wres_pack(const SwRes& s) {
+  if (s.end_ref == -3) return make_uint2(((uint32_t)s.score & 0xFFFFu) | ((uint32_t)s.end_read << 16), WRES_PREFIX);
+  return make_uint2((uint32_t)s.score, s.end_ref < -1 ? 0xFFFFFFFFu : ((uint32_t)(s.end_ref + 1) << 16) | ((uint32_t)s.end_read & 0xFFFFu));
+}
 __device__ __forceinline__ SwRes wres_unpack(const uint2 v) {
   SwRes s; s.score = (int)v.x;
   if (v.y == 0xFFFFFFFFu) { s.end_ref = -2; s.end_read = 0; }
@@ -200,23 +225,25 @@
 #endif
 template <int R>
 __global__ void __launch_bounds__(64, SW16_WAVES(R)) k_sw16(DReads rd, DIndex ix, DParams P, const WTask* __restrict__ tk, const uint32_t* __restrict__ tidx1,
-                                                           const uint32_t* __restrict__ tidx2, const unsigned long long* __restrict__ wc, uint2* __restrict__ res) {
+                                                           const uint32_t* __restrict__ tidx2, const uint32_t* __restrict__ tidx3, const unsigned long long* __restrict__ wc, uint2* __restrict__ res) {
   const int lane = lane_id(), g = lane >> 2, gl = lane & 3;
-  const uint32_t ntA = (uint32_t)wc[WC_NTASK], ntB = (uint32_t)wc[WC_NTASK2];
-  const uint32_t npassA = (ntA + 15u) / 16u, npass = npassA + (ntB + 15u) / 16u;
-  auto slot_of = [&](uint32_t p) -> uint32_t {
-    const bool keys = p < npassA;
-    const uint32_t ti = (keys ? p : p - npassA) * 16u + (uint32_t)g;
-    return (p < npass && ti < (keys ? ntA : ntB)) ? (keys ? tidx1 : tidx2)[ti] : NONE;
-  };
-  uint32_t slot_next = slot_of(blockIdx.x);
+  const uint32_t ntA = (uint32_t)wc[WC_NTASK], ntB = (uint32_t)wc[WC_NTASK2], ntC = (uint32_t)wc[WC_NTASK3];
+  const uint32_t npassA = (ntA + 15u) / 16u, npassB = npassA + (ntB + 15u) / 16u, npass = npassB + (ntC + 15u) / 16u;
+#define SW16_LIST_OF(p, lp, ln, p0)                              \
+  const uint32_t* lp = tidx1; uint32_t ln = ntA, p0 = 0u;        \
+  if ((p) >= npassA) { lp = tidx2; ln = ntB; p0 = npassA; }      \
+  if ((p) >= npassB) { lp = tidx3; ln = ntC; p0 = npassB; }
+  uint32_t slot_next = NONE;
+  { SW16_LIST_OF(blockIdx.x, lp, ln, p0)
+    const uint32_t ti = (blockIdx.x - p0) * 16u + (uint32_t)g;
+    if (blockIdx.x < npass && ti < ln) slot_next = lp[ti]; }
   for (uint32_t p = blockIdx.x; p < npass; p += gridDim.x) {
-    const bool keys = p < npassA;
-    const uint32_t ti = (keys ? p : p - npassA) * 16u + (uint32_t)g;
-    const uint32_t* const tidx = keys ? tidx1 : tidx2;
+    const bool keys = p < npassA, prefix = p >= npassB;
+    SW16_LIST_OF(p, tidx, ln_, p0_)
+    const uint32_t ti = (p - p0_) * 16u + (uint32_t)g;
     const uint32_t slot = slot_next;
     const bool have = slot != NONE;
-    int m = 0, n = 0, aq = 0, dir = 1;
+    int m = 0, n = 0, aq = 0, dir = 1, rem = 0;
     uint32_t len = 0, reversed = 0;
     const uint32_t* rec = rd.words;
     const uint8_t* ref = ix.ref_seq;
@@ -225,8 +252,13 @@
       m = t.m; n = t.nref; aq = t.aq; reversed = t.flags & 1u; dir = (t.flags & 2u) ? -1 : 1;
       len = rd.len[t.r]; rec = rd.words + rd.rec_off[t.r];
       ref = ix.ref_seq + t.rf_start;
+      if (prefix) { const int cols = (int)WT_COLS(t.flags); rem = n - cols; n = cols; }
     }
-    slot_next = slot_of(p + gridDim.x);
+    slot_next = NONE;
+    { const uint32_t pn = p + gridDim.x;
+      SW16_LIST_OF(pn, lp, ln, p0)
+      const uint32_t tn = (pn - p0) * 16u + (uint32_t)g;
+      if (pn < npass && tn < ln) slot_next = lp[tn]; }
     int nn = n;
     for (int d = 32; d > 0; d >>= 1) nn = max(nn, __shfl_xor(nn, d, 64));
     bool hn = false;
@@ -243,9 +275,11 @@
     SwRes s;
     const bool hasn = __any(hn);
 #define SW16_ARGS rec, len, reversed, m, aq, ref, n, P.match, P.mismatch, P.score_N, P.gap_open, P.gap_ext, dir
-    if (keys) { if (hasn) s = sw_quad16<R, true, true>(SW16_ARGS); else s = sw_quad16<R, false, true>(SW16_ARGS); }
-    else { if (hasn) s = sw_quad16<R, true, false>(SW16_ARGS); else s = sw_quad16<R, false, false>(SW16_ARGS); }
+    if (keys) { if (hasn) s = sw_quad16<R, true, SW16_KEYS>(SW16_ARGS); else s = sw_quad16<R, false, SW16_KEYS>(SW16_ARGS); }
+    else if (prefix) { if (hasn) s = sw_quad16<R, true, SW16_PREFIX>(SW16_ARGS, rem); else s = sw_quad16<R, false, SW16_PREFIX>(SW16_ARGS, rem); }
+    else { if (hasn) s = sw_quad16<R, true, SW16_SCORE>(SW16_ARGS); else s = sw_quad16<R, false, SW16_SCORE>(SW16_ARGS); }
 #undef SW16_ARGS
+#undef SW16_LIST_OF
     if (have && gl == 0) res[tidx[ti]] = wres_pack(s);
   }
 }
@@ -258,8 +292,8 @@
 k_walk(DReads rd, DIndex ix, DParams P, int pass, int is_last_strand, RState* __restrict__ work, AlignRec* __restrict__ work_aln, RWork* __restrict__ rw,
        unsigned long long* __restrict__ ctr, const uint2* __restrict__ mrec, const uint32_t* __restrict__ mpool, const uint32_t* __restrict__ pool,
        const uint2* __restrict__ list, const WState* __restrict__ ws_prev, const WTask* __restrict__ tk_prev, const uint2* __restrict__ res_prev,
-       WState* __restrict__ ws_cur, WTask* __restrict__ tk_cur, uint32_t* __restrict__ tidx, uint32_t* __restrict__ tidx2, unsigned long long* __restrict__ wc,
-       uint32_t K0, unsigned long long task_cap, int round, uint32_t lds_ml, uint32_t lds_rf, uint32_t assume_min) {
+       WState* __restrict__ ws_cur, WTask* __restrict__ tk_cur, uint32_t* __restrict__ tidx, uint32_t* __restrict__ tidx2, uint32_t* __restrict__ tidx3, unsigned long long* __restrict__ wc,
+       uint32_t K0, unsigned long long task_cap, int round, uint32_t lds_ml, uint32_t lds_rf, uint32_t assume_min, uint32_t prefix_pct, unsigned long long* __restrict__ pstat) {
   SMR_DYN_LDS(unsigned char, lds_raw);
   __shared__ unsigned long long l_pairs[WK_MAX_POS];
   __shared__ uint2 l_cand[64];
@@ -270,12 +304,16 @@
   __shared__ WTask s_ctk[WK_MAX];
   __shared__ uint2 s_cres[WK_MAX];
   __shared__ uint32_t s_tix[WK_CLAIM * WK_MAX];
-  __shared__ uint32_t s_next, s_tbase;
+  __shared__ uint32_t s_next, s_tbase, s_tbase3;
   const int lane = lane_id();
   const uint32_t nlist = (uint32_t)wc[WC_NLIST];
   const uint32_t K = walk_tasks_per_read(nlist, task_cap, K0, round);
   const uint32_t Kp = round > 0 ? walk_tasks_per_read((uint32_t)(wc - WC_STRIDE)[WC_NLIST], task_cap, K0, round - 1) : K0;
   unsigned long long n_fwd = 0, n_cells = 0, n_spec = 0, n_spec_used = 0, n_newhit = 0;
+  __shared__ unsigned long long s_wps[WPS_AHEAD_CELLS + 1];
+  if (lane < WPS_AHEAD_CELLS + 1) s_wps[lane] = 0;
+#define WPS_ADD(i, v) { if (lane == 0) s_wps[i] += (unsigned long long)(v); }
+  const bool pfx_opts = P.is_best && P.num_alignments > 0;
 #ifdef SMR_WALK_PHASES
   unsigned long long wph[7] = {0, 0, 0, 0, 0, 0, 0}, wlast = clock64();
 #define WPH(i) { const unsigned long long tn_ = clock64(); wph[i] += tn_ - wlast; wlast = tn_; }
@@ -290,7 +328,7 @@
     const uint32_t chunk_base = s_next;
     if (chunk_base >= nlist) break;
     const uint32_t chunk_n = min(claim, nlist - chunk_base);
-    uint32_t ntix = 0, ntix2 = 0;
+    uint32_t ntix = 0, ntix2 = 0, ntix3 = 0;
     uint32_t c_r = 0, c_prev = NONE, c_len = 0;
     uint2 c_mr = make_uint2(NONE, 0u);
     if ((uint32_t)lane < chunk_n) { const uint2 le = list[chunk_base + lane]; c_r = le.x; c_prev = le.y; c_mr = mrec[c_r]; c_len = rd.len[c_r]; }
@@ -518,10 +556,10 @@
             wk.k++; wk.started = 0;
           }
         };
-        auto put_task = [&](uint32_t j, const SwTask& t) {
+        auto put_task = [&](uint32_t j, const SwTask& t, uint32_t cols = 0) {
           if (lane == 0) {
             WTask o; o.r = r; o.max_ref = t.max_ref; o.rf_start = t.rf_start; o.ars = (uint32_t)t.align_ref_start; o.head = (uint32_t)t.head; o.aq = (uint16_t)t.align_que_start;
-            o.m = (uint16_t)t.m; o.nref = (uint16_t)t.nref; o.flags = w.reversed ? 1 : 0;
+            o.m = (uint16_t)t.m; o.nref = (uint16_t)t.nref; o.flags = (uint16_t)((w.reversed ? 1u : 0u) | cols);
             tk_cur[(size_t)e * K + j] = o;
           }
         };
@@ -543,6 +581,7 @@
           have_tk = true;
         }
         const uint32_t max_SW_score = len * (uint32_t)P.match;
+        bool pfx_off = prev != NONE && (ps.bits & 128u);
         bool live = false, rdq_staged = false, dirty = false;
         for (;;) {
           WPH(3)
@@ -558,13 +597,20 @@
             if (have_tk) ce = 0;
             else for (uint32_t q = 0; q < n_prev; q++)
               if (s_ctk[q].max_ref == tk.max_ref && s_ctk[q].rf_start == tk.rf_start && (uint32_t)s_ctk[q].aq == (uint32_t)tk.align_que_start && (int)s_ctk[q].m == m && (int)s_ctk[q].nref == nref) { ce = (int)q; break; }
-            if (ce >= 0) { fw = wres_unpack(s_cres[ce]); if (ce > 0) n_spec_used++; }
+            if (ce >= 0 && s_cres[ce].y == WRES_PREFIX) {
+              const uint32_t lo = s_cres[ce].x & 0xFFFFu, hi = s_cres[ce].x >> 16;
+              bool dec = lo > P.minimal_score && hi < max_SW_score && pfx_opts && st.n_align == (uint32_t)P.num_alignments;
+              if (dec) { __syncthreads(); dec = hi <= (uint32_t)(work_aln + (size_t)r * P.slots)[st.min_index].score1; }
+              if (dec) { fw.score = (int)lo; fw.end_ref = -2; fw.end_read = 0; WPS_ADD(WPS_DECIDED, 1) n_spec_used++; }
+              else { WPS_ADD(WPS_REDONE, 1) ce = -1; pfx_off = true; }
+            } else if (ce >= 0) { fw = wres_unpack(s_cres[ce]); if (ce > 0) n_spec_used++; }
+            if (ce >= 0) {}
             else if (!FINAL) {
               const int assume = prev == NONE ? ((ncand > 0 && (l_cand[0].y & 0xFFu) >= assume_min) ? 1 : 0) : last_aligned;
               WState o; o.k = R.k; o.it = R.it; o.ms_lo = R.ms_lo; o.ms_hi = R.ms_hi; o.begin_ref = R.begin_ref; o.begin_read = R.begin_read; o.best = R.best;
               const uint32_t bits0 = (uint32_t)(R.is_aligned & 1) | ((uint32_t)(R.go_on & 1) << 1) | ((uint32_t)(R.started & 1) << 2) | ((uint32_t)(R.pending_pop & 1) << 3) | ((uint32_t)(search & 1) << 4) |
-                                     ((uint32_t)(last_aligned & 1) << 6);
-              uint32_t nk = 1, cells = (uint32_t)m * (uint32_t)nref;
+                                     ((uint32_t)(last_aligned & 1) << 6) | (pfx_off ? 128u : 0u);
+              uint32_t nk = 1, cells = (uint32_t)m * (uint32_t)nref, pfx_mask = 0;
               put_task(0, tk);
               R.is_aligned = assume;
               bool ended = false;
@@ -572,14 +618,19 @@
                 SwTask t2;
                 if (advance(R, t2) != 1) { ended = true; break; }
                 if (!task_ok(t2)) break;
-                put_task(nk, t2); nk++; cells += (uint32_t)t2.m * (uint32_t)t2.nref;
+                uint32_t cols = 0;
+                if (assume && pfx_opts) {
+                  WPS_ADD(WPS_AHEAD, 1) WPS_ADD(WPS_AHEAD_CELLS, (uint32_t)t2.m * (uint32_t)t2.nref)
+                  if (prefix_pct && !pfx_off) { cols = walk_prefix_cols((uint32_t)t2.nref, prefix_pct); if (cols >= (uint32_t)t2.nref) cols = 0; }
+                }
+                put_task(nk, t2, cols); pfx_mask |= (cols ? 1u : 0u) << nk; nk++; cells += (uint32_t)t2.m * (uint32_t)t2.nref;
                 R.is_aligned = assume;
               }
               n_spec += nk - 1;
               o.bits = bits0 | ((ended && !assume) ? 32u : 0u) | (nk << 8); o.cells = cells;
               if (lane == 0) ws_cur[e] = o;
               live_bits = nk << 8;
-              if (assume) { for (uint32_t q = lane; q < nk; q += 64) s_tix[ntix + q] = e * K + q; ntix += nk; }
+              if (assume) { for (uint32_t q = lane; q < nk; q += 64) s_tix[ntix + q] = (e * K + q) | (((pfx_mask >> q) & 1u) << 31); ntix += nk; ntix3 += (uint32_t)__popc(pfx_mask); WPS_ADD(WPS_SCORED, __popc(pfx_mask)) }
               else { for (uint32_t q = lane; q < nk; q += 64) s_tix[WK_CLAIM * WK_MAX - 1u - (ntix2 + q)] = e * K + q; ntix2 += nk; }
               live = true;
               WPH(4)
@@ -659,10 +710,21 @@
     }
     if (!FINAL && ntix) {
       __syncthreads();
-      if (lane == 0) s_tbase = (uint32_t)atomicAdd(&wc[WC_NTASK], (unsigned long long)ntix);
+      if (lane == 0) {
+        s_tbase = (uint32_t)atomicAdd(&wc[WC_NTASK], (unsigned long long)(ntix - ntix3));
+        if (ntix3) s_tbase3 = (uint32_t)atomicAdd(&wc[WC_NTASK3], (unsigned long long)ntix3);
+      }
       __syncthreads();
-      const uint32_t tb = s_tbase;
-      for (uint32_t q = lane; q < ntix; q += 64) tidx[tb + q] = s_tix[q];
+      uint32_t tb = s_tbase, tb3 = ntix3 ? s_tbase3 : 0u;
+      const unsigned long long below = (1ull << lane) - 1ull;
+      for (uint32_t q0 = 0; q0 < ntix; q0 += 64) {
+        const uint32_t q = q0 + (uint32_t)lane, v = q < ntix ? s_tix[q] : 0u;
+        const bool is3 = q < ntix && (v >> 31), is1 = q < ntix && !(v >> 31);
+        const unsigned long long m1 = __ballot(is1), m3 = __ballot(is3);
+        if (is1) tidx[tb + (uint32_t)__popcll(m1 & below)] = v;
+        if (is3) tidx3[tb3 + (uint32_t)__popcll(m3 & below)] = v & 0x7FFFFFFFu;
+        tb += (uint32_t)__popcll(m1); tb3 += (uint32_t)__popcll(m3);
+      }
     }
     if (!FINAL && ntix2) {
       __syncthreads();
@@ -679,11 +741,13 @@
     if (n_spec) atomicAdd(&ctr[C_SW_SPEC], n_spec);
     if (n_spec_used) atomicAdd(&ctr[C_SW_SPEC_USED], n_spec_used);
     if (n_newhit) { atomicAdd(&ctr[C_NUM_ALIGNED], n_newhit); atomicAdd(&ctr[C_PER_DB + P.index_num], n_newhit); }
+    for (int q = 0; q <= WPS_AHEAD_CELLS; q++) if (s_wps[q]) atomicAdd(&pstat[q], s_wps[q]);
 #ifdef SMR_WALK_PHASES
     for (int q = 0; q < 7; q++) if (wph[q]) atomicAdd(&ctr[C_SHARDS + (blockIdx.x & (C_NSHARD - 1)) * C_SHARD_W + C_SHARD_PH + q], wph[q]);
 #endif
   }
 #undef WPH
+#undef WPS_ADD
 }
 
 __global__ void __launch_bounds__(1024) k_wnext(DParams P, int is_last_strand, RState* __restrict__ work, RWork* __restrict__ rw, unsigned long long* __restrict__ ctr,
diff --git a/sortmerna_amd/engine.py b/sortmerna_amd/engine.py
--- a/sortmerna_amd/engine.py
+++ b/sortmerna_amd/engine.py
@@ -294,6 +294,24 @@
         self._chk(self.L.smr_sw16_batch(self.h, n, t.ctypes.data, rf.ctypes.data, len(ref), int(bool(force_any_n)), match, mismatch, score_N, gap_open, gap_ext,
                                         filters, rows, blocks, out.ctypes.data), "smr_sw16_batch")
         return out[:n]
+
+    SW16_PREFIX_TASK = np.dtype([("read", "<u4"), ("win_off", "<u4"), ("aq", "<u2"), ("m", "<u2"), ("nref", "<u2"), ("cols", "<u2"), ("reversed", "u1"), ("pad_", "V3")])
+
+    def sw16_prefix_batch(self, tasks, ref, rows, match=2, mismatch=-3, score_N=-3, gap_open=5, gap_ext=2, blocks=0, force_any_n=False, **_):
+        n = len(tasks)
+        t = np.zeros(max(n, 1), dtype=self.SW16_PREFIX_TASK)
+        for i, (r, aq, m, rev, wo, nref, cols) in enumerate(tasks):
+            t[i] = (r, wo, aq, m, nref, cols, rev, b"")
+        rf = np.frombuffer(bytes(ref) + b"\0", dtype=np.uint8).copy()
+        out = np.zeros((max(n, 1), 2), dtype=np.int32)
+        self._chk(self.L.smr_sw16_prefix_batch(self.h, n, t.ctypes.data, rf.ctypes.data, len(ref), int(bool(force_any_n)), match, mismatch, score_N, gap_open, gap_ext,
+                                               rows, blocks, out.ctypes.data), "smr_sw16_prefix_batch")
+        return out[:n]
+
+    def walk_prefix_stats(self):
+        out = (C.c_uint64 * 8)()
+        self._chk(self.L.smr_walk_prefix_stats(self.h, out), "smr_walk_prefix_stats")
+        return dict(zip(("scored", "decided", "redone", "unused", "ahead", "ahead_cells", "percent", "live"), out[:8]))
 
     def sw16_launches(self):
         out = (C.c_uint64 * 8)()
```
